# DearPoca/CppPathTracer

Hardware: AMD Instinct MI355X
Metric: Mpaths/sec (pixels×spp/s) at 1920×1080; achieved HBM GB/s vs peak (higher is better)
Workload: dtype f32; 1 GPU; c4: s1000 1920x1080 1024spp depth 16; width=1920, height=1080, spp=1024, max_depth=16, seed=1234, rows_rendered=1080, walk=ordered, schedule=cost, tail_consolidation=False, scaling=strong, parallelism=row-tiled x1 (interleaved 8-row blocks)

## Files before the change

cpppathtracer_amd/_lib.py:

```python
import ctypes
import os

from . import build as _build

_lib = None

_P = ctypes.c_void_p
_I = ctypes.c_int
_U32 = ctypes.c_uint32
_U64 = ctypes.c_uint64
_SZ = ctypes.c_size_t
PROTOTYPES = {
    "cpt_abi_version": (_I, []),
    "cpt_status_string": (ctypes.c_char_p, [_I]),
    "cpt_get_device_count": (_I, [_P]),
    "cpt_create": (_I, [_I, _P]),
    "cpt_destroy": (_I, [_P]),
    "cpt_last_error": (ctypes.c_char_p, [_P]),
    "cpt_set_stream": (_I, [_P, _P]),
    "cpt_camera_get_copy": (_I, [_P]),
    "cpt_set_scene": (_I, [_P, _P, _I]),
    "cpt_update_object": (_I, [_P, _I, _P]),
    "cpt_update_objects": (_I, [_P, _I, _P, _P]),
    "cpt_update_objects_rebuild": (_I, [_P, _I, _P, _P]),
    "cpt_last_update_ms": (_I, [_P, _P]),
    "cpt_get_material_count": (_I, [_P, _P]),
    "cpt_scene_bvh_export": (_I, [_P, _P, _P, _I, _P]),
    "cpt_bvh_build_host": (_I, [_P, _I, _P, _P, _I, _P]),
    "cpt_set_env_texture": (_I, [_P, _P, _I, _I, _I]),
    "cpt_bind_texture": (_I, [_P, _U64, _P, _I, _I, _I, _I, _I]),
    "cpt_set_frame": (_I, [_P, _I, _I, _P, _I]),
    "cpt_init_rng": (_I, [_P, _U64]),
    "cpt_read_rng": (_I, [_P, _P]),
    "cpt_write_rng": (_I, [_P, _P]),
    "cpt_render": (_I, [_P, _P, _I, _I, _U32]),
    "cpt_synchronize": (_I, [_P]),
    "cpt_read_accum": (_I, [_P, _P]),
    "cpt_clear_accum": (_I, [_P]),
    "cpt_read_aux": (_I, [_P, _P, _P]),
    "cpt_write_accum": (_I, [_P, _P]),
    "cpt_write_aux": (_I, [_P, _P, _P]),
    "cpt_copy_accum_device": (_I, [_P, _P, _SZ, _P]),
    "cpt_gather_rows": (_I, [_P, _P]),
    "cpt_last_gather_mode": (_I, [_P, _P, _P]),
    "cpt_set_debug_gather": (_I, [_P, _I]),
    "cpt_get_stats": (_I, [_P, _P]),
    "cpt_reset_stats": (_I, [_P]),
    "cpt_get_raw_counters": (_I, [_P, _P]),
    "cpt_get_walk_info": (_I, [_P, _P]),
    "cpt_debug_read_nodes": (_I, [_P, _P, _SZ, _P]),
    "cpt_debug_read_tile_order": (_I, [_P, _I, _P, _SZ, _P]),
    "cpt_measure_read_bandwidth": (_I, [_P, _SZ, _I, _P]),
    "cpt_measure_read_pattern": (_I, [_P, _I, _SZ, _I, _P]),
    "cpt_cap_disk_bound": (_I, [ctypes.c_float, _P]),
    "cpt_last_render_ms": (_I, [_P, _P]),
    "cpt_get_diag_counters": (_I, [_P, _P]),
    "cpt_get_execdiag_counters": (_I, [_P, _P]),
    "cpt_last_kernel_stats": (_I, [_P, _P, _P]),
    "cpt_denoise_mix": (_I, [_P, _U32, _P]),
    "cpt_host_register": (_I, [_P, _SZ]),
    "cpt_host_unregister": (_I, [_P]),
    "cpt_denoise_mix_band": (_I, [_P, _U32, _I, _I, _P]),
    "cpt_copy_bgra_device": (_I, [_P, _P, _SZ, _P]),
    "cpt_last_display_ms": (_I, [_P, _P]),
    "cpt_reset_display": (_I, [_P]),
    "cpt_display_band": (_I, [_P, _P, _P]),
    "cpt_debug_timeline": (_I, [_P, _P, _I]),
    "cpt_tile_costs": (_I, [_P, _P, _I, _I, ctypes.c_uint32, _P, _SZ]),
    "cpt_read_mix": (_I, [_P, _P, _SZ]),
    "cpt_math_batch": (_I, [_P, _I, _P, _P, _P, _SZ]),
    "cpt_selftest_qdiv": (_I, [_P, _I, _U64, _U64, _P, _I]),
    "cpt_set_debug_consolidation": (_I, [_P, _U32, _I, _I]),
    "cpt_set_debug_grid": (_I, [_P, _I, _I]),
    "cpt_render_adaptive": (_I, [_P, _P, _I, _I, _I, ctypes.c_float, _I, _U32]),
    "cpt_adaptive_begin": (_I, [_P, _P, _I, _I, _I, ctypes.c_float, _I, _U32]),
    "cpt_adaptive_step": (_I, [_P, _P]),
    "cpt_read_noise": (_I, [_P, _P, _SZ]),
    "cpt_adaptive_info": (_I, [_P, _P, _P, _I, _P]),
    "cpt_adaptive_decide_host": (_I, [ctypes.c_float, ctypes.c_float, ctypes.c_float, ctypes.c_float, _P, _P]),
    "cpt_read_moments": (_I, [_P, _P, _SZ]),
    "cpt_write_moments": (_I, [_P, _P, _SZ]),
    "cpt_filter_frame": (_I, [_P, _I, ctypes.c_float, _I]),
    "cpt_read_filtered": (_I, [_P, _P, _P, _SZ]),
    "cpt_last_filter_ms": (_I, [_P, _P]),
    "cpt_filter_prepare_host": (_I, [_SZ, _P, _P, _P, _P]),
    "cpt_filter_level_host": (_I, [_I, _I, _I, _P, _P, _P, ctypes.c_float, _I, _P]),
}

CPT_RENDER_ACCUMULATE = 0x1
CPT_RENDER_AUX = 0x2
CPT_RENDER_STATS = 0x4
CPT_RENDER_SYNC = 0x8
CPT_PATH_MEGAKERNEL = 0x000
CPT_PATH_WAVEFRONT = 0x100
CPT_TRAVERSAL_ORDERED = 0x200
CPT_TRAVERSAL_PLAIN_LEAVES = 0x400
CPT_SCHEDULE_COST = 0x800
CPT_SCHEDULE_CONSOLIDATE = 0x1000
CPT_SCHEDULE_NO_CONSOLIDATE = 0x2000
CPT_SCHEDULE_PREVIOUS = 0x4000
CPT_ERR_STATE = 5
CPT_ERR_DEVICE = 7


class CptError(RuntimeError):
    def __init__(self, status, msg):
        super().__init__(f"[cpt status {status}] {msg}")
        self.status = status


def lib_path() -> str:
    return _build.LIB_PATH


def load(build_if_missing: bool = True):
    global _lib
    if _lib is not None:
        return _lib
    path = os.environ.get("CPT_LIB_PATH") or _build.LIB_PATH
    if not os.path.exists(path):
        if not build_if_missing:
            raise CptError(-1, f"{path} missing: run __graft_entry__.build() (hipcc) first")
        _build.build()
    L = ctypes.CDLL(path)
    ab_variant = "CPT_LIB_PATH" in os.environ
    for name, (res, args) in PROTOTYPES.items():
        if ab_variant and not hasattr(L, name):
            continue
        f = getattr(L, name)
        f.restype = res
        f.argtypes = args
    if L.cpt_abi_version() != 1:
        raise CptError(-1, f"libcpt ABI {L.cpt_abi_version()} != 1")
    _lib = L
    return L


def check(status, ctx=None):
    if status != 0:
        L = load()
        msg = L.cpt_last_error(ctx)
        raise CptError(status, (msg or b"").decode() or L.cpt_status_string(status).decode())
    return status
```

cpppathtracer_amd/csrc/cpt_capi_render.cpp:

```cpp
#include <hip/hip_runtime.h>

#include <algorithm>
#include <cstdlib>
#include <cstring>
#include <type_traits>
#include <utility>

#include "cpt_context.hpp"

using namespace cpt::ctx;

constexpr int PREV_ORDER_EVERY = 8;

void cpt::ctx::fill_params(cpt_ctx* c, const cpt_camera* cam, int spp, int max_depth, uint32_t flags, cpt::KParams& p) {
    std::memset(&p, 0, sizeof(p));
    p.nodes = c->d_nodes;
    p.mats = c->d_mats;
    p.n_nodes = c->n_bvh;
    p.n_walk = c->n_walk;
    p.n_wide = c->n_wide;
    p.n_unb = c->n_unb;
    p.n_leaves = c->n_wide > 0 ? c->n_leaves : 0;
    p.ordered = (flags & CPT_TRAVERSAL_ORDERED) ? ((flags & CPT_TRAVERSAL_PLAIN_LEAVES) ? 2 : 1) : 0;
    p.env = c->d_env;
    p.env_w = c->env_w;
    p.env_h = c->env_h;
    p.env_cols = c->d_env ? c->env_cols : 0;
    for (int k = 0; k < 3; ++k) {
        p.cam.origin[k] = (&cam->origin.x)[k];
        p.cam.u[k] = (&cam->u.x)[k];
        p.cam.v[k] = (&cam->v.x)[k];
        p.cam.top_left[k] = (&cam->top_left_corner.x)[k];
        p.cam.horizontal[k] = (&cam->horizontal.x)[k];
        p.cam.vertical[k] = (&cam->vertical.x)[k];
    }
    p.cam.lens_radius = cam->lens_radius;
    p.cam.width = cam->width;
    p.cam.height = cam->height;
    p.cam.inv_w = 1.0 / (double)(float)cam->width;
    p.cam.inv_h = 1.0 / (double)(float)cam->height;
    p.rows = c->frame.d_rows;
    p.n_rows = c->n_rows;
    p.width = c->width;
    p.rng = c->frame.d_rng;
    p.accum = c->frame.d_accum;
    p.normal = c->frame.d_normal;
    p.depth = c->frame.d_depth;
    p.stats = c->d_stats;
    p.work = c->d_work;
    p.spp = spp;
    p.max_depth = max_depth;
    p.accumulate = (flags & CPT_RENDER_ACCUMULATE) ? 1 : 0;
    p.lanes = 64;
#ifdef CPT_DIAGNOSTIC_LANES
    if (const char* e = getenv("CPT_LANES_PER_WAVE")) p.lanes = std::max(1, std::min(64, atoi(e)));
    if (const char* e = getenv("CPT_REPLICATE")) p.replicate = std::max(1, std::min(64, atoi(e)));
#endif
    if (p.replicate < 1) p.replicate = 1;
    if (c->dbg_lanes_per_wave > 0) p.lanes = c->dbg_lanes_per_wave;
    p.error = c->d_work + 4;
    p.dbg = c->dbg;
    p.keeper_spin_log2 = c->keeper_spin_log2;
    p.publish_wait_log2 = c->publish_wait_log2;
}

int cpt::ctx::renderable(cpt_ctx* c, const cpt_camera* cam, const char* who) {
    if (!c->scene_set) return fail(c, CPT_ERR_STATE, "%s: cpt_set_scene first", who);
    if (!c->frame.set || !c->frame.rng_set) return fail(c, CPT_ERR_STATE, "%s: cpt_set_frame + cpt_init_rng first", who);
    if (cam->width != c->width || cam->height != c->height)
        return fail(c, CPT_ERR_INVALID_ARG, "%s: camera %dx%d vs frame %dx%d", who, cam->width, cam->height, c->width, c->height);
    return CPT_OK;
}

size_t cpt::ctx::n_tiles(const cpt_ctx* c) { return (size_t)cpt::TileGrid{c->width, c->n_rows}.count(); }

int WfStorage::alloc(cpt_ctx* c, size_t npix, cpt::WfState& view) {
    WfStorage fresh;
    cpt::WfState v{};
    int rc = CPT_OK;
    auto take = [&](auto*& slot, size_t count) {
        using T = std::remove_reference_t<decltype(*slot)>;
        if (rc != CPT_OK) return;
        fresh.mem.emplace_back();
        rc = fresh.mem.back().ensure(c, count * sizeof(T));
        slot = reinterpret_cast<T*>(fresh.mem.back().get());
    };
    for (int b = 0; b < 2; ++b)
        for (float4** a : {&v.ray_o[b], &v.ray_d[b], &v.att[b], &v.rad[b], &v.aux[b]}) take(*a, npix);
    take(v.hit_p, npix);
    take(v.hit_n, npix);
    for (int b = 0; b < 2; ++b) {
        take(v.rng_a[b], npix);
        take(v.rng_b[b], npix);
    }
    for (int32_t** q : {&v.queue[0], &v.queue[1], &v.ident}) take(*q, npix);
    take(v.counts, 8);
    if (rc != CPT_OK) return rc;
    *this = std::move(fresh);
    view = v;
    return CPT_OK;
}

static int ensure_wavefront(cpt_ctx* c, const cpt::KParams& p, hipStream_t s) {
    Frame& f = c->frame;
    if (f.wavefront.ready || c->n_rows == 0) return CPT_OK;
    if (int rc = f.wavefront.mem.alloc(c, c->npix(), f.wavefront.view)) return rc;
    HIP_TRY(c, cpt::wavefront_build_ident(p, f.wavefront.view, s));
    f.wavefront.ready = true;
    return CPT_OK;
}

int TileSchedule::previous_begin(cpt_ctx* c, cpt::KParams& p, hipStream_t s) {
    const size_t npix = c->npix();
    if (prev_order_valid) p.tile_order = d_prev_order;
    if (int rc = d_prev_d.ensure(c, npix)) return rc;
    if (!prev_d_valid) {
        HIP_TRY(c, hipMemcpyAsync(d_prev_d, c->frame.d_rng + 5 * npix, npix * sizeof(uint32_t), hipMemcpyDeviceToDevice, s));
        prev_d_valid = true;
    }
    return CPT_OK;
}

int TileSchedule::previous_refresh(cpt_ctx* c, const cpt::KParams& p, hipStream_t s) {
    if (prev_order_valid && ++prev_since_order < PREV_ORDER_EVERY) return CPT_OK;
    int rc;
    if ((rc = d_scratch.ensure(c, cpt::tile_schedule_scratch_bytes(c->width, c->n_rows))) != CPT_OK) return rc;
    if ((rc = d_prev_order.ensure(c, n_tiles(c))) != CPT_OK) return rc;
    HIP_TRY(c, cpt::launch_tile_order_from_draws(p, d_prev_d, d_scratch, d_scratch.capacity(), d_prev_order, s));
    prev_d_valid = true;
    prev_order_valid = true;
    prev_since_order = 0;
    return CPT_OK;
}

constexpr int PILOT_MAX = 16, PILOT_DIV = 128;
int cpt::ctx::cost_pilot_passes(int spp) { return std::min(PILOT_MAX, std::max(1, spp / PILOT_DIV)); }
int cpt::ctx::cost_pilot(cpt_ctx* c, const cpt::KParams& p, int passes, hipStream_t s) {
    Frame& f = c->frame;
    int rc;
    if ((rc = f.schedule.d_scratch.ensure(c, cpt::tile_schedule_scratch_bytes(c->width, c->n_rows))) != CPT_OK) return rc;
    if ((rc = f.schedule.d_cost_order.ensure(c, n_tiles(c))) != CPT_OK) return rc;
    HIP_TRY(c, cpt::launch_tile_schedule(p, passes, f.schedule.d_scratch, f.schedule.d_scratch.capacity(), f.schedule.d_cost_order,
                                         c->dbg_max_workgroups, s));
    return CPT_OK;
}

int cpt::ctx::consolidation_slab(cpt_ctx* c, cpt::KParams& p, int spp, uint32_t flags) {
    const size_t cus = (size_t)c->cus;
    const size_t frame_px = c->npix(), grid_lanes = 1024u * cus;
    const bool cons = (flags & CPT_SCHEDULE_CONSOLIDATE) ||
                      (!(flags & CPT_SCHEDULE_NO_CONSOLIDATE) && spp >= 512 && frame_px > grid_lanes &&
                       frame_px <= 4u * grid_lanes);
    if (!cons || spp <= 1) return CPT_OK;
    const size_t cap = 3u * 256u * cus;
    if (int rc = c->d_resume.ensure(c, 5 * cap)) return rc;
    p.resume = c->d_resume;
    p.resume_cap = cap;
    return CPT_OK;
}

extern "C" {

int cpt_render(cpt_ctx* c, const cpt_camera* cam, int spp, int max_depth, uint32_t flags) {
    if (!c || !cam) return CPT_ERR_INVALID_ARG;
    if (spp < 0 || max_depth < 0 || max_depth > (int)cpt::MAX_RECURSION_DEPTH_SET)
        return fail(c, CPT_ERR_INVALID_ARG, "cpt_render: spp %d, max_depth %d (must be 0..32)", spp, max_depth);
    CPT_REFUSE_PENDING(c, "cpt_render");
    if (int rc = renderable(c, cam, "cpt_render")) return rc;
    Frame& f = c->frame;
    HIP_TRY(c, hipSetDevice(c->device));
    hipStream_t s = c->stream();
    int rc;
    const bool aux = (flags & CPT_RENDER_AUX) != 0;
    if (aux) {
        if ((rc = f.d_normal.ensure(c, c->npix() * 3)) != CPT_OK) return rc;
        if ((rc = f.d_depth.ensure(c, c->npix())) != CPT_OK) return rc;
    }
    cpt::KParams p;
    fill_params(c, cam, spp, max_depth, flags, p);
    const bool wavefront = (flags & CPT_PATH_WAVEFRONT) != 0;
    const bool work = spp > 0 && c->n_rows > 0;
    if (wavefront && (rc = ensure_wavefront(c, p, s)) != CPT_OK) return rc;
    HIP_TRY(c, hipEventRecord(c->t_render.t0, s));
    if (wavefront) {
        if (!p.accumulate && c->n_rows > 0) HIP_TRY(c, hipMemsetAsync(f.d_accum, 0, c->npix() * sizeof(float4), s));
        int launches = 0;
        HIP_TRY(c, hipEventRecord(c->ev_main, s));
        HIP_TRY(c, cpt::launch_wavefront(p, f.wavefront.view, (flags & CPT_RENDER_STATS) != 0, aux, s, &launches));
        c->last_launches = launches;
        HIP_TRY(c, hipEventRecord(c->t_render.t1, s));
    } else {
        c->last_launches = 1;
        const bool cost = (flags & CPT_SCHEDULE_COST) && work;
        const bool previous = !(flags & CPT_SCHEDULE_COST) && (flags & CPT_SCHEDULE_PREVIOUS) && work;
        if (previous && (rc = f.schedule.previous_begin(c, p, s)) != CPT_OK) return rc;
        if (cost) {
            if ((rc = cost_pilot(c, p, cost_pilot_passes(spp), s)) != CPT_OK) return rc;
            p.tile_order = f.schedule.d_cost_order;
        }
        if ((rc = consolidation_slab(c, p, spp, flags)) != CPT_OK) return rc;
        HIP_TRY(c, hipEventRecord(c->ev_main, s));
        HIP_TRY(c, cpt::launch_megakernel(p, (flags & CPT_RENDER_STATS) != 0, aux, c->dbg_max_workgroups, s));
        HIP_TRY(c, hipEventRecord(c->t_render.t1, s));
        if (previous && (rc = f.schedule.previous_refresh(c, p, s)) != CPT_OK) return rc;
    }
    c->t_render.recorded = true;
    if (flags & CPT_RENDER_SYNC) return sync_checked(c);
    return CPT_OK;
}

int cpt_tile_costs(cpt_ctx* c, const cpt_camera* cam, int passes, int max_depth, uint32_t flags, uint32_t* out,
                   size_t n_out) {
    if (!c || !cam || !out || passes < 1 || max_depth < 0 || max_depth > (int)cpt::MAX_RECURSION_DEPTH_SET)
        return CPT_ERR_INVALID_ARG;
    if (int rc = renderable(c, cam, "cpt_tile_costs")) return rc;
    if (n_out < n_tiles(c)) return fail(c, CPT_ERR_INVALID_ARG, "cpt_tile_costs: %zu < %zu tiles", n_out, n_tiles(c));
    if (n_tiles(c) == 0) return CPT_OK;
    HIP_TRY(c, hipSetDevice(c->device));
    hipStream_t s = c->stream();
    cpt::KParams p;
    fill_params(c, cam, passes, max_depth, flags & (CPT_TRAVERSAL_ORDERED | CPT_TRAVERSAL_PLAIN_LEAVES), p);
    if (int rc = cost_pilot(c, p, passes, s)) return rc;
    HIP_TRY(c, hipMemcpyAsync(out, c->frame.schedule.d_scratch, n_tiles(c) * sizeof(uint32_t), hipMemcpyDeviceToHost, s));
    return sync_checked(c);
}

int cpt_set_debug_consolidation(cpt_ctx* c, uint32_t flags, int keeper_spin_log2, int publish_wait_log2) {
    if (!c || keeper_spin_log2 < 0 || keeper_spin_log2 > 30 || publish_wait_log2 < 0 || publish_wait_log2 > 30 ||
        (flags & ~3u))
        return c ? fail(c, CPT_ERR_INVALID_ARG, "cpt_set_debug_consolidation: bad arguments") : CPT_ERR_INVALID_ARG;
    c->dbg = flags;
    c->keeper_spin_log2 = keeper_spin_log2;
    c->publish_wait_log2 = publish_wait_log2;
    return CPT_OK;
}

int cpt_set_debug_grid(cpt_ctx* c, int max_workgroups, int lanes_per_wave) {
    if (!c || max_workgroups < 0 || lanes_per_wave < 0 || lanes_per_wave > 64)
        return c ? fail(c, CPT_ERR_INVALID_ARG, "cpt_set_debug_grid: bad arguments") : CPT_ERR_INVALID_ARG;
    c->dbg_max_workgroups = max_workgroups;
    c->dbg_lanes_per_wave = lanes_per_wave;
    return CPT_OK;
}

int cpt_last_render_ms(cpt_ctx* c, float* ms) {
    if (!c || !ms) return CPT_ERR_INVALID_ARG;
    if (!c->t_render.recorded) return fail(c, CPT_ERR_STATE, "cpt_last_render_ms: nothing rendered");
    HIP_TRY(c, hipSetDevice(c->device));
    HIP_TRY(c, hipEventSynchronize(c->t_render.t1));
    HIP_TRY(c, hipEventElapsedTime(ms, c->t_render.t0, c->t_render.t1));
    c->last_kernel_ms = *ms;
    return CPT_OK;
}

int cpt_last_kernel_stats(cpt_ctx* c, float* avg_ms, int* launches) {
    if (!c || !avg_ms || !launches) return CPT_ERR_INVALID_ARG;
    float ms = 0.f;
    int rc = cpt_last_render_ms(c, &ms);
    if (rc != CPT_OK) return rc;
    HIP_TRY(c, hipEventElapsedTime(&ms, c->ev_main, c->t_render.t1));
    *launches = c->last_launches;
    *avg_ms = c->last_launches > 0 ? ms / (float)c->last_launches : 0.f;
    return CPT_OK;
}

}
```

cpppathtracer_amd/csrc/cpt_context.hpp:

```cpp
#pragma once

#include <hip/hip_runtime.h>

#include <cstdint>
#include <string>
#include <vector>

#include "../../include/cpt.h"
#include "cpt_devmem.hpp"
#include "cpt_host.hpp"
#include "cpt_internal.hpp"
#include "cpt_tiles.hpp"

using cpt::Mat;
using cpt::Node;
using cpt::TexDesc;
using cpt::ctx::DevBuf;
using cpt::ctx::DevEvent;
using cpt::host::HostBvh;

struct WfStorage {
    std::vector<DevBuf<uint8_t>> mem;
    int alloc(cpt_ctx* c, size_t npix, cpt::WfState& view);
};


struct TileSchedule {
    DevBuf<uint8_t> d_scratch;
    DevBuf<uint32_t> d_cost_order;
    DevBuf<uint32_t> d_prev_d, d_prev_order;

    void rng_replaced() {
        prev_d_valid = prev_order_valid = false;
        prev_since_order = 0;
    }
    void draws_moved() { prev_d_valid = false; }
    const uint32_t* previous_order() const { return prev_order_valid ? d_prev_order.get() : nullptr; }
    int previous_begin(cpt_ctx* c, cpt::KParams& p, hipStream_t s);
    int previous_refresh(cpt_ctx* c, const cpt::KParams& p, hipStream_t s);

private:
    bool prev_d_valid = false, prev_order_valid = false;
    int prev_since_order = 0;
};

struct WavefrontState {
    cpt::WfState view{};
    WfStorage mem;
    bool ready = false;
};

struct DisplayBand {
    DevBuf<float> d_mix;
    DevBuf<uint8_t> d_bgra;
    DevBuf<float4> d_sink;
    int y0 = -1, y1 = -1;
};

struct AdaptiveState {
    DevBuf<float4> d_snap;
    DevBuf<float> d_stat;
    DevBuf<uint32_t> d_keep, d_order[2], d_count;
    bool done = false;
    std::vector<uint32_t> rounds;
    uint64_t passes = 0;
    struct Pending {
        bool on = false, queued = false;
        cpt::KParams p{};
        bool stats = false, aux = false;
        int batch = 0, min_spp = 0, max_rounds = 0;
        float rel_error = 0.f;
        int round = 0;
        uint32_t active = 0;
        int into = 0;
    } pending;

    bool has_result(size_t npix) const { return done && d_stat.capacity() >= 4 * npix; }
    void adopt_result() {
        rounds.clear();
        passes = 0;
        done = true;
    }
};

struct FilterState {
    DevBuf<float4> d_plane[2];
    DevBuf<uint8_t> d_ok;
    int result = -1;
};

struct Frame {
    bool set = false, rng_set = false;
    DevBuf<int32_t> d_rows;
    DevBuf<uint32_t> d_rng;
    DevBuf<float4> d_accum;
    DevBuf<float> d_normal, d_depth;
    DevBuf<uint32_t> d_scratch_w, d_scratch_m;
    TileSchedule schedule;
    WavefrontState wavefront;
    DisplayBand display;
    AdaptiveState adaptive;
    FilterState filter;
};

struct TimedSpan {
    DevEvent t0, t1;
    bool recorded = false;
};

struct cpt_ctx {
    int device = 0;
    int cus = 1;
    cpt::ctx::DevStream own_stream;
    hipStream_t user_stream = nullptr;
    TimedSpan t_render;
    DevEvent ev_main;
    TimedSpan t_display;
    TimedSpan t_filter;
    std::string err;

    std::vector<cpt_object> objs;
    HostBvh bvh;
    std::vector<Node> lin;
    std::vector<int> pos_of_node;
    int n_bvh = 0;
    int n_walk = 0;
    int n_wide = 0;
    int n_unb = 0;
    int n_leaves = 0;
    std::vector<Mat> mats_h;
    std::vector<int> mat_have_tex;
    std::vector<uint64_t> mat_tex;
    std::vector<int> mat_of_obj;
    DevBuf<Node> d_nodes;
    DevBuf<Mat> d_mats;
    bool scene_set = false;
    std::vector<cpt::RefitNode> refit_plan;
    std::vector<int32_t> refit_parent, refit_height, refit_walk_leaf;
    std::vector<cpt::Box6> refit_boxes;
    std::vector<uint8_t> refit_mark;
    int refit_n_ref = 0;
    DevBuf<cpt::RefitNode> d_refit_plan;
    DevBuf<cpt::Box6> d_refit_boxes;
    DevBuf<uint8_t> d_refit_work;
    float last_update_ms = 0.f;

    struct Texture { uint64_t handle; DevBuf<uint32_t> d_texels; int w, h, cols, addr, filter; };
    std::vector<Texture> textures;
    DevBuf<TexDesc> d_texdescs;
    DevBuf<int32_t> d_tex_of_mat;

    DevBuf<uint32_t> d_env;
    int env_w = 1, env_h = 1, env_cols = 0;

    int width = 0, height = 0, n_rows = 0;
    std::vector<int32_t> rows_h;
    uint64_t frame_gen = 0;
    Frame frame;

    DevBuf<uint32_t> d_jumps;
    DevBuf<unsigned long long> d_stats;
    DevBuf<uint32_t> d_work;
    DevBuf<uint4> d_resume;
    float last_kernel_ms = 0.f;
    int last_launches = 0;
    struct GatherMap {
        const cpt_ctx* src = nullptr;
        uint64_t src_gen = 0, dst_gen = 0;
        int src_device = -1;
        bool peer = false;
        int mode = -1;
        DevBuf<int32_t> d_map;
    };
    std::vector<GatherMap> gather_maps;
    DevBuf<float4> d_gather;
    DevBuf<float> d_gather_stat;
    cpt::ctx::HostPinned<uint32_t> h_ad_words;
    DevEvent ev_round;
    DevEvent ev_ready;
    DevEvent ev_gathered;
    DevEvent ev_caller;
    DevEvent ev_copied;
    uint32_t dbg = 0;
    bool force_staged_gather = false;
    int keeper_spin_log2 = 0, publish_wait_log2 = 0;
    int dbg_max_workgroups = 0, dbg_lanes_per_wave = 0;

    hipStream_t stream() const { return user_stream ? user_stream : (hipStream_t)own_stream; }
    size_t npix() const { return (size_t)n_rows * width; }
};

namespace cpt {
namespace ctx {

#define CPT_REFUSE_PENDING(ctx, who)                                                                              \
    do {                                                                                                          \
        if ((ctx)->frame.adaptive.pending.on)                                                                           \
            return fail((ctx), CPT_ERR_STATE, who ": an adaptive render is pending (cpt_adaptive_step until 0)"); \
    } while (0)

int check_device_error(cpt_ctx* c);
int sync_checked(cpt_ctx* c);
int copy_ordered(cpt_ctx* c, void* dst, const void* src, size_t bytes, hipStream_t caller);
int renderable(cpt_ctx* c, const cpt_camera* cam, const char* who);
void fill_params(cpt_ctx* c, const cpt_camera* cam, int spp, int max_depth, uint32_t flags, cpt::KParams& p);
size_t n_tiles(const cpt_ctx* c);
int cost_pilot_passes(int spp);
int cost_pilot(cpt_ctx* c, const cpt::KParams& p, int passes, hipStream_t s);
int consolidation_slab(cpt_ctx* c, cpt::KParams& p, int spp, uint32_t flags);

int material_slot(cpt_ctx* c, const cpt_material& m);
void linearise_all(cpt_ctx* c);
int upload_scene(cpt_ctx* c);
int upload_materials(cpt_ctx* c);
int device_refit(cpt_ctx* c, int n, const int* indices, bool mats_changed);

}
}
```

cpppathtracer_amd/csrc/cpt_host.hpp:

```cpp
#pragma once

#include <cstdint>
#include <vector>

#include "../../include/cpt.h"
#include "cpt_internal.hpp"

namespace cpt {
namespace host {

struct F3 { float x, y, z; };

inline float MIN_(float a, float b) { return a < b ? a : b; }
inline float MAX_(float a, float b) { return a > b ? a : b; }
inline float ABS_(float a) { return a >= 0 ? a : -a; }

F3 aabb_max(const cpt_object& o);
F3 aabb_min(const cpt_object& o);

struct BNode {
    F3 bmin, bmax;
    bool is_object;
    int left, right, obj, parent;
    int axis;
};

struct HostBvh {
    std::vector<BNode> nodes;
    std::vector<int> leaf_of_object;
};

void build_host_bvh(HostBvh& b, const std::vector<cpt_object>& objs);
float cap_disk_bound(float r);
Node make_node(const BNode& n, const std::vector<cpt_object>& objs, const std::vector<int>& mat_of_obj);
void linearise(const HostBvh& b, const std::vector<cpt_object>& objs, const std::vector<int>& mat_of_obj,
               std::vector<Node>& out, std::vector<int>& pos_of_node, int octant, const std::vector<int>* ref_pos,
               int root = 0, const std::vector<int>& prefix = {});

namespace sah {
int leaf(HostBvh& t, const std::vector<cpt_object>& O, int o);
int build(HostBvh& t, const std::vector<cpt_object>& O, std::vector<int>& idx, int l, int r);
}

constexpr int WIDE_STACK = CPT_WSTACK;
int linearise_wide(const HostBvh& w, int root, const std::vector<int>& pos0, int n_bvh, int n_unb,
                   std::vector<Node>& out, int* n_leaves_out, std::vector<int>& slot_of, std::vector<int>& leaf_of);

const std::vector<uint32_t>& jump_tables();
void curand_seed_state(uint64_t seed, uint32_t out[6]);

}
}
```

cpppathtracer_amd/csrc/cpt_host_bvh.cpp:

```cpp
#include <algorithm>
#include <cfloat>
#include <cmath>
#include <cstring>
#include <functional>
#include <mutex>
#include <queue>
#include <vector>

#include "cpt_host.hpp"

namespace cpt {
namespace host {


F3 aabb_max(const cpt_object& o) {
    const float tol = 2e-5f * 5.f;
    switch (o.type) {
        case CPT_PRIM_SPHERE: {
            float r = ABS_(o.radius);
            return F3{o.center.x + r, o.center.y + r, o.center.z + r};
        }
        case CPT_PRIM_PLATFORM: return F3{1e30f * 5, o.y_pos + tol, 1e30f * 5};
        case CPT_PRIM_CYLINDER:
            return F3{o.center.x + ABS_(o.radius), o.center.y + o.height / 2 + tol, o.center.z + ABS_(o.radius)};
        default: return F3{0, 0, 0};
    }
}

F3 aabb_min(const cpt_object& o) {
    const float tol = 2e-5f * 5.f;
    switch (o.type) {
        case CPT_PRIM_SPHERE: {
            float r = ABS_(o.radius);
            return F3{o.center.x - r, o.center.y - r, o.center.z - r};
        }
        case CPT_PRIM_PLATFORM: return F3{-1e30f * 5, o.y_pos - tol, -1e30f * 5};
        case CPT_PRIM_CYLINDER:
            return F3{o.center.x - ABS_(o.radius), o.center.y - o.height / 2 - tol, o.center.z - ABS_(o.radius)};
        default: return F3{0, 0, 0};
    }
}


static int divide(HostBvh& b, const std::vector<cpt_object>& objs, std::vector<int>& idx, int l, int r) {
    if (l >= r) return -1;
    int ret = (int)b.nodes.size();
    b.nodes.push_back(BNode{});
    F3 lmin = aabb_min(objs[idx[l]]), lmax = aabb_max(objs[idx[l]]);
    if (l == r - 1) {
        BNode& n = b.nodes[ret];
        n.left = n.right = -1;
        n.bmin = lmin; n.bmax = lmax;
        n.is_object = true;
        n.obj = idx[l];
        b.leaf_of_object[idx[l]] = ret;
        return ret;
    }
    float minx = lmin.x, miny = lmin.y, minz = lmin.z, maxx = lmax.x, maxy = lmax.y, maxz = lmax.z;
    for (int i = l + 1; i < r; ++i) {
        F3 a = aabb_min(objs[idx[i]]), c = aabb_max(objs[idx[i]]);
        minx = MIN_(minx, a.x); miny = MIN_(miny, a.y); minz = MIN_(minz, a.z);
        maxx = MAX_(maxx, c.x); maxy = MAX_(maxy, c.y); maxz = MAX_(maxz, c.z);
    }
    float sx = maxx - minx, sy = maxy - miny, sz = maxz - minz;
    int axis = (sx >= sy && sx >= sz) ? 0 : (sy >= sz ? 1 : 2);
    std::vector<std::pair<float, int>> keyed;
    keyed.reserve(r - l);
    for (int i = l; i < r; ++i) {
        F3 a = aabb_min(objs[idx[i]]), c = aabb_max(objs[idx[i]]);
        float lo = axis == 0 ? a.x : axis == 1 ? a.y : a.z;
        float hi = axis == 0 ? c.x : axis == 1 ? c.y : c.z;
        keyed.emplace_back((lo + hi) / 2, idx[i]);
    }
    std::stable_sort(keyed.begin(), keyed.end(),
                     [](const std::pair<float, int>& p, const std::pair<float, int>& q) { return p.first < q.first; });
    for (int i = l; i < r; ++i) idx[i] = keyed[i - l].second;
    int mid = (l + r) / 2;
    int left = divide(b, objs, idx, l, mid);
    int right = divide(b, objs, idx, mid, r);
    BNode& n = b.nodes[ret];
    n.left = left; n.right = right;
    n.bmin = F3{minx, miny, minz};
    n.bmax = F3{maxx, maxy, maxz};
    n.is_object = false;
    n.obj = -1;
    n.axis = axis;
    b.nodes[left].parent = ret;
    b.nodes[right].parent = ret;
    return ret;
}

void build_host_bvh(HostBvh& b, const std::vector<cpt_object>& objs) {
    b.nodes.clear();
    b.leaf_of_object.assign(objs.size(), -1);
    if (objs.empty()) return;
    b.nodes.reserve(2 * objs.size());
    std::vector<int> idx(objs.size());
    for (size_t i = 0; i < objs.size(); ++i) idx[i] = (int)i;
    divide(b, objs, idx, 0, (int)objs.size());
    b.nodes[0].parent = -1;
}

float cap_disk_bound(float r) {
    if (!(r > 0.0f)) return -1.0f;
    if (r == INFINITY) return FLT_MAX;
    const double m = ((double)std::nextafter(r, 0.0f) + (double)r) * 0.5;
    const double x = m * m;
    float c = (float)x;
    if ((double)c > x) c = std::nextafter(c, -INFINITY);
    return c;
}

Node make_node(const BNode& n, const std::vector<cpt_object>& objs, const std::vector<int>& mat_of_obj) {
    Node g;
    if (n.is_object) {
        const cpt_object& o = objs[n.obj];
        g.a0 = o.center.x; g.a1 = o.center.y; g.a2 = o.center.z;
        g.b0 = o.radius; g.b1 = o.y_pos; g.b2 = o.height;
        int type = (o.type >= 0 && o.type <= 2) ? o.type : 3;
        if (type == CPT_PRIM_CYLINDER) g.b1 = cap_disk_bound(o.radius);
        if (type == CPT_PRIM_SPHERE) {
            const double inv_r = 1.0 / (double)o.radius;
            uint32_t w[2];
            std::memcpy(w, &inv_r, 8);
            std::memcpy(&g.b1, &w[0], 4);
            std::memcpy(&g.b2, &w[1], 4);
        }
        g.code = (mat_of_obj[n.obj] << 2) | type;
    } else {
        g.a0 = n.bmin.x; g.a1 = n.bmin.y; g.a2 = n.bmin.z;
        g.b0 = n.bmax.x; g.b1 = n.bmax.y; g.b2 = n.bmax.z;
        g.code = -1;
    }
    g.miss = -1;
    return g;
}

void linearise(const HostBvh& b, const std::vector<cpt_object>& objs, const std::vector<int>& mat_of_obj,
               std::vector<Node>& out, std::vector<int>& pos_of_node, int octant, const std::vector<int>* ref_pos,
               int root, const std::vector<int>& prefix) {
    const size_t base = out.size();
    pos_of_node.assign(b.nodes.size(), -1);
    for (int leaf : prefix) {
        pos_of_node[leaf] = (int)(out.size() - base);
        out.push_back(make_node(b.nodes[leaf], objs, mat_of_obj));
        out.back().miss = (*ref_pos)[leaf];
    }
    if (b.nodes.empty() || root < 0) return;
    struct Frame { int node; int stage; };
    std::vector<Frame> st;
    st.push_back({root, 0});
    while (!st.empty()) {
        Frame& f = st.back();
        const BNode& n = b.nodes[f.node];
        if (f.stage == 0) {
            pos_of_node[f.node] = (int)(out.size() - base);
            out.push_back(make_node(n, objs, mat_of_obj));
            if (n.is_object) {
                out.back().miss = ref_pos ? (*ref_pos)[f.node] : pos_of_node[f.node];
                st.pop_back();
                continue;
            }
            if (octant >= 0) {
                Node& q = out.back();
                if (octant & 1) std::swap(q.a0, q.b0);
                if (octant & 2) std::swap(q.a1, q.b1);
                if (octant & 4) std::swap(q.a2, q.b2);
            }
            f.stage = 1;
            const bool right_first = octant < 0 || ((octant >> n.axis) & 1);
            st.push_back({right_first ? n.right : n.left, 0});
        } else if (f.stage == 1) {
            f.stage = 2;
            const bool right_first = octant < 0 || ((octant >> n.axis) & 1);
            st.push_back({right_first ? n.left : n.right, 0});
        } else {
            out[base + pos_of_node[f.node]].miss = (int)(out.size() - base);
            st.pop_back();
        }
    }
}

namespace sah {
constexpr int NB = 16;
inline float comp(const F3& v, int a) { return a == 0 ? v.x : (a == 1 ? v.y : v.z); }
inline F3 fmin3(const F3& a, const F3& b) { return F3{MIN_(a.x, b.x), MIN_(a.y, b.y), MIN_(a.z, b.z)}; }
inline F3 fmax3(const F3& a, const F3& b) { return F3{MAX_(a.x, b.x), MAX_(a.y, b.y), MAX_(a.z, b.z)}; }
inline float area(const F3& lo, const F3& hi) {
    const float dx = hi.x - lo.x, dy = hi.y - lo.y, dz = hi.z - lo.z;
    return 2.f * (dx * dy + dy * dz + dz * dx);
}
inline int bin_of(float c, float e0, float e1) { return std::min(NB - 1, (int)((c - e0) / (e1 - e0) * NB)); }

int leaf(HostBvh& t, const std::vector<cpt_object>& O, int o) {
    BNode n{};
    n.bmin = aabb_min(O[o]);
    n.bmax = aabb_max(O[o]);
    n.is_object = true;
    n.left = n.right = -1;
    n.obj = o;
    n.parent = -1;
    t.nodes.push_back(n);
    return (int)t.nodes.size() - 1;
}

int build(HostBvh& t, const std::vector<cpt_object>& O, std::vector<int>& idx, int l, int r) {
    if (r - l == 1) return leaf(t, O, idx[l]);
    F3 lo = aabb_min(O[idx[l]]), hi = aabb_max(O[idx[l]]);
    F3 clo{1e30f, 1e30f, 1e30f}, chi{-1e30f, -1e30f, -1e30f};
    std::vector<float> cen(3 * (r - l));
    for (int i = l; i < r; ++i) {
        const F3 a = aabb_min(O[idx[i]]), b = aabb_max(O[idx[i]]);
        lo = fmin3(lo, a);
        hi = fmax3(hi, b);
        const F3 c{(a.x + b.x) * .5f, (a.y + b.y) * .5f, (a.z + b.z) * .5f};
        cen[3 * (i - l)] = c.x; cen[3 * (i - l) + 1] = c.y; cen[3 * (i - l) + 2] = c.z;
        clo = fmin3(clo, c);
        chi = fmax3(chi, c);
    }
    float best = 3.0e38f;
    int best_axis = -1, best_bin = -1;
    for (int axis = 0; axis < 3; ++axis) {
        const float e0 = comp(clo, axis), e1 = comp(chi, axis);
        if (!(e1 > e0)) continue;
        int cnt[NB] = {0};
        F3 blo[NB], bhi[NB];
        for (int b = 0; b < NB; ++b) { blo[b] = F3{1e30f, 1e30f, 1e30f}; bhi[b] = F3{-1e30f, -1e30f, -1e30f}; }
        for (int i = l; i < r; ++i) {
            const int b = bin_of(cen[3 * (i - l) + axis], e0, e1);
            cnt[b]++;
            blo[b] = fmin3(blo[b], aabb_min(O[idx[i]]));
            bhi[b] = fmax3(bhi[b], aabb_max(O[idx[i]]));
        }
        for (int sp = 1; sp < NB; ++sp) {
            int nl = 0, nr = 0;
            F3 llo{1e30f, 1e30f, 1e30f}, lhi{-1e30f, -1e30f, -1e30f}, rlo = llo, rhi = lhi;
            for (int b = 0; b < sp; ++b) if (cnt[b]) { nl += cnt[b]; llo = fmin3(llo, blo[b]); lhi = fmax3(lhi, bhi[b]); }
            for (int b = sp; b < NB; ++b) if (cnt[b]) { nr += cnt[b]; rlo = fmin3(rlo, blo[b]); rhi = fmax3(rhi, bhi[b]); }
            if (!nl || !nr) continue;
            const float cost = area(llo, lhi) * nl + area(rlo, rhi) * nr;
            if (cost < best) { best = cost; best_axis = axis; best_bin = sp; }
        }
    }
    int axis, mid;
    if (best_axis < 0) {
        axis = 0;
        mid = (l + r) / 2;
    } else {
        axis = best_axis;
        const float e0 = comp(clo, axis), e1 = comp(chi, axis);
        std::vector<int> lhs, rhs;
        for (int i = l; i < r; ++i)
            (bin_of(cen[3 * (i - l) + axis], e0, e1) < best_bin ? lhs : rhs).push_back(idx[i]);
        std::copy(lhs.begin(), lhs.end(), idx.begin() + l);
        std::copy(rhs.begin(), rhs.end(), idx.begin() + l + (int)lhs.size());
        mid = l + (int)lhs.size();
    }
    const int me = (int)t.nodes.size();
    t.nodes.push_back(BNode{});
    const int L = build(t, O, idx, l, mid), R = build(t, O, idx, mid, r);
    BNode& n = t.nodes[me];
    n.bmin = lo; n.bmax = hi;
    n.is_object = false;
    n.left = L; n.right = R; n.obj = -1; n.parent = -1; n.axis = axis;
    t.nodes[L].parent = me;
    t.nodes[R].parent = me;
    return me;
}
}


int linearise_wide(const HostBvh& w, int root, const std::vector<int>& pos0, int n_bvh, int n_unb,
                   std::vector<Node>& out, int* n_leaves_out, std::vector<int>& slot_of, std::vector<int>& leaf_of) {
    std::vector<int> wbin;
    std::vector<std::vector<int>> kids;
    std::vector<int> wide_of(w.nodes.size(), -1);
    auto area = [&](int b) {
        const BNode& n = w.nodes[b];
        const float dx = n.bmax.x - n.bmin.x, dy = n.bmax.y - n.bmin.y, dz = n.bmax.z - n.bmin.z;
        return dx * dy + dy * dz + dz * dx;
    };
    int max_push = 0;
    std::function<void(int, int)> make = [&](int b, int pushed) {
        const int id = (int)wbin.size();
        wbin.push_back(b);
        wide_of[b] = id;
        std::vector<int> ch = {w.nodes[b].left, w.nodes[b].right};
        while (ch.size() < 4) {
            int best = -1;
            float ba = -1.f;
            for (size_t k = 0; k < ch.size(); ++k)
                if (!w.nodes[ch[k]].is_object && area(ch[k]) > ba) { ba = area(ch[k]); best = (int)k; }
            if (best < 0) break;
            const int x = ch[best];
            ch.erase(ch.begin() + best);
            ch.insert(ch.begin() + best, {w.nodes[x].left, w.nodes[x].right});
        }
        kids.push_back(ch);
        pushed += (int)ch.size() - 1;
        max_push = std::max(max_push, pushed);
        for (int x : ch)
            if (!w.nodes[x].is_object) make(x, pushed);
    };
    make(root, n_unb);
    if (max_push + 1 > WIDE_STACK) return 0;
    const int n_wide = (int)wbin.size();
    std::vector<int> li_of(w.nodes.size(), -1), leaf_pos;
    for (int k = 0; k < n_unb; ++k) leaf_pos.push_back(k);
    for (int id = 0; id < n_wide; ++id)
        for (int x : kids[id])
            if (w.nodes[x].is_object && li_of[x] < 0) {
                li_of[x] = (int)leaf_pos.size();
                leaf_pos.push_back(pos0[x]);
            }
    if ((int)leaf_pos.size() > 32765) return 0;
    if (n_wide > cpt::LDS_TREE_NODES) {
        std::vector<char> top(n_wide, 0);
        std::priority_queue<std::pair<float, int>, std::vector<std::pair<float, int>>, std::greater<>> pq;
        pq.emplace(-area(wbin[0]), 0);
        for (int taken = 0; !pq.empty() && taken < cpt::LDS_TREE_NODES; ++taken) {
            const int id = pq.top().second;
            pq.pop();
            top[id] = 1;
            for (int x : kids[id])
                if (!w.nodes[x].is_object) pq.emplace(-area(x), wide_of[x]);
        }
        std::vector<int> order;
        order.reserve(n_wide);
        for (int part = 1; part >= 0; --part)
            for (int id = 0; id < n_wide; ++id)
                if (top[id] == part) order.push_back(id);
        std::vector<int> new_id(n_wide);
        for (int k = 0; k < n_wide; ++k) new_id[order[k]] = k;
        std::vector<int> wbin2(n_wide);
        std::vector<std::vector<int>> kids2(n_wide);
        for (int k = 0; k < n_wide; ++k) {
            wbin2[k] = wbin[order[k]];
            kids2[k] = kids[order[k]];
        }
        wbin.swap(wbin2);
        kids.swap(kids2);
        for (int& x : wide_of)
            if (x >= 0) x = new_id[x];
    }
    if (n_wide > 32767) return 0;
    for (int p : pos0)
        if (p > 32766) return 0;
    const size_t base = out.size();
    const size_t n_compact = (size_t)(n_wide * 7 + 1) / 2;
    out.resize(base + n_compact + leaf_pos.size());
    for (size_t i = 0; i < leaf_pos.size(); ++i) out[base + n_compact + i] = out[(size_t)n_bvh + leaf_pos[i]];
    *n_leaves_out = (int)leaf_pos.size();
    uint32_t* compact = reinterpret_cast<uint32_t*>(&out[base]);
    std::memset(compact, 0, n_compact * sizeof(Node));
    for (int id = 0; id < n_wide; ++id) {
        const std::vector<int>& ch = kids[id];
        std::vector<int> ord;
        std::function<void(int)> rec = [&](int x) {
            if (std::find(ch.begin(), ch.end(), x) != ch.end()) { ord.push_back(x); return; }
            rec(w.nodes[x].left);
            rec(w.nodes[x].right);
        };
        rec(wbin[id]);
        uint32_t* q = compact + (size_t)id * 28;
        for (int k = 0; k < 4; ++k) {
            F3 lo{1e30f, 1e30f, 1e30f}, hi{-1e30f, -1e30f, -1e30f};
            int32_t r = -1;
            if (k < (int)ord.size()) {
                const BNode& n = w.nodes[ord[k]];
                lo = n.bmin;
                hi = n.bmax;
                r = n.is_object ? ~(li_of[ord[k]] + 1) : wide_of[ord[k]];
            }
            const float l3[3] = {lo.x, lo.y, lo.z}, h3[3] = {hi.x, hi.y, hi.z};
            for (int a = 0; a < 3; ++a) {
                std::memcpy(&q[(2 * a) * 4 + k], &l3[a], 4);
                std::memcpy(&q[(2 * a + 1) * 4 + k], &h3[a], 4);
            }
            q[24 + (k >> 1)] |= (uint32_t)(uint16_t)(int16_t)r << (16 * (k & 1));
            if (k < (int)ord.size()) slot_of[ord[k]] = id * 4 + k;
        }
    }
    leaf_of = li_of;
    for (size_t b = 0; b < w.nodes.size(); ++b)
        if (w.nodes[b].is_object && leaf_of[b] < 0 && pos0[b] >= 0 && pos0[b] < n_unb) leaf_of[b] = pos0[b];
    return n_wide;
}

}
}
```

cpppathtracer_amd/csrc/cpt_internal.hpp:

```cpp
#pragma once

#include <hip/hip_runtime.h>
#include <stdint.h>

#include "cpt_device.hpp"

#define CPT_WSTACK 32

namespace cpt {

constexpr int LDS_TREE_NODES = 512;
__host__ __device__ __forceinline__ int lds_tree_nodes(int n_wide) { return n_wide < LDS_TREE_NODES ? n_wide : LDS_TREE_NODES; }

struct CamK {
    float origin[3];
    float u[3], v[3];
    float top_left[3], horizontal[3], vertical[3];
    float lens_radius;
    int width, height;
    double inv_w, inv_h;
};

struct KParams {
    const Node* nodes;
    const Mat* mats;
    int n_nodes, n_walk;
    int n_wide;
    int n_unb;
    int n_leaves;
    int ordered;
    const uint32_t* env;
    int env_w, env_h, env_cols;
    CamK cam;
    const int32_t* rows;
    int n_rows, width;
    uint32_t* rng;
    float4* accum;
    float* normal;
    float* depth;
    unsigned long long* stats;
    uint32_t* work;
    const uint32_t* tile_order;
    uint32_t* tile_cost;
    int spp, max_depth, accumulate;
    int lanes;
    int replicate;
    uint4* resume;
    size_t resume_cap;
    uint32_t* error;
    uint32_t dbg;
    int keeper_spin_log2, publish_wait_log2;
    uint32_t n_active;
};

enum : uint32_t {
    CPT_DEVERR_KEEPER_TIMEOUT = 1u,
    CPT_DEVERR_PUBLISH_TIMEOUT = 2u,
    CPT_DEVERR_RESUME_CAP = 4u,
};

size_t tile_schedule_scratch_bytes(int width, int n_rows);
hipError_t launch_cost_pilot(const KParams& p, int max_workgroups, hipStream_t stream);
hipError_t launch_tile_order_from_draws(const KParams& p, uint32_t* d_prev, void* scratch, size_t scratch_bytes,
                                        uint32_t* order, hipStream_t stream);
hipError_t launch_tile_schedule(const KParams& p, int passes, void* scratch, size_t scratch_bytes, uint32_t* order,
                                int max_workgroups, hipStream_t stream);

struct AdaptiveRound {
    const uint32_t* order;
    uint32_t n_active;
    int width, n_rows;
    const float4* accum;
    float4* snap;
    float* stat;
    uint32_t* keep;
    float rel_error;
    int eligible, last;
};
hipError_t launch_tile_noise(const AdaptiveRound& a, hipStream_t stream);
hipError_t launch_compact_order(const uint32_t* src, const uint32_t* keep, uint32_t n, int width, int n_rows,
                                uint32_t* dst, uint32_t* out, hipStream_t stream);

hipError_t launch_filter_prepare(const float4* accum, const float* stat, size_t npix, float4* plane, uint8_t* ok,
                                 hipStream_t stream);
hipError_t launch_filter_level(const float4* in, const float* normal3, const uint8_t* ok, float4* out, int width, int height,
                               int step, float sig2, int sharpness_log2, hipStream_t stream);

struct WfState {
    float4 *ray_o[2], *ray_d[2], *att[2], *rad[2], *aux[2];
    float4 *hit_p, *hit_n;
    uint4* rng_a[2];
    uint2* rng_b[2];
    int32_t* queue[2];
    int32_t* ident;
    uint32_t* counts;
};

struct RefitNode {
    int32_t left, right;
    int32_t slot;
    int32_t leaf;
    int32_t pos[8];
};
struct Box6 { float lo[3], hi[3]; };
struct RefitLeaf {
    Node prim;
    Box6 box;
    int32_t ref_id, walk_id;
};
hipError_t launch_refit(const RefitLeaf* leaves_in, int n_leaves, const int32_t* dirty, const int32_t* level_end,
                        int n_levels, int n_ref, const RefitNode* nodes_plan, Box6* boxes, Node* nodes, uint32_t* image,
                        Node* leaves, hipStream_t stream);

hipError_t launch_megakernel(const KParams& p, bool stats, bool aux, int max_workgroups, hipStream_t stream);
hipError_t launch_wavefront(const KParams& p, WfState& w, bool stats, bool aux, hipStream_t stream, int* launches);
hipError_t wavefront_build_ident(const KParams& p, WfState& w, hipStream_t stream);
hipError_t launch_prepare_materials(Mat* mats, const int32_t* tex_of_mat, const TexDesc* texs, int n,
                                    hipStream_t stream);
hipError_t launch_init_rng(const uint32_t* jumps, const uint32_t seed_state[6], int width, const int32_t* rows,
                           int n_rows, uint32_t* scratch_w, uint32_t* scratch_mats, uint32_t* rng, hipStream_t stream);
hipError_t launch_math_batch(int op, const float* a, const float* b, float* out, size_t n, hipStream_t stream);
hipError_t launch_stream_read(const float4* p, size_t n, float* out, int grid, hipStream_t stream);
hipError_t launch_read_pattern(int bpl, const float* p, size_t n_lanes, float* out, int grid, hipStream_t stream);
hipError_t timeline_read(unsigned long long* out, int n, hipStream_t stream);
hipError_t launch_selftest_qdiv(int which, uint64_t n, uint64_t seed, unsigned long long* out, int out_len,
                                hipStream_t stream);
hipError_t launch_selftest_dn_weight(int which, uint64_t n, unsigned long long* out, int out_len, hipStream_t stream);
hipError_t launch_stitch_rows(const float4* src_acc, const float* src_nrm, const float* src_dep, const int32_t* dst_row,
                              int width, int n_rows, float4* acc, float* nrm, float* dep, hipStream_t stream);
hipError_t launch_stitch_moments(const float* src, size_t src_npix, const int32_t* dst_row, int width, int n_rows,
                                 float* dst, size_t dst_npix, hipStream_t stream);
constexpr int DN_SINK_SLOTS = 1024 * 64;
hipError_t launch_denoise_mix(const float4* accum, const float* normal, const float* depth, float* mix, uint8_t* out,
                              uint8_t* out_host, float4* sink, int width, int height, int row0, int ctx_rows, int y0, int y1,
                              uint32_t cur_sample_idx, hipStream_t stream);

}
```

cpppathtracer_amd/csrc/cpt_megakernel.hip:

```cpp
#include <hip/hip_runtime.h>
#include <stdint.h>

#include <algorithm>

#include "cpt_path.hpp"

namespace cpt {

__device__ __forceinline__ uint32_t ld_coherent(const uint32_t* a) {
    return __hip_atomic_load(a, __ATOMIC_RELAXED, __HIP_MEMORY_SCOPE_AGENT);
}
__device__ __forceinline__ void st_coherent(uint32_t* a, uint32_t v) {
    __hip_atomic_store(a, v, __ATOMIC_RELAXED, __HIP_MEMORY_SCOPE_AGENT);
}
__device__ __forceinline__ void wait_stores() { asm volatile("s_waitcnt vmcnt(0)" ::: "memory"); }
template <int BLK> constexpr int ho_slots() { return (BLK / 256 - 1) * 256; }

struct Lane {
    uint32_t xy;
    uint32_t pix;
    uint32_t tile;
    Xorwow s;
    v3 sum;
    float passes;
    int left;
    template <bool ACC>
    __device__ __forceinline__ void load(const KParams& p, size_t npix) {
        s.v0 = p.rng[pix];
        s.v1 = p.rng[npix + pix];
        s.v2 = p.rng[2 * npix + (size_t)pix];
        s.v3 = p.rng[3 * npix + (size_t)pix];
        s.v4 = p.rng[4 * npix + (size_t)pix];
        s.d = p.rng[5 * npix + (size_t)pix];
        const float4 a = (p.accumulate && ACC) ? p.accum[pix] : make_float4(0.f, 0.f, 0.f, 0.f);
        sum = mk(a.x, a.y, a.z);
        passes = a.w;
    }
    __device__ __forceinline__ void store_rng(const KParams& p, size_t npix) const {
        p.rng[pix] = s.v0;
        p.rng[npix + pix] = s.v1;
        p.rng[2 * npix + (size_t)pix] = s.v2;
        p.rng[3 * npix + (size_t)pix] = s.v3;
        p.rng[4 * npix + (size_t)pix] = s.v4;
        p.rng[5 * npix + (size_t)pix] = s.d;
    }
};

template <int BLK>
struct PendingSky {
    float* q;
    __device__ __forceinline__ void park(const v3& dir, const v3& rad, const v3& att) const {
        q[0 * BLK] = dir.x; q[1 * BLK] = dir.y; q[2 * BLK] = dir.z;
        q[3 * BLK] = rad.x; q[4 * BLK] = rad.y; q[5 * BLK] = rad.z;
        q[6 * BLK] = att.x; q[7 * BLK] = att.y; q[8 * BLK] = att.z;
    }
    __device__ __forceinline__ v3 dir() const { return mk(q[0 * BLK], q[1 * BLK], q[2 * BLK]); }
    __device__ __forceinline__ v3 rad() const { return mk(q[3 * BLK], q[4 * BLK], q[5 * BLK]); }
    __device__ __forceinline__ v3 att() const { return mk(q[6 * BLK], q[7 * BLK], q[8 * BLK]); }
};

__device__ __forceinline__ bool decode_pixel(const KParams& p, uint32_t id, int& x, int& ri, uint32_t& tile) {
    tile = id >> 6;
    if (p.tile_order) tile = p.tile_order[tile];
    return TileGrid{p.width, p.n_rows}.pixel(tile, id & 63, x, ri);
}


template <bool LDST> constexpr int mk_block() { return LDST ? LDS_BLOCK : 256; }
template <bool LDST> constexpr int mk_waves() { return LDST ? LDS_BLOCK / 256 : WAVES_PER_SIMD; }

template <bool STATS, bool AUX, bool PROBE, bool LDST, bool CONS, bool HYB>
__global__ void __launch_bounds__(mk_block<LDST>(), mk_waves<LDST>()) k_megakernel(const KParams p) {
    constexpr bool COUNT = STATS || PROBE;
    constexpr int BLK = mk_block<LDST>();
    __shared__ uint4 s_tree[LDST ? LDS_TREE_NODES * 7 : 1];
    pooldiag::init();
    if (LDST) {
        const uint4* src = reinterpret_cast<const uint4*>(p.nodes + wide_image_base(p));
        for (int i = threadIdx.x; i < 7 * lds_tree_nodes(p.n_wide); i += BLK) s_tree[i] = src[i];
        __syncthreads();
    }
    const int lane = threadIdx.x & 63;
    const size_t npix = (size_t)p.n_rows * p.width;
    const uint32_t n_work = (p.n_active ? p.n_active : (uint32_t)TileGrid{p.width, p.n_rows}.count()) * 64u;
    const uint32_t max_depth = (uint32_t)p.max_depth;
    Counters cnt{};
    uint32_t work_at_take = 0;

    Lane L;
    bool busy = false;
    bool exhausted = false;
    Ray ray;
    v3 att = mk1(1.f), rad = mk1(0.f);
    uint32_t depth = 0;
    bool first = true;
    v3 first_normal = mk1(0.f);

    __shared__ float pending_q[DEFER_MISS_ROUND > 0 ? 9 * BLK : 1];
    const PendingSky<BLK> pq{pending_q + threadIdx.x};
    bool pend = false;
    WalkState ws;
    ws.active = false;
    static_assert(!CONS || (LDST && !PROBE && ho_slots<BLK>() > 0), "consolidation needs the LDS walk");
    constexpr int QS = CONS ? ho_slots<BLK>() : 1;
    __shared__ uint32_t s_q[CONS ? 4 : 1];
    __shared__ uint8_t s_qflag[QS];
    const bool cons = CONS && (size_t)(blockIdx.x + 1) * QS <= p.resume_cap;
    if (CONS && !cons && threadIdx.x == 0) atomicOr(p.error, CPT_DEVERR_RESUME_CAP);
    uint4* const qslab = cons ? p.resume + 5 * (size_t)blockIdx.x * QS : nullptr;
    volatile uint32_t* const vq = s_q;
    const uint32_t level = __builtin_amdgcn_readfirstlane((uint32_t)(threadIdx.x >> 8));
    bool retiring = false;
    uint32_t idle_spins = 0;
    const uint32_t keeper_spins = 1u << (p.keeper_spin_log2 > 0 ? p.keeper_spin_log2 : 26);
    const uint32_t publish_wait = 1u << (p.publish_wait_log2 > 0 ? p.publish_wait_log2 : 22);
    if (cons) {
        if (threadIdx.x < 4)
            s_q[threadIdx.x] = threadIdx.x == 3 ? (uint32_t)(BLK / 64) : (threadIdx.x == 2 ? (p.dbg & 1u) : 0u);
        for (int i = threadIdx.x; i < QS; i += BLK) s_qflag[i] = 0;
        __syncthreads();
    }
    auto start_pass = [&]() {
        ray = ray_gen(kernarg_field<CamK>(offsetof(KParams, cam)), (int)(L.xy & 0xffffu), (int)(L.xy >> 16), L.s);
        att = mk1(1.f);
        rad = mk1(0.f);
        depth = 0;
        first = true;
    };
    const bool stat = STATIC_FIRST && LDST && !PROBE && p.lanes == 64 && p.tile_order != nullptr;
    const uint32_t n_static = gridDim.x * (uint32_t)BLK;
    bool first_take = true;
    uint32_t res_id = 0, res_end = 0, res_seen = 0;
    bool counter_done = false;
    stamps::init();
    timeline::State tl;
    timeline::init(tl);
    for (;;) {
        stamps::lap(5);
        stamps::count(8);
        timeline::round(tl, __ballot(busy), exhausted, level);
        if (cons && !retiring && level > 0 && exhausted && vq[3] == 0u && vq[2] <= level * (uint32_t)CONS_RETIRE_PER_LEVEL) retiring = true;
        bool begin = false;
        if (!exhausted && !retiring) {
            const KParams& p = kernarg_params();
            const uint64_t need = __ballot(!busy && lane < p.lanes);
            if (need) {
                const int leader = __ffsll((unsigned long long)need) - 1;
                uint32_t base = 0;
                uint32_t lane_id = 0;
                const bool first_take_was = first_take;
                first_take = false;
                if (stat && first_take_was) {
                    base = (level * (gridDim.x * 4u) + blockIdx.x * 4u + ((threadIdx.x >> 6) & 3u)) * 64u;
                    if (n_static >= n_work) exhausted = true;
                    lane_id = base + lane_rank(need);
                }
                else if (p.replicate == 1) {
                    const uint32_t n_need = wave_count(need);
                    const uint32_t avail = res_end - res_id;
                    const uint32_t off = stat ? n_static : 0u;
                    uint32_t nb = 0, ncnt = 0;
                    if (n_need > avail && !counter_done) {
                        const uint32_t want = n_need - avail;
                        uint32_t seen = res_seen;
                        if (p.spp >= 64 && res_seen + n_static < n_work) {
                            uint32_t cur = 0;
                            if (lane == leader) cur = __hip_atomic_load(p.work, __ATOMIC_RELAXED, __HIP_MEMORY_SCOPE_AGENT);
                            seen = __builtin_amdgcn_readfirstlane(__shfl(cur, leader)) + off;
                        }
                        uint32_t bsz = (uint32_t)TAKE_BATCH;
                        const uint32_t left_ids = n_work > seen ? n_work - seen : 0u;
                        if (p.spp >= 64) {
                            const uint64_t t = (uint64_t)bsz * left_ids / ((uint64_t)n_static * TAKE_TAPER);
                            bsz = t < bsz ? (uint32_t)t : bsz;
                        }
                        const bool batch_ok = p.spp >= 64 || left_ids > n_static;
                        const uint32_t grab = !CONS && batch_ok && bsz > want ? bsz : want;
                        if (lane == leader) nb = atomicAdd(p.work, grab);
                        nb = __builtin_amdgcn_readfirstlane(__shfl(nb, leader)) + off;
                        ncnt = grab;
                    }
                    if (ncnt) {
                        res_seen = nb + ncnt;
                        if (nb + ncnt >= n_work) counter_done = true;
                    }
                    const uint32_t rank = lane_rank(need);
                    lane_id = rank < avail ? res_id + rank : (rank - avail < ncnt ? nb + (rank - avail) : n_work);
                    if (ncnt) {
                        res_id = nb + min(n_need - avail, ncnt);
                        res_end = nb + ncnt;
                    } else {
                        res_id += n_need < avail ? n_need : avail;
                    }
                    if (counter_done && res_id >= res_end) exhausted = true;
                }
                else {
                    const uint32_t rep = (uint32_t)p.replicate;
                    const uint32_t n_take = ((uint32_t)__popcll(need) + rep - 1) / rep;
                    if (lane == leader) base = atomicAdd(p.work, n_take);
                    base = __shfl(base, leader) + (stat ? n_static : 0u);
                    if (base + n_take >= n_work) exhausted = true;
                    lane_id = base + lane_rank(need) / rep;
                }
                bool took = false;
                if ((need >> lane) & 1ull) {
                    const uint32_t id = lane_id;
                    int x, ri;
                    if (id < n_work && decode_pixel(p, id, x, ri, L.tile)) {
                        execdiag::lanes(p.stats + 64, 0);
                        L.xy = (uint32_t)x | ((uint32_t)p.rows[ri] << 16);
                        L.pix = (uint32_t)ri * (uint32_t)p.width + (uint32_t)x;
                        L.load<!PROBE>(p, npix);
                        L.left = p.spp;
                        first_normal = mk1(0.f);
                        if (PROBE) work_at_take = cnt.segments + cnt.nodes + cnt.prims;
                        if (max_depth == 0) {
                            for (; L.left > 0; --L.left) {
                                (void)ray_gen(p, (int)(L.xy & 0xffffu), (int)(L.xy >> 16), L.s);
                                L.sum = L.sum + mk1(0.f);
                                L.passes += 1.0f;
                            }
                        }
                        busy = true;
                        took = true;
                        begin = L.left > 0;
                    }
                }
                if (cons) {
                    const uint64_t t = __ballot(took);
                    if (t && lane == leader) atomicAdd(&s_q[2], (uint32_t)__popcll(t));
                    if (exhausted && lane == leader) atomicSub(&s_q[3], 1u);
                }
            }
        }
        if (cons && !retiring && exhausted) {
            const uint64_t need = __ballot(!busy && lane < p.lanes);
            const bool idle_wave = !__any(busy);
            bool quit = false;
            for (;;) {
                if (idle_wave) {
                    while (vq[1] == vq[0]) {
                        if (vq[3] == 0u && vq[2] == 0u) { quit = true; break; }
                        if (++idle_spins > keeper_spins) {
                            if (lane == 0) atomicOr(p.error, CPT_DEVERR_KEEPER_TIMEOUT);
                            quit = true;
                            break;
                        }
                        __builtin_amdgcn_s_sleep(16);
                    }
                    if (quit) break;
                }
                if (need && vq[1] != vq[0]) {
                    const int leader = __ffsll((unsigned long long)need) - 1;
                    uint32_t h = 0, n = 0;
                    if (lane == leader) {
                        for (int tries = 0; tries < 16; ++tries) {
                            h = vq[0];
                            uint32_t t = vq[1];
                            t = t < (uint32_t)QS ? t : (uint32_t)QS;
                            const uint32_t want = (uint32_t)__popcll(need);
                            n = t > h ? (t - h < want ? t - h : want) : 0u;
                            if (n == 0 || atomicCAS(&s_q[0], h, h + n) == h) break;
                            n = 0;
                        }
                    }
                    h = __shfl(h, leader);
                    n = __shfl(n, leader);
                    const uint32_t rank = lane_rank(need);
                    bool lost = false;
                    if (((need >> lane) & 1ull) && rank < n) {
                        const uint32_t slot = h + rank;
                        const volatile uint8_t* fl = s_qflag + slot;
                        for (uint32_t w = 0; *fl == 0 && w < publish_wait; ++w) __builtin_amdgcn_s_sleep(1);
                        lost = *fl == 0;
                    }
                    if (lost) {
                        atomicOr(p.error, CPT_DEVERR_PUBLISH_TIMEOUT);
                        atomicSub(&s_q[2], 1u);
                    } else if (((need >> lane) & 1ull) && rank < n) {
                        const uint32_t slot = h + rank;
                        const uint32_t* e = reinterpret_cast<const uint32_t*>(qslab + 5 * (size_t)slot);
                        auto ld4 = [&](int q) {
                            return make_uint4(ld_coherent(e + 4 * q), ld_coherent(e + 4 * q + 1), ld_coherent(e + 4 * q + 2),
                                              ld_coherent(e + 4 * q + 3));
                        };
                        const uint4 e0 = ld4(0), e1 = ld4(1), e2 = ld4(2), e3 = AUX ? ld4(3) : make_uint4(0u, 0u, 0u, 0u);
                        const uint32_t left = ld_coherent(e + 16);
                        L.pix = e0.x; L.xy = e0.y; L.s.v0 = e0.z; L.s.v1 = e0.w;
                        L.s.v2 = e1.x; L.s.v3 = e1.y; L.s.v4 = e1.z; L.s.d = e1.w;
                        L.sum = mk(__uint_as_float(e2.x), __uint_as_float(e2.y), __uint_as_float(e2.z));
                        L.passes = __uint_as_float(e2.w);
                        if (AUX) {
                            first_normal = mk(__uint_as_float(e3.x), __uint_as_float(e3.y), __uint_as_float(e3.z));
                        }
                        L.left = (int)left;
                        busy = true;
                        begin = true;
                    }
                }
                if (!idle_wave || __any(busy)) break;
                if (++idle_spins > keeper_spins) {
                    if (lane == 0) atomicOr(p.error, CPT_DEVERR_KEEPER_TIMEOUT);
                    quit = true;
                    break;
                }
            }
            if (quit) break;
        }
        if (begin) {
            execdiag::lanes(p.stats + 64, 10);
            start_pass();
        }
        stamps::lap(0);
        if (!__any(busy)) {
            if (!exhausted) continue;
            break;
        }
        Hit h;
        int code = -1;
        int tr = 2;
        bool hand_over = false;
        if (busy && L.left > 0) {
            if (COUNT && !ws.active) cnt.segments++;
            execdiag::lanes(p.stats + 64, 12);
            const RayK rk = make_rayk(ray);
            const bool finite_ray = !(ray.o.x != ray.o.x || ray.o.y != ray.o.y || ray.o.z != ray.o.z ||
                                      ray.d.x != ray.d.x || ray.d.y != ray.d.y || ray.d.z != ray.d.z);
            tr = trace_segment<COUNT, BLK, LDST, HYB>(p, rk, finite_ray, h, code, cnt, s_tree, ws, LDST ? SUSPEND_AT : 0);
        }
        stamps::lap(3);
        if (busy && L.left > 0 && tr != 2) {
            const bool hit = tr == 1;
            execdiag::lanes(p.stats + 64, 13);
            Shade sh;
            v3 attr_normal;
            if (hit) {
                if (COUNT) cnt.hits++;
                execdiag::lanes(p.stats + 64, 4);
                const Mat m = p.mats[code >> 2];
#ifdef CPT_EXECDIAG
                eval_material(m, h.normal, ray.d, L.s, sh, p.stats + 64);
#else
                eval_material(m, h.normal, ray.d, L.s, sh);
#endif
                attr_normal = h.normal;
                ray.o = h.pos;
                stamps::lap(4);
            } else {
                if (COUNT) cnt.misses++;
                sh.attenuation = mk1(0.f);
                sh.bounce = ray.d;
                attr_normal = -ray.d;
            }
            bool deferred = false;
            {
                const bool ends = !hit || !(depth + 1 < max_depth);
                const bool need_now = (pend && ends) || (!hit && L.left == 1);
                const bool flush = DEFER_MISS_ROUND == 0 || retiring || __ballot(need_now) != 0 ||
                                   wave_count(__ballot(pend || !hit)) * 64u >=
                                       (uint32_t)DEFER_MISS_ROUND * wave_count(__builtin_amdgcn_read_exec());
                if (flush) {
                    const KParams& p = kernarg_params();
                    const bool had = pend;
                    if (had || !hit) {
                        execdiag::lanes(p.stats + 64, 6);
                        const v3 dir = had ? pq.dir() : ray.d;
                        const v3 sky = miss_radiance(p, dir);
                        if (had) {
                            const v3 pr = pq.rad();
                            const v3 pa = pq.att();
                            L.sum = L.sum + (pr + pa * sky);
                            pend = false;
                        } else {
                            sh.radiance = sky;
                        }
                    }
                    if (had && !hit) {
                        if (L.left == 1 || retiring) {
                            execdiag::lanes(p.stats + 64, 7);
                            sh.radiance = miss_radiance(p, ray.d);
                        } else {
                            pq.park(ray.d, rad, att);
                            pend = true;
                            deferred = true;
                            sh.radiance = mk1(0.f);
                        }
                    }
                } else if (!hit) {
                    execdiag::lanes(p.stats + 64, 8);
                    pq.park(ray.d, rad, att);
                    pend = true;
                    deferred = true;
                    sh.radiance = mk1(0.f);
                }
            }
            if (!hit) depth = MAX_RECURSION_DEPTH_SET;
            rad = rad + att * sh.radiance;
            att = att * sh.attenuation;
            if (AUX && first) first_normal = mk1(0.f) + attr_normal;
            first = false;
            ray.d = normalize_u(sh.bounce);
            ray.tmin = BOUNCE_RAY_TMIN;
            ray.tmax = DEFAULT_RAY_TMAX;
            depth++;
            if (!(depth < max_depth)) {
                if (!deferred) L.sum = L.sum + rad;
                L.passes += 1.0f;
                if (--L.left > 0) {
                    if (retiring) hand_over = true;
                    else {
                        execdiag::lanes(p.stats + 64, 9);
                        start_pass();
                    }
                }
            }
        }
        if (cons) {
            const uint64_t ho = __ballot(hand_over);
            if (ho) {
                const int leader = __ffsll((unsigned long long)ho) - 1;
                uint32_t base = 0;
                if (lane == leader) base = atomicAdd(&s_q[1], (uint32_t)__popcll(ho));
                base = __shfl(base, leader);
                if (hand_over) {
                    execdiag::lanes(p.stats + 64, 14);
                    const uint32_t slot = base + lane_rank(ho);
                    {
                        uint32_t* e = reinterpret_cast<uint32_t*>(qslab + 5 * (size_t)slot);
                        const uint32_t w[20] = {L.pix, L.xy, L.s.v0, L.s.v1, L.s.v2, L.s.v3, L.s.v4, L.s.d,
                                                __float_as_uint(L.sum.x), __float_as_uint(L.sum.y), __float_as_uint(L.sum.z),
                                                __float_as_uint(L.passes), __float_as_uint(first_normal.x),
                                                __float_as_uint(first_normal.y), __float_as_uint(first_normal.z),
                                                0u, (uint32_t)L.left, 0u, 0u, 0u};
#pragma unroll
                        for (int k = 0; k < 17; ++k)
                            if (AUX || k < 12 || k == 16) st_coherent(e + k, w[k]);
                        wait_stores();
                        if (!(p.dbg & 2u)) *(volatile uint8_t*)(s_qflag + slot) = 1;
                        busy = false;
                    }
                    hand_over = false;
                }
            }
        }
        bool finished = false;
        if (busy && L.left == 0) {
            const KParams& p = kernarg_params();
            if (PROBE) {
                atomicMax(&p.tile_cost[L.tile], cnt.segments + cnt.nodes + cnt.prims - work_at_take);
            } else {
                execdiag::lanes(p.stats + 64, 11);
                p.accum[L.pix] = make_float4(L.sum.x, L.sum.y, L.sum.z, L.passes);
                if (AUX && p.spp > 0) {
                    p.normal[3 * (size_t)L.pix + 0] = first_normal.x;
                    p.normal[3 * (size_t)L.pix + 1] = first_normal.y;
                    p.normal[3 * (size_t)L.pix + 2] = first_normal.z;
                    p.depth[L.pix] = max_depth > 0 ? DEFAULT_RAY_TMAX : 0.f;
                }
                L.store_rng(p, npix);
            }
            busy = false;
            finished = true;
        }
        if (cons) {
            const uint64_t f = __ballot(finished);
            if (f && lane == __ffsll((unsigned long long)f) - 1) atomicSub(&s_q[2], (uint32_t)__popcll(f));
        }
    }
    stamps::flush(p.stats + 16);
    pooldiag::flush(p.stats + 64);
    timeline::flush(tl);
    if (STATS && !PROBE) {
        uint64_t a = wave_sum(cnt.segments), b = wave_sum(cnt.nodes), c = wave_sum(cnt.prims);
        uint64_t d = wave_sum(cnt.hits), e = wave_sum(cnt.misses);
        const uint64_t f = wave_sum(cnt.fallbacks);
        const uint64_t g = wave_sum(cnt.gnodes);
        if (lane == 0) {
            atomicAdd((unsigned long long*)&p.stats[0], (unsigned long long)a);
            atomicAdd((unsigned long long*)&p.stats[1], (unsigned long long)b);
            atomicAdd((unsigned long long*)&p.stats[2], (unsigned long long)c);
            atomicAdd((unsigned long long*)&p.stats[3], (unsigned long long)d);
            atomicAdd((unsigned long long*)&p.stats[4], (unsigned long long)e);
            if (f) atomicAdd((unsigned long long*)&p.stats[5], (unsigned long long)f);
            if (g) atomicAdd((unsigned long long*)&p.stats[6], (unsigned long long)g);
        }
    }
}

template <bool S, bool A, bool P, bool T, bool C = false, bool H = false>
static hipError_t launch_mk(const KParams& p, int max_workgroups, hipStream_t stream) {
    static int blocks_per_cu = -1, cus = 0;
    constexpr int block = mk_block<T>();
    if (blocks_per_cu < 0) {
        int dev = 0;
        hipError_t e = hipGetDevice(&dev);
        if (e == hipSuccess) e = hipDeviceGetAttribute(&cus, hipDeviceAttributeMultiprocessorCount, dev);
        if (e == hipSuccess)
            e = hipOccupancyMaxActiveBlocksPerMultiprocessor(&blocks_per_cu, k_megakernel<S, A, P, T, C, H>, block, 0);
        if (e != hipSuccess) return e;
        if (blocks_per_cu < 1) blocks_per_cu = 1;
    }
    const long long tiles = p.n_active ? (long long)p.n_active : (long long)TileGrid{p.width, p.n_rows}.count();
    const int per_wave = std::max(1, p.lanes / std::max(1, p.replicate));
    long long want = (tiles * 64 * ((64 + per_wave - 1) / per_wave) + block - 1) / block;
    long long grid = std::min<long long>(want, (long long)blocks_per_cu * cus);
    if (max_workgroups > 0) grid = std::min<long long>(grid, max_workgroups);
    if (grid < 1) return hipSuccess;
    hipLaunchKernelGGL((k_megakernel<S, A, P, T, C, H>), dim3((unsigned)grid), dim3(block), 0, stream, p);
    return hipGetLastError();
}

static bool use_lds_tree(const KParams& p) { return p.ordered == 1 && p.n_wide > 0; }

template <bool S, bool A, bool P, bool H>
static hipError_t launch_mk_lds(const KParams& p, int max_workgroups, hipStream_t stream) {
    if constexpr (!P && ho_slots<mk_block<true>()>() > 0) {
        if (p.resume) return launch_mk<S, A, P, true, true, H>(p, max_workgroups, stream);
    }
    return launch_mk<S, A, P, true, false, H>(p, max_workgroups, stream);
}

template <bool S, bool A, bool P>
static hipError_t launch_mk_any(const KParams& p, int max_workgroups, hipStream_t stream) {
    if (!use_lds_tree(p)) return launch_mk<S, A, P, false>(p, max_workgroups, stream);
    if (p.n_wide > LDS_TREE_NODES) return launch_mk_lds<S, A, P, true>(p, max_workgroups, stream);
    return launch_mk_lds<S, A, P, false>(p, max_workgroups, stream);
}

hipError_t launch_megakernel(const KParams& p, bool stats, bool aux, int max_workgroups, hipStream_t stream) {
    if (p.width <= 0 || p.n_rows <= 0) return hipSuccess;
    hipError_t e = hipMemsetAsync(p.work, 0, sizeof(uint32_t), stream);
    if (e != hipSuccess) return e;
    if (stats && aux) return launch_mk_any<true, true, false>(p, max_workgroups, stream);
    if (stats) return launch_mk_any<true, false, false>(p, max_workgroups, stream);
    if (aux) return launch_mk_any<false, true, false>(p, max_workgroups, stream);
    return launch_mk_any<false, false, false>(p, max_workgroups, stream);
}

hipError_t launch_cost_pilot(const KParams& p, int max_workgroups, hipStream_t stream) {
    return launch_mk_any<false, false, true>(p, max_workgroups, stream);
}

hipError_t timeline_read(unsigned long long* out, int n, hipStream_t stream) {
#ifdef CPT_TIMELINE
    if (n > timeline::TL_WORDS) n = timeline::TL_WORDS;
    void* sym = nullptr;
    hipError_t e = hipGetSymbolAddress(&sym, HIP_SYMBOL(timeline::g_tl));
    if (e == hipSuccess) e = hipMemcpyAsync(out, sym, (size_t)n * 8, hipMemcpyDeviceToHost, stream);
    if (e == hipSuccess) e = hipMemsetAsync(sym, 0, (size_t)timeline::TL_WORDS * 8, stream);
    if (e == hipSuccess) e = hipMemsetAsync((unsigned long long*)sym + 4 * timeline::TL_BINS, 0xff, 8, stream);
    if (e == hipSuccess) e = hipStreamSynchronize(stream);
    return e;
#else
    (void)out; (void)n; (void)stream;
    return hipErrorNotSupported;
#endif
}

__global__ void k_prepare_materials(Mat* mats, const int32_t* tex_of_mat, const TexDesc* texs, int n) {
    int i = blockIdx.x * blockDim.x + threadIdx.x;
    if (i >= n) return;
    Mat m = mats[i];
    const v3 kd = mk(m.att_x, m.att_y, m.att_z);
    const v3 rad = m.rad_x * kd;
    m.rad_x = rad.x; m.rad_y = rad.y; m.rad_z = rad.z;
    const int t = tex_of_mat ? tex_of_mat[i] : -1;
    if (t >= 0) {
        const TexDesc d = texs[t];
        const v3 c = tex_fetch_dyn(TexView{d.texels, d.w, d.h, d.cols}, d.addr, d.filter, 0.0f, 0.0f);
        m.att_x = c.x; m.att_y = c.y; m.att_z = c.z;
    }
    float alpha = dm::powf_(1000.0f, m.smoothness);
    m.inv_alpha = 1.0 / (double)alpha;
    m.inv_ior = 1.f / m.ior;
    if (m.type == 3) {
        float r0 = (1 - m.ior) / (1 + m.ior);
        r0 *= r0;
        m.schlick_r0 = r0;
    }
    mats[i] = m;
}

hipError_t launch_prepare_materials(Mat* mats, const int32_t* tex_of_mat, const TexDesc* texs, int n,
                                    hipStream_t stream) {
    if (n <= 0) return hipSuccess;
    hipLaunchKernelGGL(k_prepare_materials, dim3((n + 63) / 64), dim3(64), 0, stream, mats, tex_of_mat, texs, n);
    return hipGetLastError();
}

}
```

cpppathtracer_amd/csrc/cpt_path.hpp:

```cpp
#pragma once

#include <hip/hip_runtime.h>
#include <stdint.h>

#include "cpt_device.hpp"
#include "cpt_internal.hpp"
#include "cpt_stamps.hpp"
#include "cpt_tiles.hpp"
#include "cpt_tuning.hpp"

namespace cpt {

__device__ __forceinline__ int mirror_index(int i, int n) {
    if (i >= -n && i < 2 * n) {
        const int m = i < 0 ? -1 - i : i;
        return m >= n ? 2 * n - 1 - m : m;
    }
    int period = 2 * n;
    int m = i % period;
    if (m < 0) m += period;
    if (m >= n) m = period - 1 - m;
    return m;
}

// ... 242 lines not shown
};

__device__ __forceinline__ float walk_limit(float tmax) {
    return ((tmax + WALK_MARGIN_ABS) * (1.0f + 2.0f * WALK_MARGIN_REL)) * SLAB_GROW;
}

__device__ __forceinline__ bool slab_pass(float& lo, float hi, float t3, float limit) {
    lo = __builtin_fmaxf(lo, t3);
    return lo <= __builtin_fminf(hi, limit);
}

template <bool FAST, bool CONS = false>
__device__ __forceinline__ bool slab_reject(const Node& nd, const RayK& ray, float tmax) {
    if (CONS) {
        const bool px = ray.inx >= 0.0f, py = ray.iny >= 0.0f, pz = ray.inz >= 0.0f;
        float lo = __builtin_fmaxf(__builtin_fmaxf(__builtin_fmaf(px ? nd.a0 : nd.b0, ray.inx, ray.nx),
                                                   __builtin_fmaf(py ? nd.a1 : nd.b1, ray.iny, ray.ny)),
                                   __builtin_fmaf(pz ? nd.a2 : nd.b2, ray.inz, ray.nz));
        const float hi = __builtin_fminf(__builtin_fminf(__builtin_fmaf(px ? nd.b0 : nd.a0, ray.ifx, ray.fx),
                                                         __builtin_fmaf(py ? nd.b1 : nd.a1, ray.ify, ray.fy)),
                                         __builtin_fmaf(pz ? nd.b2 : nd.a2, ray.ifz, ray.fz));
        return !slab_pass(lo, hi, ray.t3, tmax);
    }
    float t0x = qdiv_raw(nd.a0 - ray.o.x, ray.yx), t1x = qdiv_raw(nd.b0 - ray.o.x, ray.yx);
    float t0y = qdiv_raw(nd.a1 - ray.o.y, ray.yy), t1y = qdiv_raw(nd.b1 - ray.o.y, ray.yy);
    float t0z = qdiv_raw(nd.a2 - ray.o.z, ray.yz), t1z = qdiv_raw(nd.b2 - ray.o.z, ray.yz);
    float mn = __builtin_fminf(__builtin_fminf(__builtin_fminf(__builtin_fabsf(t0x), __builtin_fabsf(t1x)),
                                               __builtin_fminf(__builtin_fabsf(t0y), __builtin_fabsf(t1y))),
                               __builtin_fminf(__builtin_fabsf(t0z), __builtin_fabsf(t1z)));
    if (__builtin_expect(mn < FLT_MIN_NORMAL, 0)) {
        t0x = (nd.a0 - ray.o.x) / ray.d.x; t1x = (nd.b0 - ray.o.x) / ray.d.x;
        t0y = (nd.a1 - ray.o.y) / ray.d.y; t1y = (nd.b1 - ray.o.y) / ray.d.y;
        t0z = (nd.a2 - ray.o.z) / ray.d.z; t1z = (nd.b2 - ray.o.z) / ray.d.z;
    }
    float lo = -DEFAULT_RAY_TMAX * 2, hi = DEFAULT_RAY_TMAX * 2;
    float lx, hx, ly, hy, lz, hz;
    if (FAST) {
        lx = __builtin_fmaxf(lo, __builtin_fminf(t0x, t1x));
        hx = __builtin_fminf(hi, __builtin_fmaxf(t0x, t1x));
    } else {
        lx = tmax_(lo, tmin_(t0x, t1x));
        hx = tmin_(hi, tmax_(t0x, t1x));
    }
    lo = ray.d.x != 0.f ? lx : lo;
    hi = ray.d.x != 0.f ? hx : hi;
    if (FAST) {
        ly = __builtin_fmaxf(lo, __builtin_fminf(t0y, t1y));
        hy = __builtin_fminf(hi, __builtin_fmaxf(t0y, t1y));
    } else {
        ly = tmax_(lo, tmin_(t0y, t1y));
        hy = tmin_(hi, tmax_(t0y, t1y));
    }
    lo = ray.d.y != 0.f ? ly : lo;
    hi = ray.d.y != 0.f ? hy : hi;
    if (FAST) {
        lz = __builtin_fmaxf(lo, __builtin_fminf(t0z, t1z));
        hz = __builtin_fminf(hi, __builtin_fmaxf(t0z, t1z));
    } else {
        lz = tmax_(lo, tmin_(t0z, t1z));
        hz = tmin_(hi, tmax_(t0z, t1z));
    }
    lo = ray.d.z != 0.f ? lz : lo;
    hi = ray.d.z != 0.f ? hz : hi;
    return lo > hi || lo > tmax || hi < ray.tmin;
}


__device__ __forceinline__ bool slab_reject_octant(const Node& nd, const RayK& ray, float limit) {
    float lo = __builtin_fmaxf(__builtin_fmaxf(__builtin_fmaf(nd.a0, ray.inx, ray.nx), __builtin_fmaf(nd.a1, ray.iny, ray.ny)),
                               __builtin_fmaf(nd.a2, ray.inz, ray.nz));
    const float hi = __builtin_fminf(__builtin_fminf(__builtin_fmaf(nd.b0, ray.ifx, ray.fx), __builtin_fmaf(nd.b1, ray.ify, ray.fy)),
                                     __builtin_fmaf(nd.b2, ray.ifz, ray.fz));
    return !slab_pass(lo, hi, ray.t3, limit);
}

typedef unsigned int v4u32 __attribute__((ext_vector_type(4)));

struct BufSrc {
    __amdgpu_buffer_rsrc_t rsrc;
    uint32_t base;
    __device__ __forceinline__ Node operator()(uint32_t i) const {
        const uint32_t off = base + (i << 5);
        const v4u32 a = __builtin_amdgcn_raw_buffer_load_b128(rsrc, off, 0, 0);
        const v4u32 b = __builtin_amdgcn_raw_buffer_load_b128(rsrc, off + 16, 0, 0);
        Node n;
        n.a0 = __uint_as_float(a.x); n.a1 = __uint_as_float(a.y); n.a2 = __uint_as_float(a.z); n.miss = (int32_t)a.w;
        n.b0 = __uint_as_float(b.x); n.b1 = __uint_as_float(b.y); n.b2 = __uint_as_float(b.z); n.code = (int32_t)b.w;
        return n;
    }
};

__host__ __device__ __forceinline__ int wide_compact_nodes(int n_wide) { return (7 * n_wide + 1) / 2; }
__host__ __device__ __forceinline__ int wide_image_base(const KParams& p) { return p.n_nodes + 8 * p.n_walk; }
__host__ __device__ __forceinline__ int wide_leaves_base(const KParams& p) {
    return wide_image_base(p) + wide_compact_nodes(p.n_wide);
}

__device__ __forceinline__ __amdgpu_buffer_rsrc_t node_rsrc(const KParams& p) {
    const uint32_t bytes = (uint32_t)(wide_leaves_base(p) + p.n_leaves) * (uint32_t)sizeof(Node);
    return __builtin_amdgcn_make_buffer_rsrc((void*)p.nodes, (short)0, (int)bytes, 0x00020000);
}

__device__ __forceinline__ uint32_t walk_order(const KParams& p, v3 d, int& n) {
    const int oct = (d.x < 0.f ? 1 : 0) | (d.y < 0.f ? 2 : 0) | (d.z < 0.f ? 4 : 0);
    n = p.n_walk;
    return (uint32_t)(p.n_nodes + oct * p.n_walk);
}

__device__ __forceinline__ void leaf_aabb(const Node& nd, Node& box) {
    const float tol = 2e-5f * 5.f;
    const int type = nd.code & 3;
    const float r = nd.b0 >= 0 ? nd.b0 : -nd.b0;
    if (type == 0) {
        box.a0 = nd.a0 - r; box.a1 = nd.a1 - r; box.a2 = nd.a2 - r;
        box.b0 = nd.a0 + r; box.b1 = nd.a1 + r; box.b2 = nd.a2 + r;
    } else if (type == 1) {
        box.a0 = -1e30f * 5; box.a1 = nd.b1 - tol; box.a2 = -1e30f * 5;
        box.b0 = 1e30f * 5; box.b1 = nd.b1 + tol; box.b2 = 1e30f * 5;
    } else if (type == 2) {
        box.a0 = nd.a0 - r; box.a1 = nd.a1 - nd.b2 / 2 - tol; box.a2 = nd.a2 - r;
        box.b0 = nd.a0 + r; box.b1 = nd.a1 + nd.b2 / 2 + tol; box.b2 = nd.a2 + r;
    } else {
        box.a0 = box.a1 = box.a2 = box.b0 = box.b1 = box.b2 = 0.f;
    }
}

__device__ __forceinline__ bool cert_inside_axis(float a, float b, float o, float d, float t) {
    const float s_a = a - o, s_b = b - o;
    const float P = t * d;
    const float T = __builtin_fmaf(__builtin_fabsf(P), -0x1p-21f, P);
    const float U = __builtin_fmaf(__builtin_fabsf(P), 0x1p-21f, P);
    return d == 0.0f || (s_a <= T && s_b >= U && __builtin_fabsf(P) >= 0x1p-100f);
}
__device__ __forceinline__ bool cert_inside(const Node& box, const RayK& ray, float t) {
    return cert_inside_axis(box.a0, box.b0, ray.o.x, ray.d.x, t) && cert_inside_axis(box.a1, box.b1, ray.o.y, ray.d.y, t) &&
           cert_inside_axis(box.a2, box.b2, ray.o.z, ray.d.z, t);
}

__device__ __forceinline__ bool sphere_cyl_test(const Node& nd, const RayK& ray, float& tmax, int& kind) {
    const bool sph = (nd.code & 3) == 0;
    const float r = nd.b0;
    bool ret = false;
    float lower = 0.f, upper = 0.f;
    if (!sph) {
        upper = nd.a1 + nd.b2 / 2;
        if (cap_test(nd.a0, nd.a2, nd.b1, ray, tmax, kind, upper)) ret = true;
        lower = nd.a1 - nd.b2 / 2;
        if (cap_test(nd.a0, nd.a2, nd.b1, ray, tmax, kind, lower)) ret = true;
    }
    const float cx = ray.o.x - nd.a0, cy = ray.o.y - nd.a1, cz = ray.o.z - nd.a2;
    const float dx = ray.d.x, dy = ray.d.y, dz = ray.d.z;
    const float bx = cx * dx, ax = dx * dx, qx = cx * cx;
    const float b = (sph ? bx + cy * dy : bx) + cz * dz;
    const float a = sph ? ray.aa : ray.ac;
    (void)ax;
    const float c = ((sph ? qx + cy * cy : qx) + cz * cz) - r * r;
    const float disc = b * b - a * c;
    if (!(disc > 0.f)) return ret;
    const double y = sph ? ray.ya : ray.yc;
    const float sq = __builtin_sqrtf(disc);
    float temp = qdiv(-b - sq, a, y);
    float hy = ray.o.y + temp * dy;
    if (temp < tmax && temp > ray.tmin && (sph || (hy > lower && hy < upper))) {
        tmax = temp;
        kind = sph ? HK_SPHERE_ROOT1 : HK_CYL_SIDE;
        return true;
    }
    temp = qdiv(-b + sq, a, y);
    hy = ray.o.y + temp * dy;
    if (temp < tmax && temp > ray.tmin && (sph || (hy > lower && hy < upper))) {
        tmax = temp;
        kind = sph ? HK_SPHERE_ROOT2 : HK_CYL_SIDE;
        return true;
    }
    return ret;
}

template <bool FAST, bool CONS, bool PRETEST = true>
__device__ __forceinline__ bool ranked_leaf_test(const Node& nd, const RayK& ray, float& tmax, int& kind, int& best_rank) {
    float tm = nd.miss < best_rank ? __int_as_float(__float_as_int(tmax) + 1) : tmax;
    if (CONS && PRETEST && (nd.code & 3) == 2) {
        Node box;
        leaf_aabb(nd, box);
        if (slab_reject<FAST, true>(box, ray, walk_limit(tm))) return false;
    }
    if (CONS && ((nd.code & 1) == 0)) {
        if (!sphere_cyl_test(nd, ray, tm, kind)) return false;
    } else if (!leaf_test(nd, ray, tm, kind)) {
        return false;
    }
    tmax = tm;
    best_rank = nd.miss;
    return true;
}

template <bool STATS, bool FAST, bool CONS = false, typename SRC>
__device__ __forceinline__ int trace(const SRC& nodes, int n_nodes, const RayK& ray, Hit& h, int& code_out,
                                     Counters& cnt) {
    float tmax = DEFAULT_RAY_TMAX;
    int best = -1, kind = 0;
    int best_rank = 0x7fffffff;
    int ni = 0;
    Node nd{};
    if (n_nodes > 0) nd = nodes(0);
    while (ni < n_nodes) {
        const bool leaf = nd.code >= 0;
        if (STATS) cnt.nodes++;
        bool take_a = false;
        if (leaf) {
            if (STATS) cnt.prims++;
            int k;
            if (ranked_leaf_test<FAST, CONS>(nd, ray, tmax, k, best_rank)) { best = ni; kind = k; }
        } else {
            take_a = CONS ? !slab_reject_octant(nd, ray, walk_limit(tmax)) : !slab_reject<FAST>(nd, ray, tmax);
        }
        ni = take_a || leaf ? ni + 1 : nd.miss;
        nd = nodes(ni);
    }
    if (best < 0) return 0;
    const Node w = nodes(best);
    if (CONS) {
        Node box;
        leaf_aabb(w, box);
        if (!cert_inside(box, ray, tmax) && slab_reject<FAST>(box, with_slab(ray), tmax)) return -1;
    }
    h = hit_attributes(w, ray, tmax, kind);
    code_out = w.code;
    return 1;
}


constexpr int WIDE_LANES = 256;

typedef __attribute__((address_space(3))) int16_t lds_i16;


struct WideNode {
    f2v e[3][2], x[3][2];
    int ref[4];
    uint32_t r01, r23;
};

template <typename QUAD>
__device__ __forceinline__ WideNode wide_node(const QUAD& quad, int sx, int sy, int sz) {
    WideNode n;
    const uint4 ex = quad(sx), xx = quad(1 - sx), ey = quad(2 + sy), xy = quad(3 - sy), ez = quad(4 + sz),
                xz = quad(5 - sz);
    const uint4 r = quad(6);
    auto lo = [](uint4 v) { return f2v{__uint_as_float(v.x), __uint_as_float(v.y)}; };
    auto hi = [](uint4 v) { return f2v{__uint_as_float(v.z), __uint_as_float(v.w)}; };
    n.e[0][0] = lo(ex); n.e[0][1] = hi(ex); n.x[0][0] = lo(xx); n.x[0][1] = hi(xx);
    n.e[1][0] = lo(ey); n.e[1][1] = hi(ey); n.x[1][0] = lo(xy); n.x[1][1] = hi(xy);
    n.e[2][0] = lo(ez); n.e[2][1] = hi(ez); n.x[2][0] = lo(xz); n.x[2][1] = hi(xz);
    n.ref[0] = (int)(int16_t)(r.x & 0xffffu); n.ref[1] = (int)(int16_t)(r.x >> 16);
    n.ref[2] = (int)(int16_t)(r.y & 0xffffu); n.ref[3] = (int)(int16_t)(r.y >> 16);
    n.r01 = r.x;
    n.r23 = r.y;
    return n;
}

template <bool HYB>
__device__ __forceinline__ WideNode load_wide_node(const uint4* tree, int n_lds, __amdgpu_buffer_rsrc_t rsrc,
                                                   uint32_t image_off, int cur, int sx, int sy, int sz) {
    if (!HYB || __builtin_expect(cur < n_lds, 1)) {
        typedef unsigned int v4u_t __attribute__((ext_vector_type(4)));
        typedef __attribute__((address_space(3))) const v4u_t lds_v4u;
        typedef __attribute__((address_space(3))) const uint4 lds_u4;
        uint32_t a;
        asm("v_mad_u32_u24 %0, %1, %2, %3" : "=v"(a) : "v"(cur), "s"(112u), "v"((uint32_t)(uintptr_t)(lds_u4*)tree));
        lds_v4u* const q = (lds_v4u*)(uintptr_t)a;
        return wide_node([&](int k) { const v4u_t v = q[k]; return make_uint4(v.x, v.y, v.z, v.w); }, sx, sy, sz);
    }
    const uint32_t off = image_off + (uint32_t)cur * 112u;
    return wide_node(
        [&](int k) {
            const v4u32 v = __builtin_amdgcn_raw_buffer_load_b128(rsrc, off + 16u * (uint32_t)k, 0, 0);
            return make_uint4(v.x, v.y, v.z, v.w);
        },
        sx, sy, sz);
}

__device__ __forceinline__ uint32_t wide_pair(const f2v e[3], const f2v x[3], const RayK& ray, float limit,
                                              float& lo_a, float& lo_b) {
    lo_a = __builtin_fmaxf(__builtin_fmaxf(__builtin_fmaf(e[0].x, ray.inx, ray.nx), __builtin_fmaf(e[1].x, ray.iny, ray.ny)),
                           __builtin_fmaf(e[2].x, ray.inz, ray.nz));
    lo_b = __builtin_fmaxf(__builtin_fmaxf(__builtin_fmaf(e[0].y, ray.inx, ray.nx), __builtin_fmaf(e[1].y, ray.iny, ray.ny)),
                           __builtin_fmaf(e[2].y, ray.inz, ray.nz));
    const float hi_a = __builtin_fminf(__builtin_fminf(__builtin_fmaf(x[0].x, ray.ifx, ray.fx), __builtin_fmaf(x[1].x, ray.ify, ray.fy)),
                                       __builtin_fmaf(x[2].x, ray.ifz, ray.fz));
    const float hi_b = __builtin_fminf(__builtin_fminf(__builtin_fmaf(x[0].y, ray.ifx, ray.fx), __builtin_fmaf(x[1].y, ray.ify, ray.fy)),
                                       __builtin_fmaf(x[2].y, ray.ifz, ray.fz));
    const bool pa = slab_pass(lo_a, hi_a, ray.t3, limit), pb = slab_pass(lo_b, hi_b, ray.t3, limit);
    return (pa ? 1u : 0u) | (pb ? 2u : 0u);
}

struct WalkState {
    lds_i16* top;
    int cur, parked, best, kind, best_rank;
    float tmax, limit;
    bool active;
};


template <bool STATS, int BLK, bool HYB>
__device__ __forceinline__ int trace_wide(const KParams& p, __amdgpu_buffer_rsrc_t rsrc, int oct, const RayK& ray,
                                          Hit& h, int& code_out, Counters& cnt, const uint4* tree, WalkState& ws,
                                          int suspend_at) {
    __shared__ int16_t wstack[CPT_WSTACK * BLK];
    lds_i16* const stk = (lds_i16*)wstack + threadIdx.x;
    constexpr int leaf0 = 0;
    auto leaf_of = [&](int ref) { return ~ref - 1; };
    const BufSrc leaf_src{rsrc, (uint32_t)wide_leaves_base(p) * (uint32_t)sizeof(Node)};
    auto leaf = [&](int i) -> Node { return leaf_src(i); };
    const int n_lds = lds_tree_nodes(p.n_wide);
    const uint32_t image_off = (uint32_t)wide_image_base(p) * (uint32_t)sizeof(Node);
    constexpr int NONE = -1;
    const uint64_t participants = __ballot(1);
    stamps::lap(6);
#ifdef CPT_POOLDIAG
    pooldiag::resumed(wave_count(__builtin_amdgcn_ballot_w64(ws.active)));
#endif
    if (!ws.active) {
        ws.tmax = DEFAULT_RAY_TMAX;
        ws.best = -1;
        ws.kind = 0;
        ws.best_rank = 0x7fffffff;
        for (int k = 0; k < p.n_unb; ++k) {
            if (STATS) cnt.prims++;
            const Node pl = leaf(leaf0 + k);
            int kk;
            if (ranked_leaf_test<true, true, false>(pl, ray, ws.tmax, kk, ws.best_rank)) {
                ws.best = leaf0 + k;
                ws.kind = kk;
            }
        }
        ws.limit = walk_limit(ws.tmax);
        ws.top = stk;
        ws.cur = 0;
        ws.parked = -1;
    }
    stamps::lap(7);
    float& tmax = ws.tmax;
    float& limit = ws.limit;
    int& best = ws.best;
    int& kind = ws.kind;
    int& best_rank = ws.best_rank;
    lds_i16*& top = ws.top;
    int& cur = ws.cur;
    int& parked = ws.parked;
    const int sx = oct & 1, sy = (oct >> 1) & 1, sz = oct >> 2;
    auto pop = [&]() -> int {
        if (top == stk) return NONE;
        top -= BLK;
        return (int)*top;
    };
    int it = 0;
    for (;;) {
        bool leaf_round = false;
        for (;; ++it) {
            stamps::count(9);
            if (cur >= 0) {
                execdiag::lanes(p.stats + 64, 1);
                if (STATS) {
                    cnt.nodes++;
                    cnt.gnodes += HYB && cur >= n_lds ? 1u : 0u;
                }
                const WideNode n = load_wide_node<HYB>(tree, n_lds, rsrc, image_off, cur, sx, sy, sz);
                const f2v e01[3] = {n.e[0][0], n.e[1][0], n.e[2][0]}, x01[3] = {n.x[0][0], n.x[1][0], n.x[2][0]};
                const f2v e23[3] = {n.e[0][1], n.e[1][1], n.e[2][1]}, x23[3] = {n.x[0][1], n.x[1][1], n.x[2][1]};
                float lo[4];
                const uint32_t m = wide_pair(e01, x01, ray, limit, lo[0], lo[1]) |
                                   (wide_pair(e23, x23, ray, limit, lo[2], lo[3]) << 2);
                int key = 0x7fffffff;
#pragma unroll
                for (int k = 0; k < 4; ++k) {
                    const int kk = (__float_as_int(lo[k]) & ~3) | k;
                    key = ((m >> k) & 1u) && kk < key ? kk : key;
                }
                const int bk = key & 3;
                const uint32_t pm = m & ~(1u << bk);
#pragma unroll
                for (int k = 3; k >= 0; --k) {
                    *top = (int16_t)n.ref[k];
                    top += __builtin_amdgcn_ubfe(pm, (uint32_t)k, 1u) * BLK;
                }
                const uint32_t word = (bk & 2) ? n.r23 : n.r01;
                cur = m == 0 ? pop() : (int)(int16_t)(word >> ((bk & 1) << 4));
                if (cur <= -2 && parked < 0) {
                    parked = leaf_of(cur);
                    cur = pop();
                }
            }
            const uint64_t has_parked = __builtin_amdgcn_ballot_w64(parked >= 0);
            const uint64_t w = has_parked | __builtin_amdgcn_ballot_w64(cur != NONE);
            const uint64_t stopped = has_parked & __builtin_amdgcn_ballot_w64(cur < 0);
            const uint32_t n_w = wave_count(w);
#ifdef CPT_POOLDIAG
            pooldiag::iteration(wave_count(participants & ~w), n_w);
#endif
            const bool tail = n_w <= 8u;
            stamps::lap(tail ? 11 : 1);
            if (tail) stamps::count(13);
            if (!w) break;
            if (n_w <= (uint32_t)suspend_at && wave_count(participants & ~w) >= (uint32_t)SUSPEND_MIN_DONE && it > 0)
                break;
            if (wave_count(stopped) * 64u >= (uint32_t)SPEC_LEAF_ROUND * n_w) {
                leaf_round = true;
                ++it;
                break;
            }
        }
        if (!leaf_round) break;
        if (parked >= 0) {
            stamps::count(10);
            execdiag::lanes(p.stats + 64, 2);
            if (STATS) cnt.prims++;
            const Node lf = leaf(parked);
            int k;
            if (ranked_leaf_test<true, true, false>(lf, ray, tmax, k, best_rank)) {
                best = parked;
                kind = k;
                limit = walk_limit(tmax);
            }
            parked = -1;
            if (cur <= -2) {
                parked = leaf_of(cur);
                cur = pop();
            }
        }
        stamps::lap(2);
    }
    const bool working = parked >= 0 || cur != NONE;
#ifdef CPT_POOLDIAG
    pooldiag::suspended(wave_count(__builtin_amdgcn_ballot_w64(working)));
#endif
    ws.active = working;
    if (working) return 2;
    if (best < 0) return 0;
    execdiag::lanes(p.stats + 64, 3);
    const Node wn = leaf(best);
    Node box;
    leaf_aabb(wn, box);
    if (!cert_inside(box, ray, tmax) && slab_reject<true>(box, with_slab(ray), tmax)) return -1;
    h = hit_attributes(wn, ray, tmax, kind);
    code_out = wn.code;
    return 1;
}

template <bool STATS, bool FAST, bool CONS = false>
__device__ __forceinline__ int trace_any(__amdgpu_buffer_rsrc_t rsrc, uint32_t base, int n, const RayK& ray, Hit& h,
                                         int& code, Counters& cnt) {
    return trace<STATS, FAST, CONS>(BufSrc{rsrc, base}, n, ray, h, code, cnt);
}

template <bool STATS, int BLK = WIDE_LANES, bool LDST = false, bool HYB = true>
__device__ __forceinline__ int trace_segment(const KParams& p, const RayK& rk, bool finite, Hit& h, int& code,
                                             Counters& cnt, const uint4* tree, WalkState& ws, int suspend_at) {
    const __amdgpu_buffer_rsrc_t rsrc = node_rsrc(p);
    if (p.ordered && __builtin_expect(finite, 1)) {
        int n, r = -1;
        bool wide = false;
        if constexpr (LDST) {
            if (p.ordered == 1 && p.n_wide > 0) {
                const int oct = (rk.d.x < 0.f ? 1 : 0) | (rk.d.y < 0.f ? 2 : 0) | (rk.d.z < 0.f ? 4 : 0);
                r = trace_wide<STATS, BLK, HYB>(p, rsrc, oct, rk, h, code, cnt, tree, ws, suspend_at);
                wide = true;
            }
        }
        if (!wide) {
            const uint32_t base = walk_order(p, rk.d, n) * (uint32_t)sizeof(Node);
            r = trace_any<STATS, true, true>(rsrc, base, n, rk, h, code, cnt);
        }
        if (__builtin_expect(r >= 0, 1)) return r;
        if (STATS) cnt.fallbacks++;
    }
    const RayK rs = with_slab(rk);
    if (__builtin_expect(finite, 1)) return trace_any<STATS, true>(rsrc, 0u, p.n_nodes, rs, h, code, cnt) > 0 ? 1 : 0;
    return trace_any<STATS, false>(rsrc, 0u, p.n_nodes, rs, h, code, cnt) > 0 ? 1 : 0;
}

template <bool STATS, int BLK = WIDE_LANES, bool LDST = false>
__device__ __forceinline__ bool trace_segment(const KParams& p, const RayK& rk, bool finite, Hit& h, int& code,
                                              Counters& cnt, const uint4* tree = nullptr) {
    WalkState ws;
    ws.active = false;
    return trace_segment<STATS, BLK, LDST>(p, rk, finite, h, code, cnt, tree, ws, 0) == 1;
}

struct Shade { v3 radiance, attenuation, bounce; };

__device__ __forceinline__ v3 to_world(v3 a, v3 N) {
    v3 B, C;
    if (__builtin_fabsf(N.x) > __builtin_fabsf(N.y)) {
        float invLen = rcp_f(sqrt_nn(N.x * N.x + N.z * N.z));
        C = mk(N.z * invLen, 0.0f, -N.x * invLen);
    } else {
        float invLen = rcp_f(sqrt_nn(N.y * N.y + N.z * N.z));
        C = mk(0.f, N.z * invLen, -N.y * invLen);
    }
    B = cross(C, N);
    return (a.x * B + a.y * C) + a.z * N;
}

__device__ __forceinline__ v3 lobe(float x_1, float x_2, double inv_alpha) {
    float z = lobe_pow(x_1, inv_alpha);
    float r = sqrt_nn(1.0f - z * z);
    float phi = (float)(2 * REF_PI * (double)x_2);
    float sp, cp;
    lobe_sincos(phi, &sp, &cp);
    return mk(r * cp, r * sp, z);
}

__device__ __forceinline__ float schlick(float cosine, float r0) {
    return r0 + (1 - r0) * dm::pow5f(1 - cosine);
}

__device__ __forceinline__ bool refract(v3 v, v3 n, float ni_over_nt, v3& refracted) {
    v3 uv = normalize_u(v);
    float dt = dot(uv, n);
    float discriminant = (float)(1.0 - (double)(ni_over_nt * ni_over_nt * (1 - dt * dt)));
    if (discriminant > 0) {
        refracted = normalize_u(ni_over_nt * (uv - n * dt) - n * sqrt_nn(discriminant));
        return true;
    }
    return false;
}

__device__ inline void eval_material(const Mat& m, v3 normal, v3 in_dir, Xorwow& rng, Shade& out,
                                     unsigned long long* diag = nullptr) {
    const v3 kd = mk(m.att_x, m.att_y, m.att_z);
    const v3 zero = mk(0.0f, 0.0f, 0.0f);
    const int type = (m.type >= 1 && m.type <= 3) ? m.type : 0;
    const float x_1 = uniform(rng), x_2 = uniform(rng);
    double ia = type == 0 ? 1.0 / 2 : m.inv_alpha;
    v3 axis = normal;
    if (type == 1) {
        axis = reflect(in_dir, normal);
    } else if (type == 2) {
        if (diag) execdiag::lanes(diag, 15);
        if (uniform(rng) < m.reflectivity) axis = reflect(in_dir, normal);
        else ia = 1.0 / 2.0;
    } else if (type == 3) {
        if (diag) execdiag::lanes(diag, 5);
        v3 outward, refracted = mk1(0.0f);
        float ni_over_nt, reflect_prob, cosine;
        const v3 in = normalize_u(in_dir);
        if (dot(in, normal) > 0) {
            outward = -normal;
            ni_over_nt = m.ior;
            cosine = dot(in, normal);
            cosine = sqrt_nn(1 - m.ior * m.ior * (1 - cosine * cosine));
        } else {
            outward = normal;
            ni_over_nt = m.inv_ior;
            cosine = -dot(in, normal);
        }
        if (refract(in, outward, ni_over_nt, refracted)) reflect_prob = schlick(cosine, m.schlick_r0);
        else reflect_prob = 1.0f;
        axis = uniform(rng) < reflect_prob ? reflect(in, normal) : refracted;
    }
    const v3 local = lobe(x_1, x_2, ia);
    out.bounce = to_world(local, axis);
    const float c = dot(normal, out.bounce);
    const bool keep = type == 3 || (type == 2 ? !(c < 0) : c > 0.0f);
    out.attenuation = mk(keep ? kd.x : zero.x, keep ? kd.y : zero.y, keep ? kd.z : zero.z);
    out.radiance = mk(m.rad_x, m.rad_y, m.rad_z);
}

__device__ __forceinline__ v3 miss_radiance(const KParams& p, v3 dir) {
    v3 d = normalize_u(dir);
    float v = (float)(dm::div_pi(miss_asinf(d.z)) + 0.5);
    float u = (float)dm::div_pi(miss_atanf(d.y / d.x) / 2);
    return tex2d(p, u, v);
}

__device__ __forceinline__ Ray ray_gen(const CamK& c, int x, int y, Xorwow& rng) {
    float r1 = uniform(rng), r2 = uniform(rng), r3 = uniform(rng);
    v3 rd = c.lens_radius * mk(r1, r2, r3);
    v3 u = mk(c.u[0], c.u[1], c.u[2]), v = mk(c.v[0], c.v[1], c.v[2]);
    v3 origin = mk(c.origin[0], c.origin[1], c.origin[2]);
    v3 offset = u * rd.x + v * rd.y;
    float dx = x > 0 ? qdiv_raw(float(x), c.inv_w) : 0.f;
    float dy = y > 0 ? qdiv_raw(float(y), c.inv_h) : 0.f;
    Ray ray;
    ray.o = origin + offset;
    v3 tl = mk(c.top_left[0], c.top_left[1], c.top_left[2]);
    v3 hz = mk(c.horizontal[0], c.horizontal[1], c.horizontal[2]);
    v3 vt = mk(c.vertical[0], c.vertical[1], c.vertical[2]);
    ray.d = normalize((((tl + dx * hz) + dy * vt) - origin) - offset);
    ray.tmin = 0.f;
    ray.tmax = DEFAULT_RAY_TMAX;
    return ray;
}
__device__ __forceinline__ Ray ray_gen(const KParams& p, int x, int y, Xorwow& rng) { return ray_gen(p.cam, x, y, rng); }

__device__ __forceinline__ const KParams& kernarg_params() {
    typedef __attribute__((address_space(4))) const KParams kparams4;
    kparams4* base = (kparams4*)__builtin_amdgcn_kernarg_segment_ptr();
    asm volatile("" : "+s"(base));
    return *(const KParams*)base;
}
template <typename T>
__device__ __forceinline__ T kernarg_field(size_t offset) {
    typedef __attribute__((address_space(4))) const char kchar;
    kchar* base = (kchar*)__builtin_amdgcn_kernarg_segment_ptr();
    asm volatile("" : "+s"(base));
    return *(const T*)(base + offset);
}

__device__ __forceinline__ uint64_t wave_sum(uint32_t v) {
    uint64_t s = v;
#pragma unroll
    for (int off = 32; off > 0; off >>= 1) s += __shfl_xor(s, off, 64);
    return s;
}

}
```

cpppathtracer_amd/csrc/cpt_scene.cpp:

```cpp
#include <hip/hip_runtime.h>

#include <algorithm>
#include <atomic>
#include <chrono>
#include <cfloat>
#include <cmath>
#include <cstdarg>
#include <cstdio>
#include <cstring>
#include <mutex>
#include <new>
#include <string>
#include <vector>

#include "cpt_context.hpp"

using namespace cpt::host;
using namespace cpt::ctx;

namespace cpt {
namespace ctx {

static Mat to_mat(const cpt_material& m) {
    Mat g;
    std::memset(&g, 0, sizeof(g));
    g.att_x = m.u.kd.x; g.att_y = m.u.kd.y; g.att_z = m.u.kd.z;
    g.type = m.type;
    g.rad_x = m.emit_intensity;
    g.ior = m.refractive_index;
    g.reflectivity = m.reflectivity;
    g.smoothness = m.smoothness;
    g.inv_alpha = 0.0;
    return g;
}

int material_slot(cpt_ctx* c, const cpt_material& m) {
    Mat g = to_mat(m);
    const int tex = m.have_tex ? 1 : 0;
    for (size_t i = 0; i < c->mats_h.size(); ++i)
        if (std::memcmp(&c->mats_h[i], &g, sizeof(Mat)) == 0 && c->mat_have_tex[i] == tex &&
            (!tex || c->mat_tex[i] == m.u.tex))
            return (int)i;
    c->mats_h.push_back(g);
    c->mat_have_tex.push_back(tex);
    c->mat_tex.push_back(tex ? m.u.tex : 0);
    return (int)c->mats_h.size() - 1;
}

static void compact_materials(cpt_ctx* c) {
    std::vector<int> remap(c->mats_h.size(), -1);
    for (int m : c->mat_of_obj) remap[m] = 0;
    std::vector<Mat> mats;
    std::vector<int> have;
    std::vector<uint64_t> tex;
    for (size_t i = 0; i < remap.size(); ++i) {
        if (remap[i] < 0) continue;
        remap[i] = (int)mats.size();
        mats.push_back(c->mats_h[i]);
        have.push_back(c->mat_have_tex[i]);
        tex.push_back(c->mat_tex[i]);
    }
    for (int& m : c->mat_of_obj) m = remap[m];
    c->mats_h.swap(mats);
    c->mat_have_tex.swap(have);
    c->mat_tex.swap(tex);
}

static int build_walk_tree(const cpt_ctx* c, HostBvh& w, std::vector<int>& unbounded, std::vector<int>& rank);

static void build_refit_plan(cpt_ctx* c, const HostBvh& w, const std::vector<int> (&pos)[8], const std::vector<int>& slot_of,
                             const std::vector<int>& leaf_of);

void linearise_all(cpt_ctx* c) {
    c->lin.clear();
    c->n_walk = 0;
    c->n_wide = 0;
    c->n_unb = 0;
    c->refit_plan.clear();
    c->lin.reserve(9 * c->bvh.nodes.size());
    linearise(c->bvh, c->objs, c->mat_of_obj, c->lin, c->pos_of_node, -1, nullptr);
    c->n_bvh = (int)c->lin.size();
    if (c->n_bvh == 0) return;
    HostBvh w;
    std::vector<int> unbounded, rank, pos[8];
    const int root = build_walk_tree(c, w, unbounded, rank);
    for (int o = 0; o < 8; ++o) linearise(w, c->objs, c->mat_of_obj, c->lin, pos[o], o, &rank, root, unbounded);
    c->n_walk = (int)(c->lin.size() - c->n_bvh) / 8;
    c->n_unb = (int)unbounded.size();
    c->n_leaves = 0;
    std::vector<int> slot_of(w.nodes.size(), -1), leaf_of(w.nodes.size(), -1);
    if (root >= 0 && !w.nodes[root].is_object)
        c->n_wide = linearise_wide(w, root, pos[0], c->n_bvh, c->n_unb, c->lin, &c->n_leaves, slot_of, leaf_of);
    build_refit_plan(c, w, pos, slot_of, leaf_of);
}

void build_refit_plan(cpt_ctx* c, const HostBvh& w, const std::vector<int> (&pos)[8], const std::vector<int>& slot_of,
                      const std::vector<int>& leaf_of) {
    const int nr = (int)c->bvh.nodes.size(), nw = (int)w.nodes.size();
    c->refit_n_ref = nr;
    c->refit_plan.assign(nr + nw, cpt::RefitNode{});
    c->refit_parent.assign(nr + nw, -1);
    c->refit_height.assign(nr + nw, 0);
    c->refit_boxes.assign(nr + nw, cpt::Box6{});
    c->refit_walk_leaf.assign(c->objs.size(), -1);
    c->refit_mark.assign(nr + nw, 0);
    for (int i = 0; i < nr + nw; ++i) {
        const bool ref = i < nr;
        const BNode& n = ref ? c->bvh.nodes[i] : w.nodes[i - nr];
        cpt::RefitNode& r = c->refit_plan[i];
        const int off = ref ? 0 : nr;
        r.left = n.is_object ? -1 : n.left + off;
        r.right = n.is_object ? -1 : n.right + off;
        r.slot = ref ? -1 : slot_of[i - nr];
        r.leaf = ref || c->n_wide == 0 ? -1 : leaf_of[i - nr];
        for (int o = 0; o < 8; ++o) r.pos[o] = -1;
        if (ref) r.pos[0] = c->pos_of_node[i];
        else
            for (int o = 0; o < 8; ++o)
                r.pos[o] = pos[o][i - nr] < 0 ? -1 : c->n_bvh + o * c->n_walk + pos[o][i - nr];
        c->refit_boxes[i] = cpt::Box6{{n.bmin.x, n.bmin.y, n.bmin.z}, {n.bmax.x, n.bmax.y, n.bmax.z}};
        if (!n.is_object) {
            c->refit_parent[r.left] = i;
            c->refit_parent[r.right] = i;
        } else if (!ref) {
            c->refit_walk_leaf[n.obj] = i;
        }
    }
    for (int i = nr + nw - 1; i >= 0; --i) {
        const cpt::RefitNode& r = c->refit_plan[i];
        if (r.left >= 0)
            c->refit_height[i] = 1 + std::max(c->refit_height[r.left], c->refit_height[r.right]);
    }
}

int build_walk_tree(const cpt_ctx* c, HostBvh& w, std::vector<int>& unbounded, std::vector<int>& rank) {
    const std::vector<cpt_object>& O = c->objs;
    w.nodes.clear();
    w.leaf_of_object.assign(O.size(), -1);
    unbounded.clear();
    std::vector<int> idx;
    std::vector<std::pair<int, int>> flat;
    for (size_t o = 0; o < O.size(); ++o) {
        const int ref_rank = c->pos_of_node[c->bvh.leaf_of_object[o]];
        if (O[o].type == CPT_PRIM_PLATFORM) flat.emplace_back(ref_rank, (int)o);
        else idx.push_back((int)o);
    }
    std::sort(flat.begin(), flat.end());
    for (const auto& f : flat) unbounded.push_back(sah::leaf(w, O, f.second));
    const int root = idx.empty() ? -1 : sah::build(w, O, idx, 0, (int)idx.size());
    rank.assign(w.nodes.size(), -1);
    for (size_t i = 0; i < w.nodes.size(); ++i)
        if (w.nodes[i].is_object) rank[i] = c->pos_of_node[c->bvh.leaf_of_object[w.nodes[i].obj]];
    return root;
}

int upload_scene(cpt_ctx* c) {
    if (c->lin.size() * sizeof(Node) > (size_t)INT32_MAX)
        return fail(c, CPT_ERR_UNSUPPORTED, "scene too large: %zu BVH nodes in all orders (max %zu)", c->lin.size(),
                    (size_t)INT32_MAX / sizeof(Node));
    HIP_TRY(c, hipSetDevice(c->device));
    int rc;
    if ((rc = c->d_nodes.ensure(c, std::max<size_t>(1, c->lin.size()))) != CPT_OK) return rc;
    hipStream_t s = c->stream();
    if (!c->lin.empty())
        HIP_TRY(c, hipMemcpyAsync(c->d_nodes, c->lin.data(), c->lin.size() * sizeof(Node), hipMemcpyHostToDevice, s));
    if (!c->refit_plan.empty()) {
        if ((rc = c->d_refit_plan.ensure(c, c->refit_plan.size())) != CPT_OK) return rc;
        if ((rc = c->d_refit_boxes.ensure(c, c->refit_boxes.size())) != CPT_OK) return rc;
        HIP_TRY(c, hipMemcpyAsync(c->d_refit_plan, c->refit_plan.data(), c->refit_plan.size() * sizeof(cpt::RefitNode),
                                  hipMemcpyHostToDevice, s));
        HIP_TRY(c, hipMemcpyAsync(c->d_refit_boxes, c->refit_boxes.data(), c->refit_boxes.size() * sizeof(cpt::Box6),
                                  hipMemcpyHostToDevice, s));
    }
    if ((rc = upload_materials(c)) != CPT_OK) return rc;
    HIP_TRY(c, hipStreamSynchronize(s));
    c->scene_set = true;
    return CPT_OK;
}

int upload_materials(cpt_ctx* c) {
    int rc;
    hipStream_t s = c->stream();
    if (c->d_mats && c->d_mats.capacity() < c->mats_h.size()) {
        HIP_TRY(c, hipStreamSynchronize(s));
    }
    if ((rc = c->d_mats.ensure(c, std::max<size_t>(1, c->mats_h.size()))) != CPT_OK) return rc;
    if (!c->mats_h.empty()) {
        std::vector<int32_t> tex_of_mat(c->mats_h.size(), -1);
        bool any = false;
        for (size_t i = 0; i < c->mats_h.size(); ++i) {
            if (!c->mat_have_tex[i]) continue;
            for (size_t t = 0; t < c->textures.size(); ++t)
                if (c->textures[t].handle == c->mat_tex[i]) tex_of_mat[i] = (int32_t)t;
            if (tex_of_mat[i] < 0)
                return fail(c, CPT_ERR_INVALID_ARG, "textured material uses handle %llu, which is not bound (cpt_bind_texture)",
                            (unsigned long long)c->mat_tex[i]);
            any = true;
        }
        if (any) {
            std::vector<TexDesc> descs(c->textures.size());
            for (size_t t = 0; t < descs.size(); ++t) {
                const auto& x = c->textures[t];
                descs[t] = TexDesc{x.d_texels.get(), x.w, x.h, x.cols, x.addr, x.filter, 0};
            }
            if ((rc = c->d_texdescs.ensure(c, descs.size())) != CPT_OK) return rc;
            if ((rc = c->d_tex_of_mat.ensure(c, tex_of_mat.size())) != CPT_OK) return rc;
            HIP_TRY(c, hipMemcpyAsync(c->d_texdescs, descs.data(), descs.size() * sizeof(TexDesc), hipMemcpyHostToDevice, s));
            HIP_TRY(c, hipMemcpyAsync(c->d_tex_of_mat, tex_of_mat.data(), tex_of_mat.size() * sizeof(int32_t),
                                      hipMemcpyHostToDevice, s));
            HIP_TRY(c, hipStreamSynchronize(s));
        }
        HIP_TRY(c, hipMemcpyAsync(c->d_mats, c->mats_h.data(), c->mats_h.size() * sizeof(Mat), hipMemcpyHostToDevice, s));
        HIP_TRY(c, cpt::launch_prepare_materials(c->d_mats, any ? c->d_tex_of_mat : nullptr, any ? c->d_texdescs : nullptr,
                                                 (int)c->mats_h.size(), s));
    }
    return CPT_OK;
}

int device_refit(cpt_ctx* c, int n, const int* indices, bool mats_changed) {
    std::vector<int> uniq(indices, indices + n);
    std::sort(uniq.begin(), uniq.end());
    uniq.erase(std::unique(uniq.begin(), uniq.end()), uniq.end());
    const int nr = c->refit_n_ref;
    std::vector<cpt::RefitLeaf> recs(uniq.size());
    std::vector<int32_t> dirty;
    std::vector<uint8_t>& mark = c->refit_mark;
    mark.resize(c->refit_plan.size(), 0);
    for (size_t k = 0; k < uniq.size(); ++k) {
        const int o = uniq[k];
        cpt::RefitLeaf& r = recs[k];
        r.ref_id = c->bvh.leaf_of_object[o];
        r.walk_id = c->refit_walk_leaf[o];
        r.prim = make_node(c->bvh.nodes[r.ref_id], c->objs, c->mat_of_obj);
        const F3 lo = aabb_min(c->objs[o]), hi = aabb_max(c->objs[o]);
        r.box = cpt::Box6{{lo.x, lo.y, lo.z}, {hi.x, hi.y, hi.z}};
        for (int id : {r.ref_id, r.walk_id})
            for (int p = id < 0 ? -1 : c->refit_parent[id]; p >= 0 && !mark[p]; p = c->refit_parent[p]) {
                mark[p] = 1;
                dirty.push_back(p);
            }
    }
    for (int32_t d : dirty) mark[d] = 0;
    std::stable_sort(dirty.begin(), dirty.end(),
                     [&](int32_t a, int32_t b) { return c->refit_height[a] < c->refit_height[b]; });
    std::vector<int32_t> level_end;
    for (size_t i = 0; i < dirty.size(); ++i)
        if (i + 1 == dirty.size() || c->refit_height[dirty[i + 1]] != c->refit_height[dirty[i]])
            level_end.push_back((int32_t)(i + 1));
    const size_t rec_bytes = recs.size() * sizeof(cpt::RefitLeaf);
    std::vector<uint8_t> work(rec_bytes + dirty.size() * sizeof(int32_t));
    std::memcpy(work.data(), recs.data(), rec_bytes);
    if (!dirty.empty()) std::memcpy(work.data() + rec_bytes, dirty.data(), dirty.size() * sizeof(int32_t));
    HIP_TRY(c, hipSetDevice(c->device));
    int rc;
    if ((rc = c->d_refit_work.ensure(c, work.size())) != CPT_OK) return rc;
    uint8_t* const d_work = c->d_refit_work;
    hipStream_t s = c->stream();
    HIP_TRY(c, hipMemcpyAsync(d_work, work.data(), work.size(), hipMemcpyHostToDevice, s));
    const size_t image_base = (size_t)c->n_bvh + 8 * (size_t)c->n_walk;
    uint32_t* image = c->n_wide > 0 ? reinterpret_cast<uint32_t*>(c->d_nodes + image_base) : nullptr;
    Node* leaves = c->n_wide > 0 ? c->d_nodes + image_base + ((size_t)c->n_wide * 7 + 1) / 2 : nullptr;
    HIP_TRY(c, cpt::launch_refit(reinterpret_cast<const cpt::RefitLeaf*>(d_work), (int)recs.size(),
                                 reinterpret_cast<const int32_t*>(d_work + rec_bytes), level_end.data(),
                                 (int)level_end.size(), nr, c->d_refit_plan, c->d_refit_boxes, c->d_nodes, image, leaves,
                                 s));
    if (mats_changed && (rc = upload_materials(c)) != CPT_OK) return rc;
    return sync_checked(c);
}

}
}

extern "C" {

int cpt_set_scene(cpt_ctx* c, const cpt_object* objs, int n) {
    if (!c || n < 0 || (n > 0 && !objs)) return c ? fail(c, CPT_ERR_INVALID_ARG, "cpt_set_scene: bad arguments") : CPT_ERR_INVALID_ARG;
    c->scene_set = false;
    try {
        c->objs.assign(objs, objs + n);
        build_host_bvh(c->bvh, c->objs);
        c->mats_h.clear();
        c->mat_have_tex.clear();
        c->mat_tex.clear();
        c->mat_of_obj.assign(n, 0);
        for (int i = 0; i < n; ++i) c->mat_of_obj[i] = material_slot(c, c->objs[i].material);
        linearise_all(c);
    } catch (const std::bad_alloc&) {
        return fail(c, CPT_ERR_OUT_OF_MEMORY, "cpt_set_scene: host allocation failed");
    }
    return upload_scene(c);
}

static int update_objects(cpt_ctx* c, int n, const int* indices, const cpt_object* objs, bool rebuild) {
    if (!c || n < 0 || (n > 0 && (!indices || !objs))) return CPT_ERR_INVALID_ARG;
    if (!c->scene_set) return fail(c, CPT_ERR_STATE, "cpt_update_objects: cpt_set_scene first");
    for (int k = 0; k < n; ++k)
        if (indices[k] < 0 || indices[k] >= (int)c->objs.size())
            return fail(c, CPT_ERR_INVALID_ARG, "cpt_update_objects: index %d out of range", indices[k]);
    if (n == 0) return CPT_OK;
    const auto t0 = std::chrono::steady_clock::now();
    for (int k = 0; k < n && !rebuild; ++k)
        if ((c->objs[indices[k]].type == CPT_PRIM_PLATFORM) != (objs[k].type == CPT_PRIM_PLATFORM)) rebuild = true;
    if (c->refit_plan.empty()) rebuild = true;
    const size_t n_mats = c->mats_h.size();
    for (int k = 0; k < n; ++k) {
        const int index = indices[k];
        c->objs[index] = objs[k];
        c->mat_of_obj[index] = material_slot(c, objs[k].material);
        int ni = c->bvh.leaf_of_object[index];
        while (ni != -1) {
            BNode& nd = c->bvh.nodes[ni];
            if (nd.is_object) {
                nd.bmax = aabb_max(c->objs[nd.obj]);
                nd.bmin = aabb_min(c->objs[nd.obj]);
            } else {
                const BNode& L = c->bvh.nodes[nd.left];
                const BNode& R = c->bvh.nodes[nd.right];
                nd.bmax = F3{MAX_(L.bmax.x, R.bmax.x), MAX_(L.bmax.y, R.bmax.y), MAX_(L.bmax.z, R.bmax.z)};
                nd.bmin = F3{MIN_(L.bmin.x, R.bmin.x), MIN_(L.bmin.y, R.bmin.y), MIN_(L.bmin.z, R.bmin.z)};
            }
            ni = nd.parent;
        }
    }
    if (c->mats_h.size() > n_mats) {
        std::vector<char> used(c->mats_h.size(), 0);
        size_t n_used = 0;
        for (int m : c->mat_of_obj)
            if (!used[m]) { used[m] = 1; ++n_used; }
        if (c->mats_h.size() > 2 * n_used + 16) {
            compact_materials(c);
            rebuild = true;
        }
    }
    int rc;
    if (rebuild) {
        linearise_all(c);
        rc = upload_scene(c);
    } else {
        rc = device_refit(c, n, indices, c->mats_h.size() != n_mats);
    }
    c->last_update_ms = std::chrono::duration<float, std::milli>(std::chrono::steady_clock::now() - t0).count();
    return rc;
}

int cpt_update_objects(cpt_ctx* c, int n, const int* indices, const cpt_object* objs) {
    return update_objects(c, n, indices, objs, false);
}

int cpt_update_objects_rebuild(cpt_ctx* c, int n, const int* indices, const cpt_object* objs) {
    return update_objects(c, n, indices, objs, true);
}

int cpt_get_material_count(cpt_ctx* c, int* n) {
    if (!c || !n) return CPT_ERR_INVALID_ARG;
    *n = (int)c->mats_h.size();
    return CPT_OK;
}

int cpt_last_update_ms(cpt_ctx* c, float* ms) {
    if (!c || !ms) return CPT_ERR_INVALID_ARG;
    *ms = c->last_update_ms;
    return CPT_OK;
}

int cpt_update_object(cpt_ctx* c, int index, const cpt_object* obj) {
    if (!c || !obj) return CPT_ERR_INVALID_ARG;
    return cpt_update_objects(c, 1, &index, obj);
}

int cpt_scene_bvh_export(cpt_ctx* c, float* boxes, int32_t* links, int capacity, int* n_nodes) {
    if (!c || !n_nodes) return CPT_ERR_INVALID_ARG;
    int m = (int)c->bvh.nodes.size();
    *n_nodes = m;
    for (int i = 0; i < m && i < capacity; ++i) {
        const BNode& n = c->bvh.nodes[i];
        if (boxes) {
            float* b = boxes + 6 * i;
            b[0] = n.bmin.x; b[1] = n.bmin.y; b[2] = n.bmin.z; b[3] = n.bmax.x; b[4] = n.bmax.y; b[5] = n.bmax.z;
        }
        if (links) {
            int32_t* l = links + 4 * i;
            l[0] = n.is_object; l[1] = n.left; l[2] = n.right; l[3] = n.obj;
        }
    }
    return CPT_OK;
}

int cpt_bvh_build_host(const cpt_object* objs, int n, float* boxes, int32_t* links, int capacity, int* n_nodes) {
    if (n < 0 || (n > 0 && !objs) || !n_nodes) return CPT_ERR_INVALID_ARG;
    try {
        std::vector<cpt_object> v(objs, objs + n);
        HostBvh b;
        build_host_bvh(b, v);
        int m = (int)b.nodes.size();
        *n_nodes = m;
        for (int i = 0; i < m && i < capacity; ++i) {
            const BNode& nd = b.nodes[i];
            if (boxes) {
                float* x = boxes + 6 * i;
                x[0] = nd.bmin.x; x[1] = nd.bmin.y; x[2] = nd.bmin.z; x[3] = nd.bmax.x; x[4] = nd.bmax.y; x[5] = nd.bmax.z;
            }
            if (links) {
                int32_t* l = links + 4 * i;
                l[0] = nd.is_object; l[1] = nd.left; l[2] = nd.right; l[3] = nd.obj;
            }
        }
    } catch (const std::bad_alloc&) {
        return CPT_ERR_OUT_OF_MEMORY;
    }
    return CPT_OK;
}

int cpt_set_env_texture(cpt_ctx* c, const uint8_t* rgba, int logical_width, int height, int valid_cols) {
    if (!c) return CPT_ERR_INVALID_ARG;
    if (logical_width <= 0 || height <= 0 || valid_cols < 0 || valid_cols > logical_width || (valid_cols > 0 && !rgba))
        return fail(c, CPT_ERR_INVALID_ARG, "cpt_set_env_texture: bad geometry %dx%d cols %d", logical_width, height, valid_cols);
    HIP_TRY(c, hipSetDevice(c->device));
    size_t n = (size_t)valid_cols * height;
    int rc = c->d_env.ensure(c, std::max<size_t>(1, n));
    if (rc != CPT_OK) return rc;
    if (n) HIP_TRY(c, hipMemcpy(c->d_env, rgba, n * 4, hipMemcpyHostToDevice));
    c->env_w = logical_width;
    c->env_h = height;
    c->env_cols = valid_cols;
    return CPT_OK;
}

int cpt_bind_texture(cpt_ctx* c, uint64_t handle, const uint8_t* rgba, int logical_width, int height, int valid_cols,
                     int address_mode, int filter_mode) {
    if (!c) return CPT_ERR_INVALID_ARG;
    if (logical_width <= 0 || height <= 0 || valid_cols < 0 || valid_cols > logical_width || (valid_cols > 0 && !rgba) ||
        address_mode < CPT_ADDRESS_WRAP || address_mode > CPT_ADDRESS_BORDER || filter_mode < CPT_FILTER_POINT ||
        filter_mode > CPT_FILTER_LINEAR)
        return fail(c, CPT_ERR_INVALID_ARG, "cpt_bind_texture: bad geometry %dx%d cols %d or mode %d/%d", logical_width,
                    height, valid_cols, address_mode, filter_mode);
    HIP_TRY(c, hipSetDevice(c->device));
    const size_t n = (size_t)valid_cols * height;
    DevBuf<uint32_t> d;
    if (int rc = d.ensure(c, std::max<size_t>(1, n))) return rc;
    if (n) {
        hipError_t e = hipMemcpy(d, rgba, n * 4, hipMemcpyHostToDevice);
        if (e != hipSuccess) return fail(c, CPT_ERR_HIP, "cpt_bind_texture: %s", hipGetErrorString(e));
    }
    cpt_ctx::Texture t{handle, std::move(d), logical_width, height, valid_cols, address_mode, filter_mode};
    cpt_ctx::Texture* slot = nullptr;
    for (auto& x : c->textures)
        if (x.handle == handle) slot = &x;
    if (slot) *slot = std::move(t);
    else c->textures.push_back(std::move(t));
    return c->scene_set ? upload_scene(c) : CPT_OK;
}

}
```

cpppathtracer_amd/csrc/cpt_tuning.hpp:

```cpp
#pragma once

namespace cpt {

constexpr int LDS_BLOCK = 1024;
constexpr int WAVES_PER_SIMD = 3;
constexpr int SUSPEND_AT = 8;
constexpr int SUSPEND_MIN_DONE = 40;
constexpr int SPEC_LEAF_ROUND = 28;
constexpr int DEFER_MISS_ROUND = 40;
constexpr bool STATIC_FIRST = true;
constexpr int TAKE_BATCH = 64;
constexpr int TAKE_TAPER = 4;
constexpr int CONS_RETIRE_PER_LEVEL = 256;
#ifndef CPT_FILTER_LDS_MAX_STEP
#define CPT_FILTER_LDS_MAX_STEP 2
#endif
constexpr int FILTER_LDS_MAX_STEP = CPT_FILTER_LDS_MAX_STEP;

}
```

cpppathtracer_amd/csrc/cpt_wavefront.hip:

```cpp
#include <hip/hip_runtime.h>
#include <stdint.h>

#include <algorithm>

#include "cpt_path.hpp"

namespace cpt {


__device__ __forceinline__ uint32_t wave_append(bool alive, uint32_t* counter) {
    const uint64_t m = __ballot(alive);
    if (m == 0) return 0;
    const int leader = __ffsll((unsigned long long)m) - 1;
    uint32_t base = 0;
    if ((int)(threadIdx.x & 63) == leader) base = atomicAdd(counter, (uint32_t)__popcll(m));
    base = __shfl(base, leader);
    return base + lane_rank(m);
}

__device__ __forceinline__ void load_rng(const KParams& p, size_t npix, size_t pix, Xorwow& s) {
    s.v0 = p.rng[pix];
    s.v1 = p.rng[npix + pix];
    s.v2 = p.rng[2 * npix + pix];
    s.v3 = p.rng[3 * npix + pix];
    s.v4 = p.rng[4 * npix + pix];
    s.d = p.rng[5 * npix + pix];
}

__device__ __forceinline__ void load_rng_slot(const WfState& w, int b, uint32_t i, Xorwow& s) {
    const uint4 a = w.rng_a[b][i];
    const uint2 c = w.rng_b[b][i];
    s.v0 = a.x; s.v1 = a.y; s.v2 = a.z; s.v3 = a.w;
    s.v4 = c.x; s.d = c.y;
}

__device__ __forceinline__ void store_rng_slot(const WfState& w, int b, uint32_t i, const Xorwow& s) {
    w.rng_a[b][i] = make_uint4(s.v0, s.v1, s.v2, s.v3);
    w.rng_b[b][i] = make_uint2(s.v4, s.d);
}

__device__ __forceinline__ void store_rng(const KParams& p, size_t npix, size_t pix, const Xorwow& s) {
    p.rng[pix] = s.v0;
    p.rng[npix + pix] = s.v1;
    p.rng[2 * npix + pix] = s.v2;
    p.rng[3 * npix + pix] = s.v3;
    p.rng[4 * npix + pix] = s.v4;
    p.rng[5 * npix + pix] = s.d;
}

template <bool AUX>
__global__ void __launch_bounds__(256) k_wf_raygen(const KParams p, WfState w) {
    const size_t npix = (size_t)p.n_rows * p.width;
    const size_t stride = (size_t)gridDim.x * blockDim.x;
    for (size_t i = (size_t)blockIdx.x * blockDim.x + threadIdx.x; i < npix; i += stride) {
        const size_t pix = (size_t)w.ident[i];
        const int x = (int)(pix % p.width), ri = (int)(pix / p.width);
        Xorwow s;
        load_rng(p, npix, pix, s);
        const Ray ray = ray_gen(p, x, p.rows[ri], s);
        if (p.max_depth == 0) {
            store_rng(p, npix, pix, s);
            float4 a = p.accum[pix];
            p.accum[pix] = make_float4(a.x + 0.f, a.y + 0.f, a.z + 0.f, a.w + 1.0f);
            if (AUX) {
                p.normal[3 * pix] = 0.f;
                p.normal[3 * pix + 1] = 0.f;
                p.normal[3 * pix + 2] = 0.f;
                p.depth[pix] = 0.f;
            }
            continue;
        }
        w.ray_o[0][i] = make_float4(ray.o.x, ray.o.y, ray.o.z, ray.tmin);
        w.ray_d[0][i] = make_float4(ray.d.x, ray.d.y, ray.d.z, __uint_as_float(0u));
        w.att[0][i] = make_float4(1.f, 1.f, 1.f, __uint_as_float(1u));
        w.rad[0][i] = make_float4(0.f, 0.f, 0.f, 0.f);
        if (AUX) w.aux[0][i] = make_float4(0.f, 0.f, 0.f, 0.f);
        store_rng_slot(w, 0, (uint32_t)i, s);
    }
}

constexpr int WF_LDS_BLOCK = 1024;
template <bool LDST> constexpr int wf_extend_block() { return LDST ? WF_LDS_BLOCK : 256; }

template <bool STATS, bool LDST>
__global__ void __launch_bounds__(wf_extend_block<LDST>()) k_wf_extend(const KParams p, WfState w,
                                                                       const uint32_t* __restrict__ nin,
                                                                       const int sb) {
    constexpr int BLK = wf_extend_block<LDST>();
    const uint32_t n = *nin;
    __shared__ uint4 s_tree[LDST ? LDS_TREE_NODES * 7 : 1];
    if (LDST) {
        if ((uint32_t)blockIdx.x * BLK >= n) return;
        const uint4* src = reinterpret_cast<const uint4*>(p.nodes + wide_image_base(p));
        for (int i = threadIdx.x; i < 7 * lds_tree_nodes(p.n_wide); i += BLK) s_tree[i] = src[i];
        __syncthreads();
    }
    Counters cnt{};
    const uint32_t stride = gridDim.x * blockDim.x;
    for (uint32_t i = blockIdx.x * blockDim.x + threadIdx.x; i < n; i += stride) {
        const float4 o = w.ray_o[sb][i], d = w.ray_d[sb][i];
        Ray ray;
        ray.o = mk(o.x, o.y, o.z);
        ray.d = mk(d.x, d.y, d.z);
        ray.tmin = o.w;
        ray.tmax = DEFAULT_RAY_TMAX;
        const RayK rk = make_rayk(ray);
        const bool finite = !(ray.o.x != ray.o.x || ray.o.y != ray.o.y || ray.o.z != ray.o.z || ray.d.x != ray.d.x ||
                              ray.d.y != ray.d.y || ray.d.z != ray.d.z);
        Hit h;
        int code = -1;
        if (STATS) cnt.segments++;
        bool hit;
        if (LDST) hit = trace_segment<STATS, BLK, true>(p, rk, finite, h, code, cnt, s_tree);
        else hit = trace_segment<STATS>(p, rk, finite, h, code, cnt);
        w.hit_p[i] = make_float4(h.pos.x, h.pos.y, h.pos.z, __int_as_float(hit ? code : -1));
        if (hit) w.hit_n[i] = make_float4(h.normal.x, h.normal.y, h.normal.z, 0.f);
    }
    if (STATS) {
        const uint64_t a = wave_sum(cnt.segments), b = wave_sum(cnt.nodes), c = wave_sum(cnt.prims);
        if ((threadIdx.x & 63) == 0) {
            atomicAdd((unsigned long long*)&p.stats[0], (unsigned long long)a);
            atomicAdd((unsigned long long*)&p.stats[1], (unsigned long long)b);
            atomicAdd((unsigned long long*)&p.stats[2], (unsigned long long)c);
        }
        const uint64_t f = wave_sum(cnt.fallbacks);
        if ((threadIdx.x & 63) == 0 && f) atomicAdd((unsigned long long*)&p.stats[5], (unsigned long long)f);
        const uint64_t g = wave_sum(cnt.gnodes);
        if ((threadIdx.x & 63) == 0 && g) atomicAdd((unsigned long long*)&p.stats[6], (unsigned long long)g);
    }
}

template <bool STATS, bool AUX>
__global__ void __launch_bounds__(256) k_wf_shade(const KParams p, WfState w, const int32_t* __restrict__ qin,
                                                 const uint32_t* __restrict__ nin, int32_t* __restrict__ qout,
                                                 uint32_t* __restrict__ nout, const int sb) {
    const uint32_t n = *nin;
    const size_t npix = (size_t)p.n_rows * p.width;
    const uint32_t max_depth = (uint32_t)p.max_depth;
    uint32_t hits = 0, misses = 0;
    const uint32_t stride = gridDim.x * blockDim.x;
    const uint32_t trips = (n + stride - 1) / stride;
    __shared__ uint32_t s_cnt[3][4];
    __shared__ uint32_t s_slot[256];
    __shared__ uint32_t s_app[5];
    const int lane = threadIdx.x & 63, wv = threadIdx.x >> 6;
    for (uint32_t t = 0, i0 = blockIdx.x * blockDim.x + threadIdx.x; t < trips; ++t, i0 += stride) {
        const int key = i0 < n ? (__float_as_int(w.hit_p[i0].w) >= 0 ? 1 : 0) : 2;
        uint64_t mk_[3];
        for (int k = 0; k < 3; ++k) mk_[k] = __ballot(key == k);
        if (lane == 0)
            for (int k = 0; k < 3; ++k) s_cnt[k][wv] = (uint32_t)__popcll(mk_[k]);
        __syncthreads();
        uint32_t pos = 0;
        for (int k = 0; k < 3; ++k)
            for (int v = 0; v < 4; ++v)
                if (k < key || (k == key && v < wv)) pos += s_cnt[k][v];
        const uint64_t mine = mk_[key];
        pos += lane_rank(mine);
        s_slot[pos] = i0;
        __syncthreads();
        const uint32_t i = s_slot[threadIdx.x];
        bool alive = false;
        int pix = 0;
        float4 no4, nd4, na4, nr4, nx4;
        Xorwow s;
        if (i < n) {
            pix = qin[i];
            load_rng_slot(w, sb, i, s);
            const float4 o4 = w.ray_o[sb][i], d4 = w.ray_d[sb][i], a4 = w.att[sb][i], r4 = w.rad[sb][i];
            const float4 hp = w.hit_p[i];
            v3 dir = mk(d4.x, d4.y, d4.z);
            v3 att = mk(a4.x, a4.y, a4.z), rad = mk(r4.x, r4.y, r4.z);
            uint32_t depth = __float_as_uint(d4.w);
            const bool first = __float_as_uint(a4.w) != 0u;
            const int code = __float_as_int(hp.w);
            Shade sh;
            v3 attr_normal;
            v3 org = mk(o4.x, o4.y, o4.z);
            if (code >= 0) {
                hits++;
                const float4 hn = w.hit_n[i];
                const v3 normal = mk(hn.x, hn.y, hn.z);
                const Mat m = p.mats[code >> 2];
                eval_material(m, normal, dir, s, sh);
                attr_normal = normal;
                org = mk(hp.x, hp.y, hp.z);
            } else {
                misses++;
                sh.radiance = miss_radiance(p, dir);
                sh.attenuation = mk1(0.f);
                sh.bounce = dir;
                attr_normal = -dir;
                depth = MAX_RECURSION_DEPTH_SET;
            }
            rad = rad + att * sh.radiance;
            att = att * sh.attenuation;
            float4 aux4 = make_float4(0.f, 0.f, 0.f, 0.f);
            if (AUX) {
                aux4 = w.aux[sb][i];
                if (first) {
                    const v3 nn = mk(aux4.x, aux4.y, aux4.z) + attr_normal;
                    aux4 = make_float4(nn.x, nn.y, nn.z, aux4.w + DEFAULT_RAY_TMAX);
                }
            }
            dir = normalize(sh.bounce);
            depth++;
            if (!(depth < max_depth)) {
                const float4 a = p.accum[pix];
                p.accum[pix] = make_float4(a.x + rad.x, a.y + rad.y, a.z + rad.z, a.w + 1.0f);
                if (AUX) {
                    p.normal[3 * (size_t)pix] = aux4.x;
                    p.normal[3 * (size_t)pix + 1] = aux4.y;
                    p.normal[3 * (size_t)pix + 2] = aux4.z;
                    p.depth[pix] = aux4.w;
                }
                store_rng(p, npix, pix, s);
            } else {
                alive = true;
                no4 = make_float4(org.x, org.y, org.z, BOUNCE_RAY_TMIN);
                nd4 = make_float4(dir.x, dir.y, dir.z, __uint_as_float(depth));
                na4 = make_float4(att.x, att.y, att.z, __uint_as_float(0u));
                nr4 = make_float4(rad.x, rad.y, rad.z, 0.f);
                nx4 = aux4;
            }
        }
        const uint64_t am = __ballot(alive);
        if (lane == 0) s_app[wv] = (uint32_t)__popcll(am);
        __syncthreads();
        if (threadIdx.x == 0) {
            const uint32_t tot = s_app[0] + s_app[1] + s_app[2] + s_app[3];
            s_app[4] = tot ? atomicAdd(nout, tot) : 0u;
        }
        __syncthreads();
        uint32_t slot = s_app[4];
        for (int v = 0; v < wv; ++v) slot += s_app[v];
        slot += lane_rank(am);
        if (alive) {
            const int ob = sb ^ 1;
            qout[slot] = pix;
            w.ray_o[ob][slot] = no4;
            w.ray_d[ob][slot] = nd4;
            w.att[ob][slot] = na4;
            w.rad[ob][slot] = nr4;
            if (AUX) w.aux[ob][slot] = nx4;
            store_rng_slot(w, ob, slot, s);
        }
    }
    if (STATS) {
        const uint64_t a = wave_sum(hits), b = wave_sum(misses);
        if ((threadIdx.x & 63) == 0) {
            atomicAdd((unsigned long long*)&p.stats[3], (unsigned long long)a);
            atomicAdd((unsigned long long*)&p.stats[4], (unsigned long long)b);
        }
    }
}

__global__ void k_wf_ident(int width, int n_rows, int32_t* q, uint32_t* count) {
    const TileGrid grid{width, n_rows};
    const uint32_t n_work = (uint32_t)grid.count() * 64u;
    for (uint32_t id = blockIdx.x * blockDim.x + threadIdx.x; id < n_work; id += gridDim.x * blockDim.x) {
        int x, ri;
        const bool valid = grid.pixel(id >> 6, id & 63, x, ri);
        const uint32_t slot = wave_append(valid, count);
        if (valid) q[slot] = ri * width + x;
    }
}

static int persistent_grid(const void* fn, int block, size_t items) {
    static int cus = 0;
    if (cus == 0) {
        int dev = 0;
        (void)hipGetDevice(&dev);
        (void)hipDeviceGetAttribute(&cus, hipDeviceAttributeMultiprocessorCount, dev);
        if (cus <= 0) cus = 256;
    }
    int per_cu = 0;
    if (hipOccupancyMaxActiveBlocksPerMultiprocessor(&per_cu, fn, block, 0) != hipSuccess || per_cu < 1) per_cu = 1;
    const long long want = (long long)((items + block - 1) / block);
    return (int)std::max<long long>(1, std::min<long long>(want, (long long)per_cu * cus));
}

hipError_t wavefront_build_ident(const KParams& p, WfState& w, hipStream_t stream) {
    hipError_t e = hipMemsetAsync(w.counts + 3, 0, sizeof(uint32_t), stream);
    if (e != hipSuccess) return e;
    const size_t npix = (size_t)p.n_rows * p.width;
    hipLaunchKernelGGL(k_wf_ident, dim3((unsigned)std::min<size_t>(4096, (npix + 255) / 256 + 1)), dim3(256), 0, stream,
                       p.width, p.n_rows, w.ident, w.counts + 3);
    return hipGetLastError();
}

template <bool S, bool A, bool T>
static hipError_t wf_render_t(const KParams& p, WfState& w, hipStream_t stream, int* launches) {
    const size_t npix = (size_t)p.n_rows * p.width;
    constexpr int eb = wf_extend_block<T>();
    const int gr = persistent_grid((const void*)k_wf_raygen<A>, 256, npix);
    const int ge = persistent_grid((const void*)k_wf_extend<S, T>, eb, npix);
    const int gs = persistent_grid((const void*)k_wf_shade<S, A>, 256, npix);
    hipError_t e = hipSuccess;
    int n = 0;
    for (int pass = 0; pass < p.spp && e == hipSuccess; ++pass) {
        hipLaunchKernelGGL(k_wf_raygen<A>, dim3(gr), dim3(256), 0, stream, p, w);
        ++n;
        const int32_t* cur = w.ident;
        const uint32_t* cur_n = w.counts + 3;
        for (int b = 0; b < p.max_depth; ++b) {
            int32_t* nxt = w.queue[b & 1];
            uint32_t* nxt_n = w.counts + (b & 1);
            e = hipMemsetAsync(nxt_n, 0, sizeof(uint32_t), stream);
            if (e != hipSuccess) break;
            hipLaunchKernelGGL((k_wf_extend<S, T>), dim3(ge), dim3(eb), 0, stream, p, w, cur_n, b & 1);
            hipLaunchKernelGGL((k_wf_shade<S, A>), dim3(gs), dim3(256), 0, stream, p, w, cur, cur_n, nxt, nxt_n, b & 1);
            n += 2;
            cur = nxt;
            cur_n = nxt_n;
        }
        if (e == hipSuccess) e = hipGetLastError();
    }
    if (launches) *launches = n;
    return e;
}

template <bool T>
static hipError_t wf_render_any(const KParams& p, WfState& w, bool stats, bool aux, hipStream_t stream, int* launches) {
    if (stats && aux) return wf_render_t<true, true, T>(p, w, stream, launches);
    if (stats) return wf_render_t<true, false, T>(p, w, stream, launches);
    if (aux) return wf_render_t<false, true, T>(p, w, stream, launches);
    return wf_render_t<false, false, T>(p, w, stream, launches);
}

hipError_t launch_wavefront(const KParams& p, WfState& w, bool stats, bool aux, hipStream_t stream, int* launches) {
    if (p.width <= 0 || p.n_rows <= 0) return hipSuccess;
    const bool lds = p.ordered == 1 && p.n_wide > 0;
    return lds ? wf_render_any<true>(p, w, stats, aux, stream, launches)
               : wf_render_any<false>(p, w, stats, aux, stream, launches);
}

}
```

cpppathtracer_amd/renderer.py:

```python
import ctypes

import numpy as np

from . import _lib
from ._lib import (CPT_PATH_WAVEFRONT, CPT_RENDER_ACCUMULATE, CPT_RENDER_AUX, CPT_RENDER_STATS, CPT_RENDER_SYNC,
                   CPT_SCHEDULE_CONSOLIDATE, CPT_SCHEDULE_COST, CPT_SCHEDULE_NO_CONSOLIDATE, CPT_SCHEDULE_PREVIOUS,
                   CPT_TRAVERSAL_ORDERED,
                   CPT_TRAVERSAL_PLAIN_LEAVES, CptError, check)

PATHS = ("megakernel", "wavefront")
from .tiling import tile_grid
from .types import CAMERA_DTYPE, OBJECT_DTYPE


def _p(a):
    return ctypes.c_void_p(a.ctypes.data) if a is not None else None


def device_count() -> int:
    L = _lib.load()
    n = ctypes.c_int(0)
    check(L.cpt_get_device_count(ctypes.byref(n)))
    return n.value


def camera_get_copy(cam):
    L = _lib.load()
    c = np.array(cam, dtype=CAMERA_DTYPE, copy=True)
    check(L.cpt_camera_get_copy(_p(c)))
    return c


class Renderer:
    def __init__(self, device: int = 0):
        self._L = _lib.load()
        h = ctypes.c_void_p()
        st = self._L.cpt_create(device, ctypes.byref(h))
        if st != 0:
            raise CptError(st, (self._L.cpt_last_error(None) or b"").decode())
        self._ctx = h
        self.device = device
        self.width = self.height = self.n_rows = 0
        self.rows = None

    def close(self):
        if getattr(self, "_ctx", None):
            self._L.cpt_destroy(self._ctx)
            self._ctx = None

    def __del__(self):
        try:
            self.close()
        except Exception:
            pass

    def __enter__(self):
        return self

    def __exit__(self, *exc):
        self.close()

    def _check(self, st):
        return check(st, self._ctx)

    def set_stream(self, hip_stream_handle):
        self._check(self._L.cpt_set_stream(self._ctx, ctypes.c_void_p(hip_stream_handle or 0)))

    def set_scene(self, objs):
        objs = np.ascontiguousarray(objs, dtype=OBJECT_DTYPE)
        self._check(self._L.cpt_set_scene(self._ctx, _p(objs) if len(objs) else None, len(objs)))

    def update_object(self, index, obj):
        o = np.array(obj, dtype=OBJECT_DTYPE, copy=True)
        self._check(self._L.cpt_update_object(self._ctx, index, _p(o)))

    def update_objects(self, indices, objs, rebuild=False):
        idx = np.ascontiguousarray(indices, dtype=np.int32)
        o = np.ascontiguousarray(objs, dtype=OBJECT_DTYPE)
        if o.shape != idx.shape:
            raise ValueError(f"update_objects: {o.shape[0] if o.ndim else 1} objects for {idx.size} indices")
        fn = self._L.cpt_update_objects_rebuild if rebuild else self._L.cpt_update_objects
        self._check(fn(self._ctx, int(idx.size), _p(idx), _p(o)))

    def material_count(self) -> int:
        n = ctypes.c_int(0)
        self._check(self._L.cpt_get_material_count(self._ctx, ctypes.byref(n)))
        return n.value

    def last_update_ms(self) -> float:
        ms = ctypes.c_float(0)
        self._check(self._L.cpt_last_update_ms(self._ctx, ctypes.byref(ms)))
        return float(ms.value)

    def bvh_export(self):
        n = ctypes.c_int(0)
        self._check(self._L.cpt_scene_bvh_export(self._ctx, None, None, 0, ctypes.byref(n)))
        m = n.value
        boxes = np.zeros((max(m, 1), 6), dtype=np.float32)
        links = np.zeros((max(m, 1), 4), dtype=np.int32)
        self._check(self._L.cpt_scene_bvh_export(self._ctx, _p(boxes), _p(links), m, ctypes.byref(n)))
        return boxes[:m], links[:m]

    def set_env(self, env):
        if env is None:
            self._check(self._L.cpt_set_env_texture(self._ctx, None, 1, 1, 0))
            return
        rgba = np.ascontiguousarray(env.rgba, dtype=np.uint8)
        self._check(self._L.cpt_set_env_texture(self._ctx, _p(rgba), env.width, env.height, env.valid_cols))

    def bind_texture(self, handle, tex, address_mode=2, filter_mode=1):
        rgba = np.ascontiguousarray(tex.rgba, dtype=np.uint8)
        self._check(self._L.cpt_bind_texture(self._ctx, handle, _p(rgba), tex.width, tex.height, tex.valid_cols,
                                             address_mode, filter_mode))

    def set_frame(self, width, height, rows=None):
        if rows is None:
            self._check(self._L.cpt_set_frame(self._ctx, width, height, None, 0))
            self.rows = np.arange(height, dtype=np.int32)
        else:
            r = np.ascontiguousarray(rows, dtype=np.int32)
            self._check(self._L.cpt_set_frame(self._ctx, width, height, _p(r), r.size))
            self.rows = r
        self.width, self.height, self.n_rows = width, height, int(self.rows.size)

    def init_rng(self, seed):
        self._check(self._L.cpt_init_rng(self._ctx, ctypes.c_uint64(seed)))

    def render(self, cam, spp, max_depth, accumulate=False, aux=False, stats=False, sync=False, flags=0,
               path="megakernel", ordered=False, schedule="tiles", consolidate=None):
        if path not in PATHS:
            raise ValueError(f"path must be one of {PATHS}")
        if schedule not in ("tiles", "cost", "previous"):
            raise ValueError("schedule must be 'tiles', 'cost' or 'previous'")
        c = np.ascontiguousarray(np.array(cam, dtype=CAMERA_DTYPE))
        f = flags | (CPT_PATH_WAVEFRONT if path == "wavefront" else 0)
        f |= CPT_TRAVERSAL_ORDERED if ordered else 0
        f |= CPT_TRAVERSAL_PLAIN_LEAVES if ordered == "plain" else 0
        f |= CPT_RENDER_ACCUMULATE if accumulate else 0
        f |= CPT_RENDER_AUX if aux else 0
        f |= CPT_RENDER_STATS if stats else 0
        f |= CPT_RENDER_SYNC if sync else 0
        f |= CPT_SCHEDULE_COST if schedule == "cost" else 0
        f |= CPT_SCHEDULE_PREVIOUS if schedule == "previous" else 0
        if consolidate is not None:
            f |= CPT_SCHEDULE_CONSOLIDATE if consolidate else CPT_SCHEDULE_NO_CONSOLIDATE
        self._check(self._L.cpt_render(self._ctx, _p(c), spp, max_depth, f))

    def render_adaptive(self, cam, min_spp, max_spp, batch, rel_error, max_depth, flags=0):
        c = np.ascontiguousarray(np.array(cam, dtype=CAMERA_DTYPE))
        self._check(self._L.cpt_render_adaptive(self._ctx, _p(c), int(min_spp), int(max_spp), int(batch),
                                                ctypes.c_float(rel_error), int(max_depth), int(flags)))
        return self.adaptive_info()

    def adaptive_info(self):
        rounds, passes = ctypes.c_int(0), ctypes.c_uint64(0)
        self._check(self._L.cpt_adaptive_info(self._ctx, ctypes.byref(rounds), None, 0, ctypes.byref(passes)))
        active = np.zeros(max(1, rounds.value), dtype=np.uint32)
        self._check(self._L.cpt_adaptive_info(self._ctx, ctypes.byref(rounds), _p(active), active.size,
                                              ctypes.byref(passes)))
        return {"rounds": rounds.value, "active_tiles": active[:rounds.value].copy(), "passes_done": int(passes.value)}

    def adaptive_begin(self, cam, min_spp, max_spp, batch, rel_error, max_depth, flags=0):
        c = np.ascontiguousarray(np.array(cam, dtype=CAMERA_DTYPE))
        self._check(self._L.cpt_adaptive_begin(self._ctx, _p(c), int(min_spp), int(max_spp), int(batch),
                                               ctypes.c_float(rel_error), int(max_depth), int(flags)))

    def adaptive_step(self) -> int:
        active = ctypes.c_int(0)
        self._check(self._L.cpt_adaptive_step(self._ctx, ctypes.byref(active)))
        return active.value

    def read_noise(self):
        out = np.zeros(self.npix, dtype=np.float32)
        self._check(self._L.cpt_read_noise(self._ctx, _p(out), out.size))
        return out

    def read_moments(self):
        out = np.zeros((4, self.npix), dtype=np.float32)
        self._check(self._L.cpt_read_moments(self._ctx, _p(out), out.size))
        return out

    def write_moments(self, planar4):
        a = np.ascontiguousarray(planar4, dtype=np.float32)
        if a.shape != (4, self.npix):
            raise ValueError(f"write_moments: expected shape (4, {self.npix}), got {a.shape}")
        self._check(self._L.cpt_write_moments(self._ctx, _p(a), a.size))

    def filter_frame(self, levels=5, sigma_l=1.0, normal_sharpness_log2=7):
        self._check(self._L.cpt_filter_frame(self._ctx, int(levels), ctypes.c_float(sigma_l), int(normal_sharpness_log2)))

    def read_filtered(self):
        rgb = np.zeros((self.npix, 3), dtype=np.float32)
        var = np.zeros(self.npix, dtype=np.float32)
        self._check(self._L.cpt_read_filtered(self._ctx, _p(rgb), _p(var), self.npix))
        return rgb, var

    def last_filter_ms(self) -> float:
        ms = ctypes.c_float(0)
        self._check(self._L.cpt_last_filter_ms(self._ctx, ctypes.byref(ms)))
        return float(ms.value)

    def tile_costs(self, cam, passes, max_depth, ordered=True):
        c = np.ascontiguousarray(np.array(cam, dtype=CAMERA_DTYPE))
        ty, tx = tile_grid(self.width, self.n_rows)
        out = np.zeros((ty, tx), dtype=np.uint32)
        f = CPT_TRAVERSAL_ORDERED if ordered else 0
        f |= CPT_TRAVERSAL_PLAIN_LEAVES if ordered == "plain" else 0
        self._check(self._L.cpt_tile_costs(self._ctx, _p(c), int(passes), int(max_depth), f, _p(out), out.size))
        return out

    def synchronize(self):
        self._check(self._L.cpt_synchronize(self._ctx))

    def last_render_ms(self) -> float:
        ms = ctypes.c_float(0)
        self._check(self._L.cpt_last_render_ms(self._ctx, ctypes.byref(ms)))
        return float(ms.value)

    def last_kernel_stats(self):
        ms, n = ctypes.c_float(0), ctypes.c_int(0)
        self._check(self._L.cpt_last_kernel_stats(self._ctx, ctypes.byref(ms), ctypes.byref(n)))
        return float(ms.value), int(n.value)

    @property
    def npix(self):
        return self.n_rows * self.width

    def read_accum(self):
        out = np.zeros((self.npix, 4), dtype=np.float32)
        self._check(self._L.cpt_read_accum(self._ctx, _p(out)))
        return out

    def clear_accum(self):
        self._check(self._L.cpt_clear_accum(self._ctx))

    def read_rng(self):
        out = np.zeros((6, self.npix), dtype=np.uint32)
        self._check(self._L.cpt_read_rng(self._ctx, _p(out)))
        return out

    def write_rng(self, planar6):
        a = np.ascontiguousarray(planar6, dtype=np.uint32)
        if a.shape != (6, self.npix):
            raise ValueError(f"write_rng: expected shape (6, {self.npix}), got {a.shape}")
        self._check(self._L.cpt_write_rng(self._ctx, _p(a)))

    def read_aux(self):
        n = np.zeros((self.npix, 3), dtype=np.float32)
        d = np.zeros(self.npix, dtype=np.float32)
        self._check(self._L.cpt_read_aux(self._ctx, _p(n), _p(d)))
        return n, d

    def write_accum(self, rgba):
        a = np.ascontiguousarray(rgba, dtype=np.float32).reshape(self.npix, 4)
        self._check(self._L.cpt_write_accum(self._ctx, _p(a)))

    def write_aux(self, normal3, depth):
        n = np.ascontiguousarray(normal3, dtype=np.float32).reshape(self.npix, 3)
        d = np.ascontiguousarray(depth, dtype=np.float32).reshape(self.npix)
        self._check(self._L.cpt_write_aux(self._ctx, _p(n), _p(d)))

    def copy_accum_device(self, device_ptr, nbytes, stream):
        self._check(self._L.cpt_copy_accum_device(self._ctx, ctypes.c_void_p(device_ptr), nbytes,
                                                  ctypes.c_void_p(stream or None)))

    def gather_rows(self, src):
        self._check(self._L.cpt_gather_rows(self._ctx, src._ctx))

    GATHER_MODES = {-1: None, 0: "same_device", 1: "peer", 2: "staged"}

    def last_gather_mode(self, src):
        m = ctypes.c_int(-1)
        self._check(self._L.cpt_last_gather_mode(self._ctx, src._ctx, ctypes.byref(m)))
        return self.GATHER_MODES[m.value]

    def set_debug_gather(self, force_staged):
        self._check(self._L.cpt_set_debug_gather(self._ctx, int(bool(force_staged))))

    def stats(self):
        s = (ctypes.c_uint64 * 5)()
        self._check(self._L.cpt_get_stats(self._ctx, s))
        return dict(zip(("segments", "nodes", "prims", "hits", "misses"), (int(x) for x in s)))

    def raw_counters(self):
        out = np.zeros(8, dtype=np.uint64)
        self._check(self._L.cpt_get_raw_counters(self._ctx, _p(out)))
        return [int(x) for x in out]

    def debug_timeline(self):
        out = np.zeros(4 * 4096 + 4, dtype=np.uint64)
        self._check(self._L.cpt_debug_timeline(self._ctx, _p(out), out.size))
        return out[: 4 * 4096].reshape(4096, 4), int(out[4 * 4096])

    def diag_counters(self):
        out = np.zeros(16, dtype=np.uint64)
        self._check(self._L.cpt_get_diag_counters(self._ctx, _p(out)))
        return [int(x) for x in out]

    def execdiag_counters(self):
        out = np.zeros(64, dtype=np.uint64)
        self._check(self._L.cpt_get_execdiag_counters(self._ctx, _p(out)))
        return out.reshape(4, 16)

    def walk_info(self):
        out = np.zeros(4, dtype=np.int32)
        self._check(self._L.cpt_get_walk_info(self._ctx, _p(out)))
        return dict(zip(("n_bvh", "n_walk", "n_wide", "n_unb"), (int(x) for x in out)))

    def read_nodes(self):
        n = ctypes.c_size_t(0)
        self._check(self._L.cpt_debug_read_nodes(self._ctx, None, 0, ctypes.byref(n)))
        out = np.zeros(n.value, dtype=np.uint8)
        if n.value:
            self._check(self._L.cpt_debug_read_nodes(self._ctx, _p(out), out.size, ctypes.byref(n)))
        return out

    def debug_tile_order(self, which):
        ty, tx = tile_grid(self.width, self.n_rows)
        out = np.zeros(max(1, ty * tx), dtype=np.uint32)
        n = ctypes.c_size_t(0)
        self._check(self._L.cpt_debug_read_tile_order(self._ctx, int(which), _p(out), ty * tx, ctypes.byref(n)))
        return out[:n.value].copy()

    def measure_read_pattern(self, bytes_per_lane, nbytes=1 << 30, iters=1):
        out = ctypes.c_float(0.0)
        self._check(self._L.cpt_measure_read_pattern(self._ctx, int(bytes_per_lane), int(nbytes), int(iters),
                                                     ctypes.byref(out)))
        return out.value

    def measure_read_bandwidth(self, nbytes=4 << 30, iters=10):
        out = ctypes.c_float(0.0)
        self._check(self._L.cpt_measure_read_bandwidth(self._ctx, int(nbytes), int(iters), ctypes.byref(out)))
        return float(out.value)

    def set_debug_consolidation(self, flags=0, keeper_spin_log2=0, publish_wait_log2=0):
        self._check(self._L.cpt_set_debug_consolidation(self._ctx, flags, keeper_spin_log2, publish_wait_log2))

    def set_debug_grid(self, max_workgroups=0, lanes_per_wave=0):
        self._check(self._L.cpt_set_debug_grid(self._ctx, int(max_workgroups), int(lanes_per_wave)))

    def reset_stats(self):
        self._check(self._L.cpt_reset_stats(self._ctx))

    def selftest_qdiv(self, which, n, seed=1, examples=16):
        out = np.zeros(examples + 1, dtype=np.uint64)
        self._check(self._L.cpt_selftest_qdiv(self._ctx, which, n, seed, _p(out), out.size))
        cnt = int(out[0])
        pairs = [(np.uint32(int(v) >> 32).view(np.float32), np.uint32(int(v) & 0xFFFFFFFF).view(np.float32))
                 for v in out[1:1 + min(cnt, examples)]]
        return cnt, pairs

    def denoise_mix(self, cur_sample_idx, out=None, host=True):
        if not host:
            self._check(self._L.cpt_denoise_mix(self._ctx, cur_sample_idx, None))
            return None
        if out is None:
            out = np.zeros((self.height, self.width, 4), dtype=np.uint8)
        if not isinstance(out, np.ndarray) or out.dtype != np.uint8:
            raise ValueError("denoise_mix: `out` must be a numpy uint8 array")
        if out.size != self.height * self.width * 4:
            raise ValueError(f"denoise_mix: `out` holds {out.size} bytes, the frame needs "
                             f"{self.height * self.width * 4}")
        if not out.flags["C_CONTIGUOUS"] or not out.flags["WRITEABLE"]:
            raise ValueError("denoise_mix: `out` must be C-contiguous and writeable")
        self._check(self._L.cpt_denoise_mix(self._ctx, cur_sample_idx, _p(out)))
        return out

    def display_band(self):
        y0, y1 = ctypes.c_int(0), ctypes.c_int(0)
        self._check(self._L.cpt_display_band(self._ctx, ctypes.byref(y0), ctypes.byref(y1)))
        return y0.value, y1.value

    def read_mix(self):
        y0, y1 = self.display_band()
        out = np.zeros(((y1 - y0) * self.width, 3), dtype=np.float32)
        self._check(self._L.cpt_read_mix(self._ctx, _p(out), out.size))
        return out

    def last_display_ms(self) -> float:
        ms = ctypes.c_float()
        self._check(self._L.cpt_last_display_ms(self._ctx, ctypes.byref(ms)))
        return ms.value

    def denoise_mix_band(self, cur_sample_idx, y0, y1, host=True):
        out = np.zeros((y1 - y0, self.width, 4), dtype=np.uint8) if host else None
        self._check(self._L.cpt_denoise_mix_band(self._ctx, cur_sample_idx, int(y0), int(y1),
                                                 _p(out) if host else None))
        return out

    def copy_bgra_device(self, device_ptr, nbytes, stream):
        self._check(self._L.cpt_copy_bgra_device(self._ctx, ctypes.c_void_p(device_ptr), nbytes,
                                                 ctypes.c_void_p(stream or None)))

    def reset_display(self):
        self._check(self._L.cpt_reset_display(self._ctx))

    def math_batch(self, op, a, b=None):
        a = np.ascontiguousarray(a, dtype=np.float32)
        b = np.ascontiguousarray(b if b is not None else np.zeros_like(a), dtype=np.float32)
        out = np.empty_like(a)
        self._check(self._L.cpt_math_batch(self._ctx, op, _p(a), _p(b), _p(out), a.size))
        return out
```

include/cpt.h:

```cpp
#ifndef CPT_H_
#define CPT_H_

#include <stddef.h>
#include <stdint.h>

#ifdef __cplusplus
extern "C" {
#endif

#define CPT_ABI_VERSION 1

enum cpt_status {
    CPT_OK = 0,
    CPT_ERR_INVALID_ARG = 1,
    CPT_ERR_NO_DEVICE = 2,
    CPT_ERR_HIP = 3,
    CPT_ERR_OUT_OF_MEMORY = 4,
    CPT_ERR_STATE = 5,
    CPT_ERR_UNSUPPORTED = 6,
    CPT_ERR_DEVICE = 7
};

enum cpt_primitive_type { CPT_PRIM_SPHERE = 0, CPT_PRIM_PLATFORM = 1, CPT_PRIM_CYLINDER = 2 };
enum cpt_material_type {
    CPT_MAT_DIFFUSE = 0,
    CPT_MAT_METAL = 1,
    CPT_MAT_MIRROR = 2,
    CPT_MAT_GLASS = 3,
    CPT_MAT_TEST = 4
};

typedef struct cpt_float3 { float x, y, z; } cpt_float3;

typedef struct cpt_material {
    int32_t type;
    uint8_t have_tex;
    uint8_t pad_[3];
    union {
        cpt_float3 kd;
        uint64_t tex;
    } u;
    float refractive_index;
    float emit_intensity;
    float smoothness;
    float reflectivity;
} cpt_material;

typedef struct cpt_object {
    int32_t type;
    int32_t pad_;
    cpt_material material;
    cpt_float3 center;
    float radius;
    float y_pos;
    float height;
} cpt_object;

typedef struct cpt_camera {
    cpt_float3 vup;
    int32_t width, height;
    uint32_t cur_sample_idx;
    cpt_float3 origin;
    cpt_float3 look_at;
    float view_fov;
    float dist_to_focus;
    float lens_radius;
    float move_speed;
    cpt_float3 u, v, w;
    cpt_float3 top_left_corner;
    cpt_float3 horizontal;
    cpt_float3 vertical;
} cpt_camera;

typedef struct cpt_stats {
    uint64_t segments;
    uint64_t node_visits;
    uint64_t prim_tests;
    uint64_t hits;
    uint64_t misses;
} cpt_stats;

typedef struct cpt_ctx cpt_ctx;

#define CPT_RENDER_ACCUMULATE 0x1u
#define CPT_RENDER_AUX        0x2u
#define CPT_RENDER_STATS      0x4u
#define CPT_RENDER_SYNC       0x8u
#define CPT_PATH_MEGAKERNEL   0x000u
#define CPT_PATH_WAVEFRONT    0x100u
#define CPT_TRAVERSAL_ORDERED 0x200u
#define CPT_TRAVERSAL_PLAIN_LEAVES 0x400u
#define CPT_SCHEDULE_COST 0x800u
#define CPT_SCHEDULE_CONSOLIDATE    0x1000u
#define CPT_SCHEDULE_NO_CONSOLIDATE 0x2000u
#define CPT_SCHEDULE_PREVIOUS       0x4000u

int cpt_abi_version(void);
const char* cpt_status_string(int status);
int cpt_get_device_count(int* count);

int cpt_create(int device, cpt_ctx** out);
int cpt_destroy(cpt_ctx* ctx);
const char* cpt_last_error(const cpt_ctx* ctx);
int cpt_set_stream(cpt_ctx* ctx, void* hip_stream);

int cpt_camera_get_copy(cpt_camera* cam);

int cpt_set_scene(cpt_ctx* ctx, const cpt_object* objs, int n_objs);
int cpt_update_object(cpt_ctx* ctx, int index, const cpt_object* obj);
int cpt_update_objects(cpt_ctx* ctx, int n, const int* indices, const cpt_object* objs);
int cpt_update_objects_rebuild(cpt_ctx* ctx, int n, const int* indices, const cpt_object* objs);
int cpt_get_material_count(cpt_ctx* ctx, int* n);
int cpt_last_update_ms(cpt_ctx* ctx, float* ms);
int cpt_scene_bvh_export(cpt_ctx* ctx, float* boxes, int32_t* links, int capacity, int* n_nodes);
int cpt_bvh_build_host(const cpt_object* objs, int n_objs, float* boxes, int32_t* links, int capacity, int* n_nodes);

int cpt_set_env_texture(cpt_ctx* ctx, const uint8_t* rgba, int logical_width, int height, int valid_cols);

#define CPT_ADDRESS_WRAP   0
#define CPT_ADDRESS_CLAMP  1
#define CPT_ADDRESS_MIRROR 2
#define CPT_ADDRESS_BORDER 3
#define CPT_FILTER_POINT   0
#define CPT_FILTER_LINEAR  1

int cpt_bind_texture(cpt_ctx* ctx, uint64_t handle, const uint8_t* rgba, int logical_width, int height,
                     int valid_cols, int address_mode, int filter_mode);

int cpt_set_frame(cpt_ctx* ctx, int width, int height, const int32_t* rows, int n_rows);
int cpt_init_rng(cpt_ctx* ctx, uint64_t seed);
int cpt_read_rng(cpt_ctx* ctx, uint32_t* planar6);
int cpt_write_rng(cpt_ctx* ctx, const uint32_t* planar6);

int cpt_render(cpt_ctx* ctx, const cpt_camera* cam, int spp, int max_depth, uint32_t flags);
int cpt_synchronize(cpt_ctx* ctx);
int cpt_read_accum(cpt_ctx* ctx, float* rgba);
int cpt_clear_accum(cpt_ctx* ctx);
int cpt_read_aux(cpt_ctx* ctx, float* normal3, float* depth);
int cpt_write_accum(cpt_ctx* ctx, const float* rgba);
int cpt_write_aux(cpt_ctx* ctx, const float* normal3, const float* depth);
int cpt_tile_costs(cpt_ctx* ctx, const cpt_camera* cam, int passes, int max_depth, uint32_t flags, uint32_t* out,
                   size_t n_out);
int cpt_render_adaptive(cpt_ctx* ctx, const cpt_camera* cam, int min_spp, int max_spp, int batch, float rel_error,
                        int max_depth, uint32_t flags);
int cpt_adaptive_begin(cpt_ctx* ctx, const cpt_camera* cam, int min_spp, int max_spp, int batch, float rel_error,
                       int max_depth, uint32_t flags);
int cpt_adaptive_step(cpt_ctx* ctx, int* active_tiles);
int cpt_read_noise(cpt_ctx* ctx, float* rel, size_t capacity);
int cpt_adaptive_info(cpt_ctx* ctx, int* rounds, uint32_t* active_tiles_per_round, int capacity,
                      uint64_t* passes_done);
int cpt_adaptive_decide_host(float m1, float m2, float k, float t, int* converged, float* rel);
int cpt_read_moments(cpt_ctx* ctx, float* planar4, size_t capacity);
int cpt_write_moments(cpt_ctx* ctx, const float* planar4, size_t count);

int cpt_filter_frame(cpt_ctx* ctx, int levels, float sigma_l, int normal_sharpness_log2);
int cpt_read_filtered(cpt_ctx* ctx, float* rgb, float* variance, size_t capacity_pixels);
int cpt_last_filter_ms(cpt_ctx* ctx, float* ms);
int cpt_filter_prepare_host(size_t npix, const float* accum_rgba, const float* moments_planar4, float* out_rgbv,
                            uint8_t* out_valid);
int cpt_filter_level_host(int width, int height, int step, const float* in_rgbv, const float* normal3, const uint8_t* valid,
                          float sigma_l, int normal_sharpness_log2, float* out_rgbv);
int cpt_copy_accum_device(cpt_ctx* ctx, void* device_dst, size_t bytes, void* caller_stream);
int cpt_gather_rows(cpt_ctx* dst, cpt_ctx* src);
#define CPT_GATHER_SAME_DEVICE 0
#define CPT_GATHER_PEER 1
#define CPT_GATHER_STAGED 2
int cpt_last_gather_mode(cpt_ctx* dst, cpt_ctx* src, int* mode);
int cpt_set_debug_gather(cpt_ctx* dst, int force_staged);
int cpt_get_stats(cpt_ctx* ctx, cpt_stats* out);
int cpt_reset_stats(cpt_ctx* ctx);
int cpt_get_raw_counters(cpt_ctx* ctx, uint64_t* out8);
int cpt_debug_timeline(cpt_ctx* ctx, uint64_t* out, int n);
int cpt_get_diag_counters(cpt_ctx* ctx, uint64_t* out16);
int cpt_get_execdiag_counters(cpt_ctx* ctx, uint64_t* out64);
int cpt_get_walk_info(cpt_ctx* ctx, int32_t* out4);
int cpt_debug_read_nodes(cpt_ctx* ctx, void* out, size_t capacity_bytes, size_t* n_bytes);
int cpt_debug_read_tile_order(cpt_ctx* ctx, int which, uint32_t* out, size_t capacity, size_t* n);
int cpt_last_render_ms(cpt_ctx* ctx, float* ms);
int cpt_last_kernel_stats(cpt_ctx* ctx, float* avg_ms, int* launches);

int cpt_denoise_mix(cpt_ctx* ctx, uint32_t cur_sample_idx, uint8_t* bgra_host);
int cpt_host_register(void* ptr, size_t bytes);
int cpt_host_unregister(void* ptr);
int cpt_denoise_mix_band(cpt_ctx* ctx, uint32_t cur_sample_idx, int y0, int y1, uint8_t* bgra_host);
int cpt_copy_bgra_device(cpt_ctx* ctx, void* device_dst, size_t bytes, void* caller_stream);
int cpt_display_band(const cpt_ctx* ctx, int* y0, int* y1);
int cpt_read_mix(cpt_ctx* ctx, float* rgb, size_t capacity);
int cpt_last_display_ms(cpt_ctx* ctx, float* ms);
int cpt_reset_display(cpt_ctx* ctx);

int cpt_measure_read_bandwidth(cpt_ctx* ctx, size_t bytes, int iters, float* gbps);
int cpt_measure_read_pattern(cpt_ctx* ctx, int bytes_per_lane, size_t bytes, int iters, float* gbps);
int cpt_cap_disk_bound(float radius, float* out);
int cpt_math_batch(cpt_ctx* ctx, int op, const float* a, const float* b, float* out, size_t n);
int cpt_selftest_qdiv(cpt_ctx* ctx, int which, uint64_t n, uint64_t seed, uint64_t* out, int out_len);
int cpt_set_debug_consolidation(cpt_ctx* ctx, uint32_t flags, int keeper_spin_log2, int publish_wait_log2);
int cpt_set_debug_grid(cpt_ctx* ctx, int max_workgroups, int lanes_per_wave);

#ifdef __cplusplus
}
#endif

#endif
```

Baseline: 2230 Mpaths/s.

## Stage wide-BVH leaves in dynamic LDS and size traversal stack to tree bound

After: 2244 Mpaths/s (median of 6 runs). About the same (+0.6%).

```diff
diff --git a/cpppathtracer_amd/_lib.py b/cpppathtracer_amd/_lib.py
--- a/cpppathtracer_amd/_lib.py
+++ b/cpppathtracer_amd/_lib.py
@@ -48,6 +48,10 @@
     "cpt_reset_stats": (_I, [_P]),
     "cpt_get_raw_counters": (_I, [_P, _P]),
     "cpt_get_walk_info": (_I, [_P, _P]),
+    "cpt_get_walk_layout": (_I, [_P, _P]),
+    "cpt_walk_build_host": (_I, [_P, _I, _P, _P, _SZ, _P]),
+    "cpt_walk_lds_layout": (_I, [_I, _I, _I, _I, _I, _P]),
+    "cpt_set_debug_leaf_staging": (_I, [_P, _I]),
     "cpt_debug_read_nodes": (_I, [_P, _P, _SZ, _P]),
     "cpt_debug_read_tile_order": (_I, [_P, _I, _P, _SZ, _P]),
     "cpt_measure_read_bandwidth": (_I, [_P, _SZ, _I, _P]),
diff --git a/cpppathtracer_amd/csrc/cpt_capi_render.cpp b/cpppathtracer_amd/csrc/cpt_capi_render.cpp
--- a/cpppathtracer_amd/csrc/cpt_capi_render.cpp
+++ b/cpppathtracer_amd/csrc/cpt_capi_render.cpp
@@ -7,10 +7,13 @@
 #include <utility>
 
 #include "cpt_context.hpp"
+#include "cpt_tuning.hpp"
 
 using namespace cpt::ctx;
 
 constexpr int PREV_ORDER_EVERY = 8;
+
+static int stage_leaves(const cpt_ctx* c) { return c->dbg_leaf_staging < 0 ? (cpt::STAGE_LEAVES ? 1 : 0) : c->dbg_leaf_staging; }
 
 void cpt::ctx::fill_params(cpt_ctx* c, const cpt_camera* cam, int spp, int max_depth, uint32_t flags, cpt::KParams& p) {
     std::memset(&p, 0, sizeof(p));
@@ -21,6 +24,8 @@
     p.n_wide = c->n_wide;
     p.n_unb = c->n_unb;
     p.n_leaves = c->n_wide > 0 ? c->n_leaves : 0;
+    p.stack_bound = c->wide_stack_bound;
+    p.stage_leaves = stage_leaves(c);
     p.ordered = (flags & CPT_TRAVERSAL_ORDERED) ? ((flags & CPT_TRAVERSAL_PLAIN_LEAVES) ? 2 : 1) : 0;
     p.env = c->d_env;
     p.env_w = c->env_w;
@@ -243,6 +248,50 @@
     return CPT_OK;
 }
 
+int cpt_set_debug_leaf_staging(cpt_ctx* c, int mode) {
+    if (!c || mode < -1 || mode > 1) return c ? fail(c, CPT_ERR_INVALID_ARG, "cpt_set_debug_leaf_staging: bad mode") : CPT_ERR_INVALID_ARG;
+    c->dbg_leaf_staging = mode;
+    return CPT_OK;
+}
+
+static void layout_words(const cpt::LdsLayout& l, int32_t* out8) {
+    out8[0] = l.tree_nodes;
+    out8[1] = l.stack_entries;
+    out8[2] = l.n_lds_leaves;
+    out8[3] = (int32_t)l.off_pending;
+    out8[4] = (int32_t)l.off_tree;
+    out8[5] = (int32_t)l.off_stack;
+    out8[6] = (int32_t)l.off_leaves;
+    out8[7] = (int32_t)l.bytes;
+}
+
+int cpt_walk_lds_layout(int n_wide, int stack_bound, int n_unb, int n_leaves, int stage_leaves, int32_t* out8) {
+    if (!out8 || n_wide < 0 || n_unb < 0 || n_leaves < n_unb || stack_bound < 0 || stack_bound + 1 > CPT_WSTACK)
+        return CPT_ERR_INVALID_ARG;
+    cpt::KParams p{};
+    p.n_wide = n_wide;
+    p.n_unb = n_unb;
+    p.n_leaves = n_leaves;
+    p.stack_bound = stack_bound;
+    p.stage_leaves = stage_leaves;
+    layout_words(cpt::megakernel_lds_layout(p), out8);
+    return CPT_OK;
+}
+
+int cpt_get_walk_layout(cpt_ctx* c, int32_t* out10) {
+    if (!c || !out10) return CPT_ERR_INVALID_ARG;
+    out10[0] = c->n_wide > 0 ? c->n_leaves : 0;
+    out10[1] = c->wide_stack_bound;
+    cpt::KParams p{};
+    p.n_wide = c->n_wide;
+    p.n_unb = c->n_unb;
+    p.n_leaves = out10[0];
+    p.stack_bound = c->wide_stack_bound;
+    p.stage_leaves = stage_leaves(c);
+    layout_words(cpt::megakernel_lds_layout(p), out10 + 2);
+    return CPT_OK;
+}
+
 int cpt_last_render_ms(cpt_ctx* c, float* ms) {
     if (!c || !ms) return CPT_ERR_INVALID_ARG;
     if (!c->t_render.recorded) return fail(c, CPT_ERR_STATE, "cpt_last_render_ms: nothing rendered");
diff --git a/cpppathtracer_amd/csrc/cpt_context.hpp b/cpppathtracer_amd/csrc/cpt_context.hpp
--- a/cpppathtracer_amd/csrc/cpt_context.hpp
+++ b/cpppathtracer_amd/csrc/cpt_context.hpp
@@ -128,6 +128,7 @@
     int n_wide = 0;
     int n_unb = 0;
     int n_leaves = 0;
+    int wide_stack_bound = 0;
     std::vector<Mat> mats_h;
     std::vector<int> mat_have_tex;
     std::vector<uint64_t> mat_tex;
@@ -185,6 +186,7 @@
     bool force_staged_gather = false;
     int keeper_spin_log2 = 0, publish_wait_log2 = 0;
     int dbg_max_workgroups = 0, dbg_lanes_per_wave = 0;
+    int dbg_leaf_staging = -1;
 
     hipStream_t stream() const { return user_stream ? user_stream : (hipStream_t)own_stream; }
     size_t npix() const { return (size_t)n_rows * width; }
diff --git a/cpppathtracer_amd/csrc/cpt_host.hpp b/cpppathtracer_amd/csrc/cpt_host.hpp
--- a/cpppathtracer_amd/csrc/cpt_host.hpp
+++ b/cpppathtracer_amd/csrc/cpt_host.hpp
@@ -44,7 +44,8 @@
 
 constexpr int WIDE_STACK = CPT_WSTACK;
 int linearise_wide(const HostBvh& w, int root, const std::vector<int>& pos0, int n_bvh, int n_unb,
-                   std::vector<Node>& out, int* n_leaves_out, std::vector<int>& slot_of, std::vector<int>& leaf_of);
+                   std::vector<Node>& out, int* n_leaves_out, int* stack_bound_out, std::vector<int>& slot_of,
+                   std::vector<int>& leaf_of);
 
 const std::vector<uint32_t>& jump_tables();
 void curand_seed_state(uint64_t seed, uint32_t out[6]);
diff --git a/cpppathtracer_amd/csrc/cpt_host_bvh.cpp b/cpppathtracer_amd/csrc/cpt_host_bvh.cpp
--- a/cpppathtracer_amd/csrc/cpt_host_bvh.cpp
+++ b/cpppathtracer_amd/csrc/cpt_host_bvh.cpp
@@ -271,7 +271,8 @@
 
 
 int linearise_wide(const HostBvh& w, int root, const std::vector<int>& pos0, int n_bvh, int n_unb,
-                   std::vector<Node>& out, int* n_leaves_out, std::vector<int>& slot_of, std::vector<int>& leaf_of) {
+                   std::vector<Node>& out, int* n_leaves_out, int* stack_bound_out, std::vector<int>& slot_of,
+                   std::vector<int>& leaf_of) {
     std::vector<int> wbin;
     std::vector<std::vector<int>> kids;
     std::vector<int> wide_of(w.nodes.size(), -1);
@@ -304,6 +305,7 @@
     };
     make(root, n_unb);
     if (max_push + 1 > WIDE_STACK) return 0;
+    *stack_bound_out = max_push - n_unb;
     const int n_wide = (int)wbin.size();
     std::vector<int> li_of(w.nodes.size(), -1), leaf_pos;
     for (int k = 0; k < n_unb; ++k) leaf_pos.push_back(k);
diff --git a/cpppathtracer_amd/csrc/cpt_internal.hpp b/cpppathtracer_amd/csrc/cpt_internal.hpp
--- a/cpppathtracer_amd/csrc/cpt_internal.hpp
+++ b/cpppathtracer_amd/csrc/cpt_internal.hpp
@@ -11,6 +11,28 @@
 
 constexpr int LDS_TREE_NODES = 512;
 __host__ __device__ __forceinline__ int lds_tree_nodes(int n_wide) { return n_wide < LDS_TREE_NODES ? n_wide : LDS_TREE_NODES; }
+
+constexpr uint32_t LDS_CU_BYTES = 160u * 1024u, LDS_STATIC_RESERVE = 1024u;
+constexpr uint32_t LDS_PENDING_FLOATS = 9;
+struct LdsLayout {
+    int tree_nodes, stack_entries, n_lds_leaves;
+    uint32_t off_pending, off_tree, off_stack, off_leaves, bytes;
+};
+inline LdsLayout lds_layout(int n_wide, int stack_bound, int n_unb, int n_leaves, int lanes, bool stage_leaves) {
+    LdsLayout l{};
+    l.tree_nodes = lds_tree_nodes(n_wide);
+    l.stack_entries = (stack_bound + 2) & ~1;
+    l.off_pending = 0;
+    l.off_tree = LDS_PENDING_FLOATS * (uint32_t)lanes * 4u;
+    l.off_stack = l.off_tree + (uint32_t)l.tree_nodes * 112u;
+    l.off_leaves = l.off_stack + (uint32_t)l.stack_entries * (uint32_t)lanes * 2u;
+    const uint32_t budget = LDS_CU_BYTES - LDS_STATIC_RESERVE;
+    const int room = l.off_leaves < budget ? (int)((budget - l.off_leaves) / 32u) : 0;
+    l.n_lds_leaves = n_leaves < room ? n_leaves : room;
+    if (!stage_leaves && l.n_lds_leaves > n_unb) l.n_lds_leaves = n_unb;
+    l.bytes = l.off_leaves + (uint32_t)l.n_lds_leaves * 32u;
+    return l;
+}
 
 struct CamK {
     float origin[3];
@@ -51,6 +73,9 @@
     uint32_t dbg;
     int keeper_spin_log2, publish_wait_log2;
     uint32_t n_active;
+    int stack_bound, stage_leaves;
+    uint32_t lds_stack, lds_leaves;
+    int n_lds_leaves;
 };
 
 enum : uint32_t {
@@ -113,6 +138,7 @@
                         Node* leaves, hipStream_t stream);
 
 hipError_t launch_megakernel(const KParams& p, bool stats, bool aux, int max_workgroups, hipStream_t stream);
+LdsLayout megakernel_lds_layout(const KParams& p);
 hipError_t launch_wavefront(const KParams& p, WfState& w, bool stats, bool aux, hipStream_t stream, int* launches);
 hipError_t wavefront_build_ident(const KParams& p, WfState& w, hipStream_t stream);
 hipError_t launch_prepare_materials(Mat* mats, const int32_t* tex_of_mat, const TexDesc* texs, int n,
diff --git a/cpppathtracer_amd/csrc/cpt_megakernel.hip b/cpppathtracer_amd/csrc/cpt_megakernel.hip
--- a/cpppathtracer_amd/csrc/cpt_megakernel.hip
+++ b/cpppathtracer_amd/csrc/cpt_megakernel.hip
@@ -69,16 +69,26 @@
 template <bool LDST> constexpr int mk_block() { return LDST ? LDS_BLOCK : 256; }
 template <bool LDST> constexpr int mk_waves() { return LDST ? LDS_BLOCK / 256 : WAVES_PER_SIMD; }
 
-template <bool STATS, bool AUX, bool PROBE, bool LDST, bool CONS, bool HYB>
+extern __shared__ uint4 s_dyn[];
+template <bool LDST> constexpr uint32_t mk_tree_off() { return LDS_PENDING_FLOATS * (uint32_t)mk_block<LDST>() * 4u; }
+
+template <bool STATS, bool AUX, bool PROBE, bool LDST, bool CONS, bool HYB, int LEAVES>
 __global__ void __launch_bounds__(mk_block<LDST>(), mk_waves<LDST>()) k_megakernel(const KParams p) {
     constexpr bool COUNT = STATS || PROBE;
     constexpr int BLK = mk_block<LDST>();
-    __shared__ uint4 s_tree[LDST ? LDS_TREE_NODES * 7 : 1];
+    static_assert(LDST ? LEAVES != LEAVES_GLOBAL : LEAVES == LEAVES_GLOBAL, "the LDS kernels stage leaves");
     pooldiag::init();
+    WideLds lds{};
     if (LDST) {
+        uint4* const s_tree = s_dyn + mk_tree_off<LDST>() / 16u;
+        uint4* const s_leaves = s_dyn + p.lds_leaves / 16u;
         const uint4* src = reinterpret_cast<const uint4*>(p.nodes + wide_image_base(p));
         for (int i = threadIdx.x; i < 7 * lds_tree_nodes(p.n_wide); i += BLK) s_tree[i] = src[i];
+        src = reinterpret_cast<const uint4*>(p.nodes + wide_leaves_base(p));
+        for (int i = threadIdx.x; i < 2 * p.n_lds_leaves; i += BLK) s_leaves[i] = src[i];
         __syncthreads();
+        lds = WideLds{s_tree, (lds_i16*)reinterpret_cast<int16_t*>(s_dyn + p.lds_stack / 16u) + threadIdx.x, s_leaves,
+                      p.n_lds_leaves};
     }
     const int lane = threadIdx.x & 63;
     const size_t npix = (size_t)p.n_rows * p.width;
@@ -96,7 +106,8 @@
     bool first = true;
     v3 first_normal = mk1(0.f);
 
-    __shared__ float pending_q[DEFER_MISS_ROUND > 0 ? 9 * BLK : 1];
+    __shared__ float s_pending[!LDST && DEFER_MISS_ROUND > 0 ? LDS_PENDING_FLOATS * BLK : 1];
+    float* const pending_q = LDST ? reinterpret_cast<float*>(s_dyn) : s_pending;
     const PendingSky<BLK> pq{pending_q + threadIdx.x};
     bool pend = false;
     WalkState ws;
@@ -326,7 +337,7 @@
             const RayK rk = make_rayk(ray);
             const bool finite_ray = !(ray.o.x != ray.o.x || ray.o.y != ray.o.y || ray.o.z != ray.o.z ||
                                       ray.d.x != ray.d.x || ray.d.y != ray.d.y || ray.d.z != ray.d.z);
-            tr = trace_segment<COUNT, BLK, LDST, HYB>(p, rk, finite_ray, h, code, cnt, s_tree, ws, LDST ? SUSPEND_AT : 0);
+            tr = trace_segment<COUNT, BLK, LDST, HYB, LEAVES>(p, rk, finite_ray, h, code, cnt, lds, ws, LDST ? SUSPEND_AT : 0);
         }
         stamps::lap(3);
         if (busy && L.left > 0 && tr != 2) {
@@ -487,16 +498,24 @@
     }
 }
 
-template <bool S, bool A, bool P, bool T, bool C = false, bool H = false>
-static hipError_t launch_mk(const KParams& p, int max_workgroups, hipStream_t stream) {
+LdsLayout megakernel_lds_layout(const KParams& p) {
+    return lds_layout(p.n_wide, p.stack_bound, p.n_unb, p.n_leaves, mk_block<true>(), p.stage_leaves != 0);
+}
+
+template <bool S, bool A, bool P, bool T, bool C = false, bool H = false, int L = LEAVES_GLOBAL>
+static hipError_t launch_mk(const KParams& p, int max_workgroups, hipStream_t stream, uint32_t lds_bytes = 0) {
     static int blocks_per_cu = -1, cus = 0;
     constexpr int block = mk_block<T>();
     if (blocks_per_cu < 0) {
         int dev = 0;
         hipError_t e = hipGetDevice(&dev);
         if (e == hipSuccess) e = hipDeviceGetAttribute(&cus, hipDeviceAttributeMultiprocessorCount, dev);
+        if (e == hipSuccess && T)
+            e = hipFuncSetAttribute(reinterpret_cast<const void*>(&k_megakernel<S, A, P, T, C, H, L>),
+                                    hipFuncAttributeMaxDynamicSharedMemorySize, (int)(LDS_CU_BYTES - LDS_STATIC_RESERVE));
         if (e == hipSuccess)
-            e = hipOccupancyMaxActiveBlocksPerMultiprocessor(&blocks_per_cu, k_megakernel<S, A, P, T, C, H>, block, 0);
+            e = hipOccupancyMaxActiveBlocksPerMultiprocessor(&blocks_per_cu, k_megakernel<S, A, P, T, C, H, L>, block,
+                                                             lds_bytes);
         if (e != hipSuccess) return e;
         if (blocks_per_cu < 1) blocks_per_cu = 1;
     }
@@ -506,25 +525,38 @@
     long long grid = std::min<long long>(want, (long long)blocks_per_cu * cus);
     if (max_workgroups > 0) grid = std::min<long long>(grid, max_workgroups);
     if (grid < 1) return hipSuccess;
-    hipLaunchKernelGGL((k_megakernel<S, A, P, T, C, H>), dim3((unsigned)grid), dim3(block), 0, stream, p);
+    hipLaunchKernelGGL((k_megakernel<S, A, P, T, C, H, L>), dim3((unsigned)grid), dim3(block), lds_bytes, stream, p);
     return hipGetLastError();
 }
 
 static bool use_lds_tree(const KParams& p) { return p.ordered == 1 && p.n_wide > 0; }
 
+template <bool S, bool A, bool P, bool H, int L>
+static hipError_t launch_mk_lds(const KParams& p, int max_workgroups, hipStream_t stream, uint32_t lds_bytes) {
+    if constexpr (!P && ho_slots<mk_block<true>()>() > 0) {
+        if (p.resume) return launch_mk<S, A, P, true, true, H, L>(p, max_workgroups, stream, lds_bytes);
+    }
+    return launch_mk<S, A, P, true, false, H, L>(p, max_workgroups, stream, lds_bytes);
+}
+
 template <bool S, bool A, bool P, bool H>
-static hipError_t launch_mk_lds(const KParams& p, int max_workgroups, hipStream_t stream) {
-    if constexpr (!P && ho_slots<mk_block<true>()>() > 0) {
-        if (p.resume) return launch_mk<S, A, P, true, true, H>(p, max_workgroups, stream);
-    }
-    return launch_mk<S, A, P, true, false, H>(p, max_workgroups, stream);
+static hipError_t launch_mk_laid_out(const KParams& p0, int max_workgroups, hipStream_t stream) {
+    const LdsLayout l = megakernel_lds_layout(p0);
+    if (l.off_tree != mk_tree_off<true>() || l.n_lds_leaves < p0.n_unb || l.bytes > LDS_CU_BYTES - LDS_STATIC_RESERVE)
+        return hipErrorInvalidValue;
+    KParams p = p0;
+    p.lds_stack = l.off_stack;
+    p.lds_leaves = l.off_leaves;
+    p.n_lds_leaves = l.n_lds_leaves;
+    if (l.n_lds_leaves == p.n_leaves) return launch_mk_lds<S, A, P, H, LEAVES_LDS_ALL>(p, max_workgroups, stream, l.bytes);
+    return launch_mk_lds<S, A, P, H, LEAVES_LDS_PREFIX>(p, max_workgroups, stream, l.bytes);
 }
 
 template <bool S, bool A, bool P>
 static hipError_t launch_mk_any(const KParams& p, int max_workgroups, hipStream_t stream) {
     if (!use_lds_tree(p)) return launch_mk<S, A, P, false>(p, max_workgroups, stream);
-    if (p.n_wide > LDS_TREE_NODES) return launch_mk_lds<S, A, P, true>(p, max_workgroups, stream);
-    return launch_mk_lds<S, A, P, false>(p, max_workgroups, stream);
+    if (p.n_wide > LDS_TREE_NODES) return launch_mk_laid_out<S, A, P, true>(p, max_workgroups, stream);
+    return launch_mk_laid_out<S, A, P, false>(p, max_workgroups, stream);
 }
 
 hipError_t launch_megakernel(const KParams& p, bool stats, bool aux, int max_workgroups, hipStream_t stream) {
diff --git a/cpppathtracer_amd/csrc/cpt_path.hpp b/cpppathtracer_amd/csrc/cpt_path.hpp
--- a/cpppathtracer_amd/csrc/cpt_path.hpp
+++ b/cpppathtracer_amd/csrc/cpt_path.hpp
@@ -568,16 +568,39 @@
 };
 
 
-template <bool STATS, int BLK, bool HYB>
+struct WideLds {
+    const uint4* tree;
+    lds_i16* stack;
+    const uint4* leaves;
+    int n_lds_leaves;
+};
+enum : int { LEAVES_GLOBAL = 0, LEAVES_LDS_PREFIX = 1, LEAVES_LDS_ALL = 2 };
+
+template <bool STATS, int BLK, bool HYB, int LEAVES>
 __device__ __forceinline__ int trace_wide(const KParams& p, __amdgpu_buffer_rsrc_t rsrc, int oct, const RayK& ray,
-                                          Hit& h, int& code_out, Counters& cnt, const uint4* tree, WalkState& ws,
+                                          Hit& h, int& code_out, Counters& cnt, const WideLds& lds, WalkState& ws,
                                           int suspend_at) {
-    __shared__ int16_t wstack[CPT_WSTACK * BLK];
-    lds_i16* const stk = (lds_i16*)wstack + threadIdx.x;
+    const uint4* const tree = lds.tree;
+    lds_i16* const stk = lds.stack;
     constexpr int leaf0 = 0;
     auto leaf_of = [&](int ref) { return ~ref - 1; };
     const BufSrc leaf_src{rsrc, (uint32_t)wide_leaves_base(p) * (uint32_t)sizeof(Node)};
-    auto leaf = [&](int i) -> Node { return leaf_src(i); };
+    auto leaf_lds = [&](int i) -> Node {
+        typedef unsigned int v4u_t __attribute__((ext_vector_type(4)));
+        typedef __attribute__((address_space(3))) const v4u_t lds_v4u;
+        typedef __attribute__((address_space(3))) const uint4 lds_u4;
+        lds_v4u* const q = (lds_v4u*)(uintptr_t)((uint32_t)(uintptr_t)(lds_u4*)lds.leaves + ((uint32_t)i << 5));
+        const v4u_t a = q[0], b = q[1];
+        Node n;
+        n.a0 = __uint_as_float(a.x); n.a1 = __uint_as_float(a.y); n.a2 = __uint_as_float(a.z); n.miss = (int32_t)a.w;
+        n.b0 = __uint_as_float(b.x); n.b1 = __uint_as_float(b.y); n.b2 = __uint_as_float(b.z); n.code = (int32_t)b.w;
+        return n;
+    };
+    auto leaf = [&](int i) -> Node {
+        if (LEAVES == LEAVES_LDS_ALL || (LEAVES == LEAVES_LDS_PREFIX && __builtin_expect(i < lds.n_lds_leaves, 1)))
+            return leaf_lds(i);
+        return leaf_src(i);
+    };
     const int n_lds = lds_tree_nodes(p.n_wide);
     const uint32_t image_off = (uint32_t)wide_image_base(p) * (uint32_t)sizeof(Node);
     constexpr int NONE = -1;
@@ -593,7 +616,7 @@
         ws.best_rank = 0x7fffffff;
         for (int k = 0; k < p.n_unb; ++k) {
             if (STATS) cnt.prims++;
-            const Node pl = leaf(leaf0 + k);
+            const Node pl = LEAVES != LEAVES_GLOBAL ? leaf_lds(leaf0 + k) : leaf_src(leaf0 + k);
             int kk;
             if (ranked_leaf_test<true, true, false>(pl, ray, ws.tmax, kk, ws.best_rank)) {
                 ws.best = leaf0 + k;
@@ -719,9 +742,9 @@
     return trace<STATS, FAST, CONS>(BufSrc{rsrc, base}, n, ray, h, code, cnt);
 }
 
-template <bool STATS, int BLK = WIDE_LANES, bool LDST = false, bool HYB = true>
+template <bool STATS, int BLK = WIDE_LANES, bool LDST = false, bool HYB = true, int LEAVES = LEAVES_GLOBAL>
 __device__ __forceinline__ int trace_segment(const KParams& p, const RayK& rk, bool finite, Hit& h, int& code,
-                                             Counters& cnt, const uint4* tree, WalkState& ws, int suspend_at) {
+                                             Counters& cnt, const WideLds& lds, WalkState& ws, int suspend_at) {
     const __amdgpu_buffer_rsrc_t rsrc = node_rsrc(p);
     if (p.ordered && __builtin_expect(finite, 1)) {
         int n, r = -1;
@@ -729,7 +752,7 @@
         if constexpr (LDST) {
             if (p.ordered == 1 && p.n_wide > 0) {
                 const int oct = (rk.d.x < 0.f ? 1 : 0) | (rk.d.y < 0.f ? 2 : 0) | (rk.d.z < 0.f ? 4 : 0);
-                r = trace_wide<STATS, BLK, HYB>(p, rsrc, oct, rk, h, code, cnt, tree, ws, suspend_at);
+                r = trace_wide<STATS, BLK, HYB, LEAVES>(p, rsrc, oct, rk, h, code, cnt, lds, ws, suspend_at);
                 wide = true;
             }
         }
@@ -747,10 +770,10 @@
 
 template <bool STATS, int BLK = WIDE_LANES, bool LDST = false>
 __device__ __forceinline__ bool trace_segment(const KParams& p, const RayK& rk, bool finite, Hit& h, int& code,
-                                              Counters& cnt, const uint4* tree = nullptr) {
+                                              Counters& cnt, const WideLds& lds = WideLds{}) {
     WalkState ws;
     ws.active = false;
-    return trace_segment<STATS, BLK, LDST>(p, rk, finite, h, code, cnt, tree, ws, 0) == 1;
+    return trace_segment<STATS, BLK, LDST>(p, rk, finite, h, code, cnt, lds, ws, 0) == 1;
 }
 
 struct Shade { v3 radiance, attenuation, bounce; };
diff --git a/cpppathtracer_amd/csrc/cpt_scene.cpp b/cpppathtracer_amd/csrc/cpt_scene.cpp
--- a/cpppathtracer_amd/csrc/cpt_scene.cpp
+++ b/cpppathtracer_amd/csrc/cpt_scene.cpp
@@ -76,6 +76,8 @@
     c->n_walk = 0;
     c->n_wide = 0;
     c->n_unb = 0;
+    c->n_leaves = 0;
+    c->wide_stack_bound = 0;
     c->refit_plan.clear();
     c->lin.reserve(9 * c->bvh.nodes.size());
     linearise(c->bvh, c->objs, c->mat_of_obj, c->lin, c->pos_of_node, -1, nullptr);
@@ -88,9 +90,11 @@
     c->n_walk = (int)(c->lin.size() - c->n_bvh) / 8;
     c->n_unb = (int)unbounded.size();
     c->n_leaves = 0;
+    c->wide_stack_bound = 0;
     std::vector<int> slot_of(w.nodes.size(), -1), leaf_of(w.nodes.size(), -1);
     if (root >= 0 && !w.nodes[root].is_object)
-        c->n_wide = linearise_wide(w, root, pos[0], c->n_bvh, c->n_unb, c->lin, &c->n_leaves, slot_of, leaf_of);
+        c->n_wide = linearise_wide(w, root, pos[0], c->n_bvh, c->n_unb, c->lin, &c->n_leaves, &c->wide_stack_bound, slot_of,
+                                   leaf_of);
     build_refit_plan(c, w, pos, slot_of, leaf_of);
 }
 
@@ -411,6 +415,29 @@
     return CPT_OK;
 }
 
+int cpt_walk_build_host(const cpt_object* objs, int n, int32_t* info8, void* out, size_t capacity_bytes, size_t* n_bytes) {
+    if (n < 0 || (n > 0 && !objs) || !info8 || !n_bytes) return CPT_ERR_INVALID_ARG;
+    try {
+        cpt_ctx c;
+        c.objs.assign(objs, objs + n);
+        build_host_bvh(c.bvh, c.objs);
+        c.mat_of_obj.assign(n, 0);
+        for (int i = 0; i < n; ++i) c.mat_of_obj[i] = material_slot(&c, c.objs[i].material);
+        linearise_all(&c);
+        const int32_t info[8] = {c.n_bvh, c.n_walk, c.n_wide, c.n_unb, c.n_wide > 0 ? c.n_leaves : 0, c.wide_stack_bound, 0, 0};
+        std::memcpy(info8, info, sizeof(info));
+        const size_t bytes = c.lin.size() * sizeof(Node);
+        *n_bytes = bytes;
+        if (out) {
+            if (capacity_bytes < bytes) return CPT_ERR_INVALID_ARG;
+            if (bytes) std::memcpy(out, c.lin.data(), bytes);
+        }
+    } catch (const std::bad_alloc&) {
+        return CPT_ERR_OUT_OF_MEMORY;
+    }
+    return CPT_OK;
+}
+
 int cpt_set_env_texture(cpt_ctx* c, const uint8_t* rgba, int logical_width, int height, int valid_cols) {
     if (!c) return CPT_ERR_INVALID_ARG;
     if (logical_width <= 0 || height <= 0 || valid_cols < 0 || valid_cols > logical_width || (valid_cols > 0 && !rgba))
diff --git a/cpppathtracer_amd/csrc/cpt_tuning.hpp b/cpppathtracer_amd/csrc/cpt_tuning.hpp
--- a/cpppathtracer_amd/csrc/cpt_tuning.hpp
+++ b/cpppathtracer_amd/csrc/cpt_tuning.hpp
@@ -12,6 +12,10 @@
 constexpr int TAKE_BATCH = 64;
 constexpr int TAKE_TAPER = 4;
 constexpr int CONS_RETIRE_PER_LEVEL = 256;
+#ifndef CPT_STAGE_LEAVES
+#define CPT_STAGE_LEAVES 1
+#endif
+constexpr bool STAGE_LEAVES = CPT_STAGE_LEAVES != 0;
 #ifndef CPT_FILTER_LDS_MAX_STEP
 #define CPT_FILTER_LDS_MAX_STEP 2
 #endif
diff --git a/cpppathtracer_amd/csrc/cpt_wavefront.hip b/cpppathtracer_amd/csrc/cpt_wavefront.hip
--- a/cpppathtracer_amd/csrc/cpt_wavefront.hip
+++ b/cpppathtracer_amd/csrc/cpt_wavefront.hip
@@ -89,6 +89,8 @@
     constexpr int BLK = wf_extend_block<LDST>();
     const uint32_t n = *nin;
     __shared__ uint4 s_tree[LDST ? LDS_TREE_NODES * 7 : 1];
+    __shared__ int16_t s_wstack[LDST ? CPT_WSTACK * BLK : 1];
+    const WideLds lds{s_tree, (lds_i16*)s_wstack + threadIdx.x, nullptr, 0};
     if (LDST) {
         if ((uint32_t)blockIdx.x * BLK >= n) return;
         const uint4* src = reinterpret_cast<const uint4*>(p.nodes + wide_image_base(p));
@@ -111,7 +113,7 @@
         int code = -1;
         if (STATS) cnt.segments++;
         bool hit;
-        if (LDST) hit = trace_segment<STATS, BLK, true>(p, rk, finite, h, code, cnt, s_tree);
+        if (LDST) hit = trace_segment<STATS, BLK, true>(p, rk, finite, h, code, cnt, lds);
         else hit = trace_segment<STATS>(p, rk, finite, h, code, cnt);
         w.hit_p[i] = make_float4(h.pos.x, h.pos.y, h.pos.z, __int_as_float(hit ? code : -1));
         if (hit) w.hit_n[i] = make_float4(h.normal.x, h.normal.y, h.normal.z, 0.f);
diff --git a/cpppathtracer_amd/renderer.py b/cpppathtracer_amd/renderer.py
--- a/cpppathtracer_amd/renderer.py
+++ b/cpppathtracer_amd/renderer.py
@@ -22,6 +22,31 @@
     n = ctypes.c_int(0)
     check(L.cpt_get_device_count(ctypes.byref(n)))
     return n.value
+
+
+LDS_LAYOUT_KEYS = ("tree_nodes", "stack_entries", "n_lds_leaves", "off_pending", "off_tree", "off_stack", "off_leaves",
+                   "bytes")
+
+
+def host_walk_tree(objs):
+    L = _lib.load()
+    objs = np.ascontiguousarray(objs, dtype=OBJECT_DTYPE)
+    info = np.zeros(8, dtype=np.int32)
+    n = ctypes.c_size_t(0)
+    ptr = _p(objs) if len(objs) else None
+    check(L.cpt_walk_build_host(ptr, len(objs), _p(info), None, 0, ctypes.byref(n)))
+    out = np.zeros(n.value, dtype=np.uint8)
+    if n.value:
+        check(L.cpt_walk_build_host(ptr, len(objs), _p(info), _p(out), out.size, ctypes.byref(n)))
+    keys = ("n_bvh", "n_walk", "n_wide", "n_unb", "n_leaves", "stack_bound")
+    return dict(zip(keys, (int(x) for x in info))), out
+
+
+def walk_lds_layout(n_wide, stack_bound, n_unb, n_leaves, stage_leaves=True):
+    L = _lib.load()
+    out = np.zeros(8, dtype=np.int32)
+    check(L.cpt_walk_lds_layout(int(n_wide), int(stack_bound), int(n_unb), int(n_leaves), int(bool(stage_leaves)), _p(out)))
+    return dict(zip(LDS_LAYOUT_KEYS, (int(x) for x in out)))
 
 
 def camera_get_copy(cam):
@@ -305,7 +330,19 @@
     def walk_info(self):
         out = np.zeros(4, dtype=np.int32)
         self._check(self._L.cpt_get_walk_info(self._ctx, _p(out)))
-        return dict(zip(("n_bvh", "n_walk", "n_wide", "n_unb"), (int(x) for x in out)))
+        info = dict(zip(("n_bvh", "n_walk", "n_wide", "n_unb"), (int(x) for x in out)))
+        if hasattr(self._L, "cpt_get_walk_layout"):
+            lay = self.walk_layout()
+            info["n_leaves"], info["stack_bound"] = lay["n_leaves"], lay["stack_bound"]
+        return info
+
+    def walk_layout(self):
+        out = np.zeros(10, dtype=np.int32)
+        self._check(self._L.cpt_get_walk_layout(self._ctx, _p(out)))
+        return dict(zip(("n_leaves", "stack_bound") + LDS_LAYOUT_KEYS, (int(x) for x in out)))
+
+    def set_debug_leaf_staging(self, mode=-1):
+        self._check(self._L.cpt_set_debug_leaf_staging(self._ctx, int(mode)))
 
     def read_nodes(self):
         n = ctypes.c_size_t(0)
diff --git a/include/cpt.h b/include/cpt.h
--- a/include/cpt.h
+++ b/include/cpt.h
@@ -174,6 +174,9 @@
 int cpt_get_diag_counters(cpt_ctx* ctx, uint64_t* out16);
 int cpt_get_execdiag_counters(cpt_ctx* ctx, uint64_t* out64);
 int cpt_get_walk_info(cpt_ctx* ctx, int32_t* out4);
+int cpt_get_walk_layout(cpt_ctx* ctx, int32_t* out10);
+int cpt_walk_lds_layout(int n_wide, int stack_bound, int n_unb, int n_leaves, int stage_leaves, int32_t* out8);
+int cpt_walk_build_host(const cpt_object* objs, int n, int32_t* info8, void* out, size_t capacity_bytes, size_t* n_bytes);
 int cpt_debug_read_nodes(cpt_ctx* ctx, void* out, size_t capacity_bytes, size_t* n_bytes);
 int cpt_debug_read_tile_order(cpt_ctx* ctx, int which, uint32_t* out, size_t capacity, size_t* n);
 int cpt_last_render_ms(cpt_ctx* ctx, float* ms);
@@ -196,6 +199,7 @@
 int cpt_selftest_qdiv(cpt_ctx* ctx, int which, uint64_t n, uint64_t seed, uint64_t* out, int out_len);
 int cpt_set_debug_consolidation(cpt_ctx* ctx, uint32_t flags, int keeper_spin_log2, int publish_wait_log2);
 int cpt_set_debug_grid(cpt_ctx* ctx, int max_workgroups, int lanes_per_wave);
+int cpt_set_debug_leaf_staging(cpt_ctx* ctx, int mode);
 
 #ifdef __cplusplus
 }
```
